# TinfoilHat0/Defending-Against-Backdoors-with-Robust-Learning-Rate

Hardware: NVIDIA H100
Metric: fl_rounds_per_sec (higher is better)
Workload: dtype bf16

## Files before the change

### defending-against-backdoors-with-robust-learning-rate_b200/models/native.py

```python
from __future__ import annotations

import math
import os

import torch
import torch.nn.functional as F

from .. import ops
from .graph import FlatLayout

ACT = torch.bfloat16
FUSE_DROPOUT = bool(int(os.environ.get("RLR_FUSE_DROPOUT", "1")))
FUSE_RELU_POOL = bool(int(os.environ.get("RLR_FUSE_RELU_POOL", "1")))
EPILOGUE_BN_STATS = bool(int(os.environ.get("RLR_EPILOGUE_BN_STATS", "0")))
FWD_BRANCH = bool(int(os.environ.get("RLR_FWD_BRANCH", "1")))
BWD_BRANCH = bool(int(os.environ.get("RLR_BWD_BRANCH", "1")))
EPI_STAT_SLOTS = min(16, max(1, int(os.environ.get("RLR_EPI_STAT_SLOTS", "2"))))
FWD_SLOTS = BWD_SLOTS = max(1, int(os.environ.get("RLR_BN_SLOTS", "1")))
WGRAD_OVERLAP = bool(int(os.environ.get("RLR_WGRAD_OVERLAP", "1")))


def dropout_stream_base(seed: int, agent_id: int, rnd: int) -> int:
    z = (int(seed) * 0x9E3779B97F4A7C15 + (int(agent_id) + 1) * 0xBF58476D1CE4E5B9 + (int(rnd) + 1) * 0x94D049BB133111EB) & (2 ** 64 - 1)
    z = ((z ^ (z >> 30)) * 0xBF58476D1CE4E5B9) & (2 ** 64 - 1)
    z = ((z ^ (z >> 27)) * 0x94D049BB133111EB) & (2 ** 64 - 1)
    return (z ^ (z >> 31)) & (2 ** 62 - 1)


def native_supported(layout: FlatLayout) -> bool:
    return all(nd.op in ("conv", "bn", "relu", "maxpool", "avgpool", "flatten", "dropout", "linear", "save", "add")
               for nd in layout.nodes)


class _Op:
    __slots__ = ("kind", "node", "name", "attrs", "x", "y", "res", "relu", "saved", "acc_dx", "need_dx", "in_shape", "out_shape")

    def __init__(self, kind, **kw):
        self.kind = kind
        self.node = self.name = self.x = self.y = self.res = None
        self.attrs, self.relu, self.saved, self.acc_dx, self.need_dx = {}, False, {}, False, True
        self.in_shape = self.out_shape = None
        for k, v in kw.items():
            setattr(self, k, v)


class NativeNet:
    def __init__(self, layout: FlatLayout, device, max_batch: int, impl: str | dict = "auto", seed: int = 0, act_dtype=None):
        self.layout, self.device, self.max_batch = layout, torch.device(device), int(max_batch)
        self.act_dtype = act_dtype or ACT
        default = ("sm100" if self.device.type == "cuda" else "aten") if impl == "auto" else impl
        self.impl = dict(conv_fwd=default, conv_dgrad=default, conv_wgrad=default, bn=default, pool=default,
                         linear=default, dropout=default) if not isinstance(impl, dict) else dict(impl)
        self.seed = seed
        self.fuse_bn_stats = False
        self.first_wait = None
        self.after_first_op = None
        self.step_counter = torch.zeros(1, dtype=torch.int64, device=device)
        self._build_plan()
        self._alloc()

    def _build_plan(self):
        nodes = self.layout.nodes
        C, H, W = self.layout.in_shape
        shape = {"x": (H, W, C)}
        ver = {"x": 0}
        tid = lambda s: f"{s}@{ver[s]}"
        self.tshape = {tid("x"): shape["x"]}
        plan, consumed = [], set()
        pending_bn = {}
        alias = {}

        def new_out(slot, shp):
            ver[slot] = ver.get(slot, -1) + 1
            shape[slot] = shp
            self.tshape[tid(slot)] = shp
            return tid(slot)

        def next_same_slot(i, slot):
            for j in range(i + 1, len(nodes)):
                if j in consumed:
                    continue
                nd = nodes[j]
                if nd.op == "save":
                    if nd.inp == slot:
                        return None, None
                    continue
                if nd.inp == slot or nd.out == slot:
                    return j, nd
            return None, None

        for i, nd in enumerate(nodes):
            if i in consumed:
                continue
            a = nd.attrs
            if nd.op == "save":
                ver[nd.out] = ver.get(nd.out, -1) + 1
                alias[f"{nd.out}@{ver[nd.out]}"] = tid(nd.inp)
                shape[nd.out] = shape[nd.inp]
                self.tshape[f"{nd.out}@{ver[nd.out]}"] = shape[nd.inp]
                continue
            src = alias.get(tid(nd.inp), tid(nd.inp))
            if nd.op == "conv":
                h, w, c = shape[nd.inp]
                k, s, p = a["k"], a.get("stride", 1), a.get("pad", 0)
                ho, wo = (h + 2 * p - k) // s + 1, (w + 2 * p - k) // s + 1
                op = _Op("conv", node=i, name=nd.name, attrs=a, x=src, in_shape=(h, w, c), out_shape=(ho, wo, a["cout"]))
                j, nx = next_same_slot(i, nd.out)
                want_stats = nx is not None and nx.op == "bn"
                if nx is not None and nx.op == "relu":
                    op.relu = True
                    consumed.add(j)
                op.saved["want_stats"] = want_stats
                op.y = new_out(nd.out, op.out_shape)
                plan.append(op)
            elif nd.op == "bn":
                shp = shape[nd.inp]
                op = _Op("bn", node=i, name=nd.name, attrs=a, x=src, in_shape=shp, out_shape=shp)
                j, nx = next_same_slot(i, nd.out)
                if nx is not None and nx.op == "relu":
                    op.relu = True
                    consumed.add(j)
                    op.y = new_out(nd.out, shp)
                    plan.append(op)
                elif nx is not None and nx.op == "add":
                    pending_bn[j] = op
                else:
                    op.y = new_out(nd.out, shp)
                    plan.append(op)
            elif nd.op == "add":
                other = alias.get(tid(a["other"]), tid(a["other"]))
                op = pending_bn.pop(i, None)
                if op is None:
                    raise NotImplementedError("add without a preceding BatchNorm is not used by any model in the zoo")
                op.res = other
                j, nx = next_same_slot(i, nd.out)
                if nx is not None and nx.op == "relu":
                    op.relu = True
                    consumed.add(j)
                op.y = new_out(nd.out, op.out_shape)
                plan.append(op)
            elif nd.op == "relu":
                raise NotImplementedError("stand-alone ReLU (every ReLU in the zoo follows conv/bn/linear)")
            elif nd.op == "maxpool":
                h, w, c = shape[nd.inp]
                op = _Op("maxpool", node=i, x=src, in_shape=(h, w, c), out_shape=(h // 2, w // 2, c))
                op.y = new_out(nd.out, op.out_shape)
                plan.append(op)
            elif nd.op == "avgpool":
                h, w, c = shape[nd.inp]
                op = _Op("avgpool", node=i, x=src, in_shape=(h, w, c), out_shape=(1, 1, c))
                op.y = new_out(nd.out, op.out_shape)
                plan.append(op)
            elif nd.op == "flatten":
                shp = shape[nd.inp]
                ver[nd.out] += 1
                alias[tid(nd.out)] = src
                shape[nd.out] = (int(math.prod(shp)),)
                self.tshape[tid(nd.out)] = shape[nd.out]
            elif nd.op == "dropout":
                shp = shape[nd.inp]
                prod = next((q for q in reversed(plan) if q.y == src), None)
                fusable = (prod is not None and a.get("p", 0.0) > 0 and "drop" not in prod.saved and
                           (prod.kind == "maxpool" or
                            (prod.kind == "linear" and prod.relu and ops.linear_fused_dropout_ok(prod.attrs["cout"], prod.attrs["cin"]))))
                if fusable and FUSE_DROPOUT:
                    prod.saved["drop"] = (float(a["p"]), i)
                    ver[nd.out] += 1
                    alias[tid(nd.out)] = src
                    shape[nd.out] = shp
                    self.tshape[tid(nd.out)] = shp
                else:
                    op = _Op("dropout", node=i, attrs=a, x=src, in_shape=shp, out_shape=shp)
                    op.y = new_out(nd.out, shp)
                    plan.append(op)
            elif nd.op == "linear":
                op = _Op("linear", node=i, name=nd.name, attrs=a, x=src, in_shape=shape[nd.inp], out_shape=(a["cout"],))
                j, nx = next_same_slot(i, nd.out)
                if nx is not None and nx.op == "relu":
                    op.relu = True
                    consumed.add(j)
                op.y = new_out(nd.out, op.out_shape)
                plan.append(op)
            else:
                raise NotImplementedError(nd.op)
        for op in plan:
            if op.kind != "maxpool":
                continue
            prod = next((q for q in plan if q.y == op.x), None)
            users = [q for q in plan if q.x == op.x or q.res == op.x]
            if prod is not None and prod.kind == "conv" and prod.relu and len(users) == 1 and FUSE_RELU_POOL:
                op.saved["relu_bwd_here"] = True
                prod.saved["relu_bwd_fused"] = True
        self.plan = plan
        self.alias = alias
        self.out_tid = alias.get(tid("x"), tid("x"))
        self.in_tid = "x@0"
        written = set()
        for op in reversed(plan):
            op.need_dx = op.x != self.in_tid
            if op.res is not None:
                written.add(op.res)
            if op.need_dx:
                op.acc_dx = op.x in written
                written.add(op.x)

    def _numel(self, shp):
        return int(math.prod(shp))

    def _alloc(self):
        B, dev = self.max_batch, self.device
        self.act, self.grad = {}, {}
        for op in self.plan:
            self.act[op.y] = torch.empty((B, *op.out_shape), dtype=self.act_dtype, device=dev)
        for op in self.plan:
            for t in (op.x, op.res):
                if t is not None and t != self.in_tid and t not in self.grad:
                    self.grad[t] = torch.empty((B, *self.tshape[t]), dtype=self.act_dtype, device=dev)
        self.grad[self.out_tid] = torch.empty((B, *self.tshape[self.out_tid]), dtype=self.act_dtype, device=dev)
        self.logits = torch.empty((B, self.tshape[self.out_tid][-1]), dtype=torch.float32, device=dev)
        need = [op for op in self.plan if op.kind == "bn" or (op.kind == "conv" and op.saved.get("want_stats"))]
        S = ops.STAT_SLOTS
        tot = sum(2 * op.out_shape[-1] for op in need)
        self.stats_arena = torch.zeros(max(1, tot * S), dtype=torch.float32, device=dev)
        D = BWD_SLOTS
        self.dsum_arena = torch.zeros(max(1, tot * D), dtype=torch.float32, device=dev)
        off = 0
        for op in need:
            c = op.out_shape[-1]
            op.saved["stats"] = self.stats_arena[off * S:(off + 2 * c) * S].view(S, 2, c)
            op.saved["dsum"] = self.dsum_arena[off * D:(off + 2 * c) * D].view(D, 2, c)
            op.saved["mean_rstd"] = torch.zeros(2, c, dtype=torch.float32, device=dev)
            off += 2 * c
        for op in self.plan:
            if op.kind == "maxpool":
                op.saved["idx"] = torch.empty((B, *op.out_shape), dtype=torch.uint8, device=dev)
                if "drop" in op.saved and self.impl["pool"] != "sm100":
                    op.saved["dmask"] = torch.ones((B, *op.out_shape), dtype=torch.uint8, device=dev)
            if op.kind == "dropout":
                op.saved["mask"] = torch.empty((B, *op.out_shape), dtype=torch.uint8, device=dev)
        self._bn_src = {}
        for i, op in enumerate(self.plan):
            if not (FWD_BRANCH and op.kind == "conv" and ".downsample." in (op.name or "")):
                continue
            nxt = self.plan[i + 1] if i + 1 < len(self.plan) else None
            first = next((q for q in self.plan[:i] if q.x == op.x and q is not op), None)
            join = next((q for q in self.plan[i + 1:] if nxt is not None and q.res == nxt.y), None)
            if nxt is None or nxt.kind != "bn" or nxt.x != op.y or first is None or join is None:
                continue
            first.saved["fork_before"] = True
            op.saved["side_branch"] = nxt.saved["side_branch"] = True
            join.saved["join_before"] = True
        for i, op in enumerate(self.plan):
            if op.kind == "bn":
                prod = next((q for q in self.plan[:i] if q.y == op.x and q.kind == "conv"), None)
                op.saved["producer"] = prod

    def bind(self, w, wb, g, w_buffers=None):
        self.w, self.wb, self.g = w, wb, g
        lay = self.layout
        self.pw = {p.name: lay.view(w, p) for p in lay.params}
        self.pw.update({b.name: lay.view(w if w_buffers is None else w_buffers, b) for b in lay.buffers})
        self.pwb = {p.name: lay.view(wb, p) for p in lay.params} if wb is not None else {}
        self.pg = {p.name: lay.view(g, p) for p in lay.params} if g is not None else {}

    def T(self, t, B):
        return self.act[t][:B] if t != self.in_tid else self._x

    def stem_geometry(self):
        op = self.plan[0]
        if op.kind != "conv" or op.x != self.in_tid or self.impl["conv_fwd"] != "sm100" or self.impl["conv_wgrad"] != "sm100":
            return None
        return ops.stem_geometry(op.in_shape, op.attrs)

    def G(self, t, B):
        return self.grad[t][:B]

    def forward(self, x_nhwc, train: bool):
        out = self.forward_raw(x_nhwc, train)
        B = out.shape[0]
        self.logits[:B].copy_(out)
        return self.logits[:B]

    def forward_raw(self, x_nhwc, train: bool):
        B = x_nhwc.shape[0] if x_nhwc.dim() == 4 else x_nhwc.shape[0] // (self.plan[0].out_shape[0] * self.plan[0].out_shape[1])
        self._x, self._B, self._train = x_nhwc, B, train
        self._epoch = getattr(self, "_epoch", 0) + 1
        if train:
            ops.zero_(self.stats_arena)
        branch = FWD_BRANCH and self.device.type == "cuda" and ops.nn.USE_STRIDED_TMA and self.impl["conv_fwd"] == "sm100"
        if branch and getattr(self, "_branch_stream", None) is None:
            self._branch_stream = torch.cuda.Stream(self.device)
        for i, op in enumerate(self.plan):
            if branch and op.saved.get("fork_before"):
                self._branch_stream.wait_stream(torch.cuda.current_stream(self.device))
            if branch and op.saved.get("join_before"):
                torch.cuda.current_stream(self.device).wait_stream(self._branch_stream)
            if branch and op.saved.get("side_branch"):
                with torch.cuda.stream(self._branch_stream):
                    getattr(self, "_fwd_" + op.kind)(op, B, train)
            else:
                getattr(self, "_fwd_" + op.kind)(op, B, train)
            if i == 0 and self.after_first_op is not None:
                self.after_first_op()
        return self.T(self.out_tid, B).reshape(B, -1)

    def dlogits_buffer(self, B):
        return self.G(self.out_tid, B).reshape(B, -1)

    def backward(self, dlogits):
        B = dlogits.shape[0]
        gout = self.G(self.out_tid, B)
        if dlogits.data_ptr() != gout.data_ptr():
            gout.copy_(dlogits.reshape(gout.shape))
        ops.zero_(self.g)
        ops.zero_(self.dsum_arena)
        self._side = None
        if WGRAD_OVERLAP and self.device.type == "cuda":
            if getattr(self, "_side_stream", None) is None:
                self._side_stream = torch.cuda.Stream(self.device)
            self._side = self._side_stream
            self._side.wait_stream(torch.cuda.current_stream(self.device))
        branch = (BWD_BRANCH and FWD_BRANCH and self.device.type == "cuda" and ops.nn.USE_STRIDED_TMA and self.impl["conv_fwd"] == "sm100"
                  and getattr(self, "_branch_stream", None) is not None)
        cur = torch.cuda.current_stream(self.device) if branch else None
        for op in reversed(self.plan):
            if branch and op.saved.get("fork_before"):
                cur.wait_stream(self._branch_stream)
            if branch and op.saved.get("side_branch"):
                if op.kind == "bn":
                    self._branch_stream.wait_stream(cur)
                with torch.cuda.stream(self._branch_stream):
                    getattr(self, "_bwd_" + op.kind)(op, B)
            else:
                getattr(self, "_bwd_" + op.kind)(op, B)
        if self._side is not None:
            torch.cuda.current_stream(self.device).wait_stream(self._side)
            self._side = None

    def _epilogue_stats_free(self, op):
        if not EPILOGUE_BN_STATS or self.impl["conv_fwd"] != "sm100":
            return False
        a = op.attrs
        return a.get("stride", 1) == 1 and a["cin"] % 64 == 0 and a["cout"] % 64 == 0 and not (a["k"] == 3 and a["cin"] == 64)

    def _fwd_conv(self, op, B, train):
        a = op.attrs
        x, y = self.T(op.x, B), self.T(op.y, B)
        bias = self.pw.get(op.name + ".bias")
        stats = op.saved.get("stats") if (train and op.saved.get("want_stats") and (self.fuse_bn_stats or self._epilogue_stats_free(op))) else None
        op.saved["stats_done"] = stats is not None
        if self.impl["conv_fwd"] == "sm100" and ops.conv_supported(op.in_shape, a, "fwd"):
            ops.conv2d_fwd_sm100(x, self.pwb[op.name + ".weight"], bias, y, a.get("stride", 1), a.get("pad", 0), op.relu, stats, tag=(id(self), op.name),
                                 zero_stats=False, s2d_epoch=self._epoch, wait=self.first_wait if (op is self.plan[0] and x.dim() == 2) else None)
            return
        if self.impl["conv_fwd"] == "sm100":
            ops.note_fallback("conv_fwd", f"{op.name} in={op.in_shape} {a}")
        wt = self.pwb[op.name + ".weight"].permute(0, 3, 1, 2)
        out = F.conv2d(x.permute(0, 3, 1, 2), wt, bias.to(self.act_dtype) if bias is not None else None, a.get("stride", 1), a.get("pad", 0))
        if op.relu:
            out = F.relu(out)
        y.copy_(out.permute(0, 2, 3, 1))
        if stats is not None:
            yf = y.float().reshape(-1, y.shape[-1])
            stats[0, 0].copy_(yf.sum(0)); stats[0, 1].copy_((yf * yf).sum(0))

    def _bwd_conv(self, op, B):
        a = op.attrs
        x, y, dy = self.T(op.x, B), self.T(op.y, B), self.G(op.y, B)
        if op.relu and not op.saved.get("relu_bwd_fused"):
            ops.relu_bwd_(dy, y, self.impl["bn"])
        name = op.name + ".weight"
        gw, gb = self.pg[name], self.pg.get(op.name + ".bias")
        s, p = a.get("stride", 1), a.get("pad", 0)
        if self.impl["conv_wgrad"] == "sm100" and ops.conv_supported(op.in_shape, a, "wgrad"):
            if getattr(self, "_side", None) is not None:
                self._side.wait_stream(torch.cuda.current_stream(self.device))
                with torch.cuda.stream(self._side):
                    ops.conv2d_wgrad_sm100(x, dy, gw, gb, s, p, tag=(id(self), op.name), zero=False)
            else:
                ops.conv2d_wgrad_sm100(x, dy, gw, gb, s, p, tag=(id(self), op.name), zero=False)
        else:
            if self.impl["conv_wgrad"] == "sm100":
                ops.note_fallback("conv_wgrad", f"{op.name} in={op.in_shape} {a}")
            _, dw, db = torch.ops.aten.convolution_backward(
                dy.permute(0, 3, 1, 2), x.permute(0, 3, 1, 2), self.pwb[name].permute(0, 3, 1, 2),
                [a["cout"]] if gb is not None else None, [s, s], [p, p], [1, 1], False, [0, 0], 1, [False, True, gb is not None])
            gw.copy_(dw.permute(0, 2, 3, 1))
            if gb is not None:
                gb.copy_(db)
        if not op.need_dx:
            return
        dx = self.G(op.x, B)
        if self.impl["conv_dgrad"] == "sm100" and ops.conv_supported(op.in_shape, a, "dgrad"):
            ops.conv2d_dgrad_sm100(dy, self.pwb[name], dx, s, p, op.acc_dx)
            return
        if self.impl["conv_dgrad"] == "sm100":
            ops.note_fallback("conv_dgrad", f"{op.name} in={op.in_shape} {a}")
        di, _, _ = torch.ops.aten.convolution_backward(
            dy.permute(0, 3, 1, 2), x.permute(0, 3, 1, 2), self.pwb[name].permute(0, 3, 1, 2), None, [s, s], [p, p], [1, 1],
            False, [0, 0], 1, [True, False, False])
        di = di.permute(0, 2, 3, 1)
        if op.acc_dx:
            dx.add_(di)
        else:
            dx.copy_(di)

    def _fwd_bn(self, op, B, train):
        a = op.attrs
        x, y = self.T(op.x, B), self.T(op.y, B)
        res = self.T(op.res, B) if op.res is not None else None
        gamma, beta = self.pw[op.name + ".weight"], self.pw[op.name + ".bias"]
        rm, rv = self.pw[op.name + ".running_mean"], self.pw[op.name + ".running_var"]
        prod = op.saved["producer"]
        stats = prod.saved["stats"] if (train and prod is not None and prod.saved.get("stats_done")) else None
        if stats is not None and not self.fuse_bn_stats:
            stats = stats[0:EPI_STAT_SLOTS]
        count = x.numel() // x.shape[-1]
        ops.bn_fwd(x, y, res, gamma, beta, rm, rv, stats, op.saved["mean_rstd"], count, a.get("eps", 1e-5),
                   a.get("momentum", 0.1), train, op.relu, self.impl["bn"],
                   stats_buf=op.saved["stats"][0:FWD_SLOTS] if train else None)

    def _bwd_bn(self, op, B):
        x, y, dy = self.T(op.x, B), self.T(op.y, B), self.G(op.y, B)
        dres = self.G(op.res, B) if op.res is not None else None
        dx = self.G(op.x, B)
        gamma = self.pw[op.name + ".weight"]
        ops.bn_bwd(dy, y, x, gamma, op.saved["mean_rstd"], op.saved["dsum"], dx, dres,
                   self.pg[op.name + ".weight"], self.pg[op.name + ".bias"], op.relu, self.impl["bn"], zero_dsum=False,
                   beta=self.pw[op.name + ".bias"])

    def _drop(self, op, train=True):
        d = op.saved.get("drop")
        return (d[0], self.seed, self.step_counter, d[1]) if (d is not None and train) else None

    def _fwd_maxpool(self, op, B, train):
        drop = self._drop(op, train)
        op.saved["drop_on"] = drop is not None
        mask = op.saved["dmask"][:B] if (drop is not None and "dmask" in op.saved) else None
        ops.maxpool2_fwd(self.T(op.x, B), self.T(op.y, B), op.saved["idx"][:B], self.impl["pool"], drop, mask)

    def _bwd_maxpool(self, op, B):
        drop = self._drop(op, op.saved.get("drop_on", False))
        mask = op.saved["dmask"][:B] if (drop is not None and "dmask" in op.saved) else None
        ops.maxpool2_bwd(self.G(op.y, B), op.saved["idx"][:B], self.G(op.x, B), self.impl["pool"], drop, mask,
                         relu_out=self.T(op.y, B) if op.saved.get("relu_bwd_here") else None)

    def _fwd_avgpool(self, op, B, train):
        ops.avgpool_fwd(self.T(op.x, B), self.T(op.y, B), self.impl["pool"])

    def _bwd_avgpool(self, op, B):
        ops.avgpool_bwd(self.G(op.y, B), self.G(op.x, B), self.impl["pool"])

    def _fwd_dropout(self, op, B, train):
        x, y = self.T(op.x, B), self.T(op.y, B)
        if not train:
            y.copy_(x.reshape(y.shape))
            return
        ops.dropout_fwd(x.reshape(B, -1), y.reshape(B, -1), op.saved["mask"][:B].reshape(B, -1), op.attrs["p"], self.seed,
                        self.step_counter, op.node, self.impl["dropout"])

    def _bwd_dropout(self, op, B):
        ops.dropout_bwd(self.G(op.y, B).reshape(B, -1), op.saved["mask"][:B].reshape(B, -1), self.G(op.x, B).reshape(B, -1),
                        op.attrs["p"], self.impl["dropout"])

    def _fwd_linear(self, op, B, train):
        x, y = self.T(op.x, B).reshape(B, -1), self.T(op.y, B)
        drop = self._drop(op, train)
        op.saved["drop_on"] = drop is not None
        ops.linear_fwd(x, self.pwb[op.name + ".weight"], self.pw.get(op.name + ".bias"), y, op.relu, self.impl["linear"], drop)

    def _bwd_linear(self, op, B):
        x, y, dy = self.T(op.x, B).reshape(B, -1), self.T(op.y, B), self.G(op.y, B)
        if op.relu:
            scale = 1.0 / (1.0 - op.saved["drop"][0]) if op.saved.get("drop_on", False) else 1.0
            ops.relu_bwd_(dy, y, self.impl["bn"], scale)
        dx = self.G(op.x, B).reshape(B, -1) if op.need_dx else None
        ops.linear_bwd(x, dy, self.pwb[op.name + ".weight"], dx, self.pg[op.name + ".weight"], self.pg.get(op.name + ".bias"),
                       op.acc_dx, self.impl["linear"], zero=False)


class NativeTrainer:
    name = "native"

    def __init__(self, layout, args, device, max_shard: int, impl="auto"):
        self.layout, self.args = layout, args
        self.device = torch.device(device)
        assert self.device.type == "cuda", "the native trainer runs on sm_90a devices only"
        n = layout.n_total
        self.w = torch.zeros(n, dtype=torch.float32, device=device)
        self.wb = torch.zeros(n, dtype=torch.bfloat16, device=device)
        self.g = torch.zeros(n, dtype=torch.float32, device=device)
        self.m = torch.zeros(n, dtype=torch.float32, device=device)
        self.bs = args.bs
        self.net = NativeNet(layout, device, self.bs, impl, seed=args.seed)
        self.net.bind(self.w, self.wb, self.g)
        self.opt = ops.FlatSGD(n, device, args.client_lr, args.client_moment, 10.0, args.clip, n_pgd=layout.n_vote)
        self.loss_sum = torch.zeros(1, dtype=torch.float32, device=device)
        self.use_graphs = not args.no_graphs
        self.max_shard = max_shard
        self.perm = torch.zeros(max(1, max_shard), dtype=torch.int64, device=device)
        self.cursor = torch.zeros(1, dtype=torch.int32, device=device)
        self.y = torch.zeros(self.bs, dtype=torch.int64, device=device)
        C, H, W = layout.in_shape
        self.x = torch.zeros(self.bs, H, W, C, dtype=ACT, device=device)
        self.stem = self.net.stem_geometry()
        self.xA = torch.zeros(self.bs * self.stem[2] * self.stem[3], 64, dtype=ACT, device=device) if self.stem else None
        self._graphs = {}
        self._eval_nets = {}
        self.bcast = None

    def attach_broadcast(self, fused):
        if self.stem is None or fused.w_bf16 is None:
            return False
        self.bcast = fused
        return True

    def _bind_first(self, w0):
        f = self.bcast
        self.net.bind(f.w_global, f.w_bf16, self.g, w_buffers=self.w)
        lay = self.layout
        first_w = lay.by_name[self.net.plan[0].name + ".weight"]
        lo, hi = f.slices_of(first_w.offset, first_w.offset + first_w.numel)
        self.net.first_wait = (f.ready_ptr, lo, hi, f.epoch_dev) if f.ready_ptr else None
        tail_src, tail_dst = f.w_global[lay.n_vote:], self.w[lay.n_vote:]
        self.net.after_first_op = lambda: ops.ext().acquire_slices(f.ready_ptr, 0, max(0, f.n_slices - 1), f.epoch_dev, tail_src, tail_dst)

    def _bind_normal(self):
        self.net.bind(self.w, self.wb, self.g)
        self.net.first_wait = None
        self.net.after_first_op = None

    def _step(self, dataset, B, w0, first=False):
        if first:
            self._bind_first(w0)
        meta = dataset.meta
        if self.stem is not None:
            k, pad, Ho, Wo = self.stem
            xin = self.xA[:B * Ho * Wo]
            ops.gather_im2col(dataset.data, self.perm, meta.mean, meta.std, k, pad, xin, cursor=self.cursor, targets=dataset.targets,
                              out_labels=self.y, batch=B)
        else:
            xin = self.x[:B]
            ops.gather_normalize(dataset.data, self.perm, meta.mean, meta.std, out=xin, nhwc=True, cursor=self.cursor,
                                 targets=dataset.targets, out_labels=self.y, batch=B)
        logits = self.net.forward_raw(xin, True)
        _, dl = ops.softmax_xent(logits, self.y[:B], True, self.loss_sum, dlogits=self.net.dlogits_buffer(B))
        self.net.backward(dl)
        self.opt.step(self.w, self.g, self.m, w0=w0, w_bf16=self.wb, w_in=self.bcast.w_global if first else None)
        ops.ext().advance_cursor(self.cursor, B, self.net.step_counter)
        if first:
            self._bind_normal()

    def _get_graph(self, dataset, B, w0, first=False):
        key = (B, dataset.data.data_ptr(), w0.data_ptr(), bool(first))
        if key in self._graphs:
            return self._graphs[key]
        keep = (self.w.clone(), self.wb.clone(), self.m.clone(), self.cursor.clone(), self.loss_sum.clone(),
                self.net.step_counter.clone())
        self.perm.zero_()
        s = torch.cuda.Stream(self.device)
        s.wait_stream(torch.cuda.current_stream(self.device))
        with torch.cuda.stream(s):
            for _ in range(3):
                self.cursor.zero_()
                c0 = ops.launch_calls()
                self._step(dataset, B, w0, first)
                self._launches = ops.launch_calls() - c0
        torch.cuda.current_stream(self.device).wait_stream(s)
        self.cursor.zero_()
        graph = torch.cuda.CUDAGraph()
        with torch.cuda.graph(graph, capture_error_mode="thread_local"):
            self._step(dataset, B, w0, first)
        self.w.copy_(keep[0]); self.wb.copy_(keep[1]); self.m.copy_(keep[2]); self.cursor.copy_(keep[3])
# ... 58 lines not shown
```

### defending-against-backdoors-with-robust-learning-rate_b200/ops/csrc/common.cuh

```cuda
#pragma once
#include <cuda_runtime.h>
#include <cuda_bf16.h>
#include <stdint.h>

#include "dropspec.h"

#define RLR_CUDA_CHECK(expr)                                                                     \
    do {                                                                                         \
        cudaError_t _e = (expr);                                                                 \
        if (_e != cudaSuccess) return _e;                                                        \
    } while (0)

namespace rlr {

constexpr int kWarp = 32;

__device__ __forceinline__ void pdl_wait() { asm volatile("griddepcontrol.wait;" ::: "memory"); }
__device__ __forceinline__ void pdl_trigger() { asm volatile("griddepcontrol.launch_dependents;" ::: "memory"); }

extern int g_pdl;
bool pdl_enabled();

template <typename... KArgs, typename... Args>
inline cudaError_t launch_kernel(void (*kernel)(KArgs...), dim3 grid, dim3 block, size_t smem, cudaStream_t st, Args&&... args) {
    if (!pdl_enabled()) {
        kernel<<<grid, block, smem, st>>>(static_cast<KArgs>(args)...);
        return cudaGetLastError();
    }
    cudaLaunchConfig_t cfg = {};
    cfg.gridDim = grid; cfg.blockDim = block; cfg.dynamicSmemBytes = smem; cfg.stream = st;
    cudaLaunchAttribute attr[1];
    attr[0].id = cudaLaunchAttributeProgrammaticStreamSerialization;
    attr[0].val.programmaticStreamSerializationAllowed = 1;
    cfg.attrs = attr; cfg.numAttrs = 1;
    return cudaLaunchKernelEx(&cfg, kernel, static_cast<KArgs>(args)...);
}

void* scratch_alloc(size_t bytes, cudaStream_t st);
void scratch_free(void* p);
struct Scratch {
    void* p;
    Scratch(size_t bytes, cudaStream_t st) : p(scratch_alloc(bytes, st)) {}
    ~Scratch() { scratch_free(p); }
    Scratch(const Scratch&) = delete;
    Scratch& operator=(const Scratch&) = delete;
    template <typename T> T* as() const { return static_cast<T*>(p); }
};
template <typename T>
__global__ void __launch_bounds__(256) ordered_sum_kernel(T* __restrict__ out, const T* __restrict__ part, int nparts, long long n) {
    pdl_wait();
    pdl_trigger();
    for (long long i = (long long)blockIdx.x * 256 + threadIdx.x; i < n; i += (long long)gridDim.x * 256) {
        T s = part[i];
        for (int j = 1; j < nparts; ++j) s += part[(size_t)j * n + i];
        out[i] += s;
    }
}

template <typename T>
__global__ void __launch_bounds__(256) ordered_sum_cols_kernel(T* __restrict__ out, const T* __restrict__ part, int nparts, long long n) {
    constexpr int kRows = 64, kPerWarp = kRows / 8;
    __shared__ T tile[kRows][33];
    pdl_wait();
    pdl_trigger();
    const int lane = threadIdx.x & 31, warp = threadIdx.x >> 5;
    const long long col = (long long)blockIdx.x * 32 + lane;
    T s = T(0);
    for (int j0 = 0; j0 < nparts; j0 += kRows) {
        T v[kPerWarp];
#pragma unroll
        for (int q = 0; q < kPerWarp; ++q) {
            const int j = j0 + warp + 8 * q;
            v[q] = (j < nparts && col < n) ? part[(size_t)j * n + col] : T(0);
        }
#pragma unroll
        for (int q = 0; q < kPerWarp; ++q) tile[warp + 8 * q][lane] = v[q];
        __syncthreads();
        if (warp == 0) {
            const int rows = nparts - j0 < kRows ? nparts - j0 : kRows;
            int r = 0;
            if (j0 == 0) { s = tile[0][lane]; r = 1; }
            for (; r < rows; ++r) s += tile[r][lane];
        }
        __syncthreads();
    }
    if (warp == 0 && col < n) out[col] += s;
}

__device__ __forceinline__ unsigned long long gtimer() {
    unsigned long long t;
    asm volatile("mov.u64 %0, %%globaltimer;" : "=l"(t));
    return t;
}

__device__ __forceinline__ float warp_sum(float v) {
#pragma unroll
    for (int o = 16; o > 0; o >>= 1) v += __shfl_xor_sync(0xffffffffu, v, o);
    return v;
}
__device__ __forceinline__ double warp_sum(double v) {
#pragma unroll
    for (int o = 16; o > 0; o >>= 1) v += __shfl_xor_sync(0xffffffffu, v, o);
    return v;
}
__device__ __forceinline__ unsigned long long warp_sum(unsigned long long v) {
#pragma unroll
    for (int o = 16; o > 0; o >>= 1) v += __shfl_xor_sync(0xffffffffu, v, o);
    return v;
}
__device__ __forceinline__ int warp_sum(int v) {
#pragma unroll
    for (int o = 16; o > 0; o >>= 1) v += __shfl_xor_sync(0xffffffffu, v, o);
    return v;
}

__device__ __forceinline__ float warp_transpose_sum32(float (&v)[32], int lane) {
#define RLR_TSTAGE(O, N)                                                         \
    {                                                                            \
        const bool up = (lane & (O)) != 0;                                       \
        _Pragma("unroll") for (int i = 0; i < (N); ++i) {                        \
            const float send = up ? v[i] : v[i + (N)];                           \
            const float keep = up ? v[i + (N)] : v[i];                           \
            v[i] = keep + __shfl_xor_sync(0xffffffffu, send, (O));               \
        }                                                                        \
    }
    RLR_TSTAGE(16, 16) RLR_TSTAGE(8, 8) RLR_TSTAGE(4, 4) RLR_TSTAGE(2, 2) RLR_TSTAGE(1, 1)
#undef RLR_TSTAGE
    return v[0];
}

template <typename T>
__device__ __forceinline__ T block_sum(T v, T* scratch) {
    v = warp_sum(v);
    const int lane = threadIdx.x & 31, wid = threadIdx.x >> 5;
    if (lane == 0) scratch[wid] = v;
    __syncthreads();
    const int nw = (blockDim.x + 31) >> 5;
    v = (threadIdx.x < nw) ? scratch[threadIdx.x] : T(0);
    if (wid == 0) v = warp_sum(v);
    __syncthreads();
    return v;
}

__device__ __forceinline__ float4 ld_stream_f4(const float* p) {
    float4 r;
    asm volatile("ld.global.nc.L1::no_allocate.v4.f32 {%0,%1,%2,%3}, [%4];"
                 : "=f"(r.x), "=f"(r.y), "=f"(r.z), "=f"(r.w) : "l"(p));
    return r;
}
__device__ __forceinline__ float4 ld_f4(const float* p) {
    float4 r;
    asm volatile("ld.global.v4.f32 {%0,%1,%2,%3}, [%4];"
                 : "=f"(r.x), "=f"(r.y), "=f"(r.z), "=f"(r.w) : "l"(p));
    return r;
}
__device__ __forceinline__ float ld_f1(const float* p) {
    float r;
    asm volatile("ld.global.f32 %0, [%1];" : "=f"(r) : "l"(p));
    return r;
}
__device__ __forceinline__ void st_f4(float* p, float4 v) {
    asm volatile("st.global.v4.f32 [%0], {%1,%2,%3,%4};" ::"l"(p), "f"(v.x), "f"(v.y), "f"(v.z), "f"(v.w) : "memory");
}
__device__ __forceinline__ void multimem_st_f4(float* mc, float4 v) {
    asm volatile("multimem.st.relaxed.sys.global.v4.f32 [%0], {%1,%2,%3,%4};" ::"l"(mc), "f"(v.x), "f"(v.y),
                 "f"(v.z), "f"(v.w) : "memory");
}
__device__ __forceinline__ void multimem_st_b2(uint2* mc, uint2 v) {
    asm volatile("multimem.st.relaxed.sys.global.v2.f32 [%0], {%1,%2};" ::"l"(mc), "f"(__uint_as_float(v.x)),
                 "f"(__uint_as_float(v.y)) : "memory");
}

__device__ __forceinline__ void st_release_sys(uint32_t* p, uint32_t v) {
    asm volatile("st.release.sys.global.u32 [%0], %1;" ::"l"(p), "r"(v) : "memory");
}
__device__ __forceinline__ uint32_t ld_acquire_sys(const uint32_t* p) {
    uint32_t v;
    asm volatile("ld.acquire.sys.global.u32 %0, [%1];" : "=r"(v) : "l"(p) : "memory");
    return v;
}
__device__ __forceinline__ void st_release_gpu(uint32_t* p, uint32_t v) {
    asm volatile("st.release.gpu.global.u32 [%0], %1;" ::"l"(p), "r"(v) : "memory");
}
__device__ __forceinline__ uint32_t ld_acquire_gpu(const uint32_t* p) {
    uint32_t v;
    asm volatile("ld.acquire.gpu.global.u32 %0, [%1];" : "=r"(v) : "l"(p) : "memory");
    return v;
}

struct Philox {
    uint32_t k0, k1;
    __device__ __forceinline__ Philox(uint64_t seed) : k0((uint32_t)seed), k1((uint32_t)(seed >> 32)) {}
    __device__ __forceinline__ uint4 operator()(uint64_t ctr, uint64_t stream) const {
        uint32_t c0 = (uint32_t)ctr, c1 = (uint32_t)(ctr >> 32), c2 = (uint32_t)stream, c3 = (uint32_t)(stream >> 32);
        uint32_t a = k0, b = k1;
#pragma unroll
        for (int r = 0; r < 10; ++r) {
            const uint32_t hi0 = __umulhi(0xD2511F53u, c0), lo0 = 0xD2511F53u * c0;
            const uint32_t hi1 = __umulhi(0xCD9E8D57u, c2), lo1 = 0xCD9E8D57u * c2;
            const uint32_t n0 = hi1 ^ c1 ^ a, n2 = hi0 ^ c3 ^ b;
            c0 = n0; c1 = lo1; c2 = n2; c3 = lo0;
            a += 0x9E3779B9u; b += 0xBB67AE85u;
        }
        return make_uint4(c0, c1, c2, c3);
    }
};
__device__ __forceinline__ float u32_to_unit(uint32_t x) {
    return ((float)(x >> 8) + 1.0f) * (1.0f / 16777216.0f);
}
__device__ __forceinline__ float4 philox_normal4(const Philox& ph, uint64_t ctr, uint64_t stream) {
    const uint4 u = ph(ctr, stream);
    const float r0 = sqrtf(-2.0f * logf(u32_to_unit(u.x))), r1 = sqrtf(-2.0f * logf(u32_to_unit(u.z)));
    float s0, c0, s1, c1;
    sincospif(2.0f * u32_to_unit(u.y), &s0, &c0);
    sincospif(2.0f * u32_to_unit(u.w), &s1, &c1);
    return make_float4(r0 * c0, r0 * s0, r1 * c1, r1 * s1);
}

__device__ __forceinline__ uint32_t dropout_keep8(const DropSpec& d, long long q) {
    const Philox ph(d.seed);
    const uint4 u = ph((uint64_t)q, ((uint64_t)(*d.step) << 20) ^ d.stream);
    const uint32_t r[4] = {u.x, u.y, u.z, u.w};
    uint32_t keep = 0;
#pragma unroll
    for (int i = 0; i < 8; ++i) keep |= (uint32_t)(((r[i >> 1] >> (16 * (i & 1))) & 0xffffu) >= d.thr) << i;
    return keep;
}

template <typename T>
inline cudaError_t launch_ordered_sum(T* out, const T* part, int nparts, long long n, cudaStream_t st) {
    if (nparts >= 16)
        return launch_kernel(ordered_sum_cols_kernel<T>, dim3((unsigned)((n + 31) / 32)), dim3(256), (size_t)0, st, out, part, nparts, n);
    long long blocks = (n + 255) / 256;
    if (blocks > 1024) blocks = 1024;
    if (blocks < 1) blocks = 1;
    return launch_kernel(ordered_sum_kernel<T>, dim3((unsigned)blocks), dim3(256), (size_t)0, st, out, part, nparts, n);
}

__device__ __forceinline__ uint32_t pack_bf16x2(float lo, float hi) {
    __nv_bfloat162 v = __floats2bfloat162_rn(lo, hi);
    return *reinterpret_cast<uint32_t*>(&v);
}

}
```

### defending-against-backdoors-with-robust-learning-rate_b200/ops/csrc/conv_halo.cu

```cuda
#include <cuda.h>

#include "common.cuh"
#include "gemm.h"
#include "wgmma.cuh"

namespace rlr {

using namespace wg;

cudaError_t make_tmap_bf16(CUtensorMap* map, const void* base, int rank, const uint64_t* dims, const uint64_t* strides_bytes,
                           const uint32_t* box, const uint32_t* elem_strides = nullptr);

constexpr int HL_THREADS = 256 + 32;
constexpr int HL_TH = 16, HL_TW = 8;
constexpr int HL_PITCH = 16;
constexpr int HL_HALO_BYTES = (HL_TH + 2) * HL_PITCH * 128;
constexpr int HL_W_BYTES = 9 * 64 * 128;
constexpr int HL_STAGES = 3;
constexpr int HL_PITCH_OUT = 64 * 2 + 16;
constexpr int HL_STAGING = 128 * HL_PITCH_OUT;
constexpr int HL_SMEM = HL_W_BYTES + HL_STAGES * HL_HALO_BYTES + 2 * HL_STAGING + 1024 + 1024;

struct HaloParams {
    int NB, H, W;
    int pad;
    int tiles_h, tiles_w, num_tiles;
    int N;
    void* out; int ldc;
    const float* bias;
    float* stats;
    int relu, accumulate;
    long long* dbg;
    int bo_mode;
};

struct __align__(8) HaloShared {
    uint64_t w_full;
    uint64_t halo_full[HL_STAGES];
    uint64_t halo_empty[HL_STAGES];
    float red[128];
    float bias[64];
};

template <bool kStats, bool kAcc>
__global__ void __launch_bounds__(HL_THREADS, 1)
umma_conv3x3_halo_kernel(const __grid_constant__ CUtensorMap tmX, const __grid_constant__ CUtensorMap tmW, const HaloParams p) {
    extern __shared__ uint8_t smem_raw[];
    uint8_t* smem = reinterpret_cast<uint8_t*>((reinterpret_cast<uintptr_t>(smem_raw) + 1023) & ~uintptr_t(1023));
    uint8_t* s_w = smem;
    uint8_t* s_halo = smem + HL_W_BYTES;
    uint8_t* s_stage = s_halo + HL_STAGES * HL_HALO_BYTES;
    HaloShared* sh = reinterpret_cast<HaloShared*>(s_stage + 2 * HL_STAGING);
    const int warp = threadIdx.x >> 5, lane = threadIdx.x & 31;
    const int tile_n = blockIdx.y;
    const int col0 = tile_n * 64;

    if (warp == 8 && lane == 0) {
        prefetch_tmap(&tmX); prefetch_tmap(&tmW);
        mbar_init(&sh->w_full, 1);
        for (int s = 0; s < HL_STAGES; ++s) { mbar_init(&sh->halo_full[s], 1); mbar_init(&sh->halo_empty[s], 4); }
        fence_barrier_init();
    }
    if (threadIdx.x < 128) sh->red[threadIdx.x] = 0.f;
    const int tiles_per_img = p.tiles_h * p.tiles_w;
    pdl_wait();
    pdl_trigger();
    if (threadIdx.x < 64) sh->bias[threadIdx.x] = (p.bias && col0 + (int)threadIdx.x < p.N) ? p.bias[col0 + threadIdx.x] : 0.f;
    __syncthreads();

    if (warp == 8) {
        if (lane == 0) {
            mbar_expect_tx(&sh->w_full, HL_W_BYTES);
            for (int t = 0; t < 9; ++t) tma_load_2d(&tmW, &sh->w_full, s_w + t * 8192, t * 64, tile_n * 64);
            int stage = 0;
            uint32_t phase = 0;
            for (int tile = blockIdx.x; tile < p.num_tiles; tile += gridDim.x) {
                const int n = tile / tiles_per_img, r = tile - n * tiles_per_img;
                const int h0 = (r / p.tiles_w) * HL_TH, w0 = (r % p.tiles_w) * HL_TW;
                mbar_wait(&sh->halo_empty[stage], phase ^ 1);
                mbar_expect_tx(&sh->halo_full[stage], HL_HALO_BYTES);
                tma_load_4d(&tmX, &sh->halo_full[stage], s_halo + stage * HL_HALO_BYTES, 0, w0 - p.pad, h0 - p.pad, n);
                if (++stage == HL_STAGES) { stage = 0; phase ^= 1; }
            }
        }
    } else {
        const int wgi = threadIdx.x >> 7, t = threadIdx.x & 127;
        uint8_t* stage_buf = s_stage + wgi * HL_STAGING;
        const int r0 = frag_row(t, 0);
        __nv_bfloat16* out = reinterpret_cast<__nv_bfloat16*>(p.out);
        float st1[16], st2[16];
#pragma unroll
        for (int i = 0; i < 16; ++i) { st1[i] = 0.f; st2[i] = 0.f; }
        const uint32_t w_base = smem_u32(s_w);
        mbar_wait(&sh->w_full, 0);
        for (int q = wgi;; q += 2) {
            const int tile = blockIdx.x + q * gridDim.x;
            if (tile >= p.num_tiles) break;
            const int stage = q % HL_STAGES;
            const uint32_t phase = (uint32_t)(q / HL_STAGES) & 1u;
            const int n = tile / tiles_per_img, r = tile - n * tiles_per_img;
            const int h0 = (r / p.tiles_w) * HL_TH, w0 = (r % p.tiles_w) * HL_TW;
            uint4 oldv[8];
            if (kAcc) {
#pragma unroll
                for (int it = 0; it < 8; ++it) {
                    const int idx = t + it * 128, rr = idx >> 3, ch = idx & 7;
                    const int h = h0 + (rr >> 3), w = w0 + (rr & 7);
                    oldv[it] = make_uint4(0, 0, 0, 0);
                    if (col0 + ch * 8 < p.N && h < p.H && w < p.W)
                        oldv[it] = *reinterpret_cast<const uint4*>(out + (((size_t)n * p.H + h) * p.W + w) * p.ldc + col0 + ch * 8);
                }
            }
            const bool trace = p.dbg && blockIdx.x == 0 && blockIdx.y == 0 && t == 0;
            if (trace) p.dbg[q * 8 + 0] = clock64();
            mbar_wait(&sh->halo_full[stage], phase);
            if (trace) p.dbg[q * 8 + 2] = clock64();
            const uint32_t halo = smem_u32(s_halo + stage * HL_HALO_BYTES);
            float acc[2][32];
#pragma unroll
            for (int m = 0; m < 2; ++m)
#pragma unroll
                for (int i = 0; i < 32; ++i) acc[m][i] = 0.f;
            wgmma_fence();
#pragma unroll
            for (int tp = 0; tp < 9; ++tp) {
                const int dy = tp / 3, dx = tp - dy * 3;
#pragma unroll
                for (int k = 0; k < 4; ++k) {
                    const uint64_t db = smem_desc_sw128(w_base + tp * 8192 + k * 32, 16, 1024);
#pragma unroll
                    for (int m = 0; m < 2; ++m) {
                        const uint32_t a0 = halo + (dy * HL_PITCH + dx) * 128 + m * 8 * HL_PITCH * 128 + k * 32;
                        const uint32_t bo = p.bo_mode ? ((a0 >> 7) & 7u) : 0u;
                        wgmma_bf16<64, 0, 0>(acc[m], smem_desc_sw128(a0, 16, HL_PITCH * 128, bo), db, (tp > 0 || k > 0) ? 1u : 0u);
                    }
                }
            }
            wgmma_commit();
            wgmma_wait<0>();
            fence_acc(acc[0]);
            fence_acc(acc[1]);
            if (lane == 0) mbar_arrive(&sh->halo_empty[stage]);
            if (trace) p.dbg[q * 8 + 3] = clock64();
#pragma unroll
            for (int m = 0; m < 2; ++m)
#pragma unroll
                for (int j = 0; j < 8; ++j) {
                    const int c = frag_col(t, 4 * j);
#pragma unroll
                    for (int h = 0; h < 2; ++h) {
                        float a = acc[m][4 * j + 2 * h], b = acc[m][4 * j + 2 * h + 1];
                        a += sh->bias[c]; b += sh->bias[c + 1];
                        if (p.relu) { a = fmaxf(a, 0.f); b = fmaxf(b, 0.f); }
                        const uint32_t packed = pack_bf16x2(a, b);
                        if (kStats) {
                            const float2 rq = __bfloat1622float2(*reinterpret_cast<const __nv_bfloat162*>(&packed));
                            st1[2 * j] += rq.x; st1[2 * j + 1] += rq.y;
                            st2[2 * j] += rq.x * rq.x; st2[2 * j + 1] += rq.y * rq.y;
                        }
                        *reinterpret_cast<uint32_t*>(stage_buf + (m * 64 + r0 + 8 * h) * HL_PITCH_OUT + c * 2) = packed;
                    }
                }
            named_bar(1 + wgi, 128);
            if (trace) p.dbg[q * 8 + 6] = clock64();
#pragma unroll
            for (int it = 0; it < 8; ++it) {
                const int idx = t + it * 128;
                const int rr = idx >> 3, ch = idx & 7;
                if (col0 + ch * 8 >= p.N) continue;
                const int h = h0 + (rr >> 3), w = w0 + (rr & 7);
                if (h >= p.H || w >= p.W) continue;
                const size_t gi = ((size_t)n * p.H + h) * p.W + w;
                uint4 val = *reinterpret_cast<const uint4*>(stage_buf + rr * HL_PITCH_OUT + ch * 16);
                uint4* gp = reinterpret_cast<uint4*>(out + gi * p.ldc + col0 + ch * 8);
                if (kAcc) {
                    const __nv_bfloat162* o2 = reinterpret_cast<const __nv_bfloat162*>(&oldv[it]);
                    __nv_bfloat162* v2 = reinterpret_cast<__nv_bfloat162*>(&val);
#pragma unroll
                    for (int qq = 0; qq < 4; ++qq) {
                        const float2 a = __bfloat1622float2(v2[qq]), b = __bfloat1622float2(o2[qq]);
                        v2[qq] = __floats2bfloat162_rn(a.x + b.x, a.y + b.y);
                    }
                }
                *gp = val;
            }
            named_bar(1 + wgi, 128);
            if (trace) p.dbg[q * 8 + 7] = clock64();
        }
        if (kStats) {
#pragma unroll
            for (int i = 0; i < 16; ++i)
#pragma unroll
                for (int o = 4; o < 32; o <<= 1) {
                    st1[i] += __shfl_xor_sync(0xffffffffu, st1[i], o);
                    st2[i] += __shfl_xor_sync(0xffffffffu, st2[i], o);
                }
            if (lane < 4)
#pragma unroll
                for (int i = 0; i < 16; ++i) {
                    const int c = frag_col(t, 2 * (i & ~1)) + (i & 1);
                    atomicAdd(&sh->red[c], st1[i]);
                    atomicAdd(&sh->red[64 + c], st2[i]);
                }
            named_bar(3, 256);
            if (threadIdx.x < 128 && col0 + (threadIdx.x & 63) < p.N)
                atomicAdd(p.stats + (size_t)(blockIdx.x % kStatSlots) * 2 * p.N + (threadIdx.x < 64 ? 0 : p.N) + col0 + (threadIdx.x & 63),
                          sh->red[threadIdx.x]);
        }
    }
}

cudaError_t launch_conv3x3_halo_bf16(const void* x, const void* w, void* out, int NB, int Hin, int Win, int H, int W, int Cout, const float* bias,
                                     int relu, int accumulate, float* stats, int bo_mode, long long* dbg, int num_sms, cudaStream_t st) {
    const int pad = (H - Hin + 2) / 2;
    if (pad < 0 || pad > 2 || H != Hin + 2 * pad - 2 || W != Win + 2 * pad - 2 || H < 1 || W < 1 || Cout % 8) return cudaErrorInvalidValue;
    if (stats && (H % HL_TH || W % HL_TW)) return cudaErrorInvalidValue;
    static bool configured = false;
    if (!configured) {
        RLR_CUDA_CHECK(cudaFuncSetAttribute(umma_conv3x3_halo_kernel<false, false>, cudaFuncAttributeMaxDynamicSharedMemorySize, HL_SMEM));
        RLR_CUDA_CHECK(cudaFuncSetAttribute(umma_conv3x3_halo_kernel<true, false>, cudaFuncAttributeMaxDynamicSharedMemorySize, HL_SMEM));
        RLR_CUDA_CHECK(cudaFuncSetAttribute(umma_conv3x3_halo_kernel<false, true>, cudaFuncAttributeMaxDynamicSharedMemorySize, HL_SMEM));
        configured = true;
    }
    if (stats && accumulate) return cudaErrorInvalidValue;
    HaloParams p{};
    p.NB = NB; p.H = H; p.W = W; p.pad = pad;
    p.tiles_h = (H + HL_TH - 1) / HL_TH; p.tiles_w = (W + HL_TW - 1) / HL_TW; p.num_tiles = NB * p.tiles_h * p.tiles_w;
    p.N = Cout; p.out = out; p.ldc = Cout; p.bias = bias; p.stats = stats; p.relu = relu; p.accumulate = accumulate; p.bo_mode = bo_mode; p.dbg = dbg;
    CUtensorMap tmX, tmW;
    {
        const uint64_t d[4] = {64, (uint64_t)Win, (uint64_t)Hin, (uint64_t)NB};
        const uint64_t s[3] = {128, (uint64_t)Win * 128, (uint64_t)Hin * Win * 128};
        const uint32_t b[4] = {64, HL_PITCH, HL_TH + 2, 1};
        RLR_CUDA_CHECK(make_tmap_bf16(&tmX, x, 4, d, s, b));
    }
    {
        const uint64_t d[2] = {9 * 64, (uint64_t)Cout}, s[1] = {9 * 64 * 2};
        const uint32_t b[2] = {64, 64};
        RLR_CUDA_CHECK(make_tmap_bf16(&tmW, w, 2, d, s, b));
    }
    const int n_tiles_n = (Cout + 63) / 64;
    int gx = num_sms / n_tiles_n;
    if (gx > p.num_tiles) gx = p.num_tiles;
    if (gx < 1) gx = 1;
    const dim3 grid(gx, n_tiles_n);
    if (stats) return launch_kernel(umma_conv3x3_halo_kernel<true, false>, grid, dim3(HL_THREADS), HL_SMEM, st, tmX, tmW, p);
    if (accumulate) return launch_kernel(umma_conv3x3_halo_kernel<false, true>, grid, dim3(HL_THREADS), HL_SMEM, st, tmX, tmW, p);
    return launch_kernel(umma_conv3x3_halo_kernel<false, false>, grid, dim3(HL_THREADS), HL_SMEM, st, tmX, tmW, p);
}

}
```

### defending-against-backdoors-with-robust-learning-rate_b200/ops/csrc/gemm.cu

```cuda
#include <cuda.h>
#include <stdlib.h>

#include "common.cuh"
#include "gemm.h"
#include "stem_gather.cuh"
#include "wgmma.cuh"

namespace rlr {

using namespace wg;

constexpr int BM = 128;
constexpr int BK = 64;
constexpr int kConsumers = 256;
constexpr int kThreads = kConsumers + 64;
constexpr int kEpiThreads = kConsumers;

template <int BN, int kOcc = 2>
struct TileCfg {
    static constexpr int kStages = kOcc == 3 ? (BN == 64 ? 3 : 2) : (BN == 64 ? 4 : 3);
    static constexpr int kABytes = BM * BK * 2;
    static constexpr int kBBytes = BN * BK * 2;
    static constexpr int kStageBytes = kABytes + kBBytes;
    static constexpr int kPitch = BN * 2 + 16;
    static constexpr int kStagingBytes = BM * kPitch;
    static constexpr int kRingBytes = kStages * kStageBytes;
    static_assert(kStagingBytes + 2 * BN * 4 <= kRingBytes, "staging aliases the operand ring");
    static constexpr int kTailBytes = BN == 128 ? 2048 : 1024;
    static constexpr int kSmemBytes = kRingBytes + 1024  + kTailBytes;
};

struct __align__(8) SharedTail {
    uint64_t full[4];
    uint64_t empty[4];
    uint64_t pad0;
    uint32_t pad1;
    uint32_t pad2;
    int row_index[BM];
};
static_assert(sizeof(SharedTail) <= 640, "the bias slice starts 640 bytes into the tail");

template <int BN, bool kStats, bool kBMN, int kOcc = 2>
__global__ void __launch_bounds__(kThreads, kOcc)
umma_conv_gemm_kernel(const __grid_constant__ CUtensorMap tmA, const __grid_constant__ CUtensorMap tmB, const __grid_constant__ CUtensorMap tmC,
                       const ConvGemmParams p) {
    using Cfg = TileCfg<BN, kOcc>;
    extern __shared__ uint8_t smem_raw[];
    uint8_t* smem = reinterpret_cast<uint8_t*>((reinterpret_cast<uintptr_t>(smem_raw) + 1023) & ~uintptr_t(1023));
    SharedTail* tail = reinterpret_cast<SharedTail*>(smem + Cfg::kRingBytes);

    const int warp = threadIdx.x >> 5, lane = threadIdx.x & 31;
    const int tile_m = blockIdx.x, tile_n = blockIdx.y;
    long long* dbg = p.dbg ? p.dbg + ((size_t)blockIdx.y * gridDim.x + blockIdx.x) * 8 : nullptr;
    if (dbg && threadIdx.x == 0) { dbg[0] = (long long)gtimer(); uint32_t sm; asm volatile("mov.u32 %0, %%smid;" : "=r"(sm)); dbg[7] = sm; }

    int n0 = 0, h0 = 0, w0 = 0;
    if (p.mode == 1) {
        const int tw_i = tile_m % p.tiles_w;
        const int th_i = (tile_m / p.tiles_w) % p.tiles_h;
        const int tn_i = tile_m / (p.tiles_w * p.tiles_h);
        w0 = tw_i * p.TW; h0 = th_i * p.TH; n0 = tn_i * p.TN;
    }

    if (warp == 8 && lane == 0) {
        prefetch_tmap(&tmA);
        prefetch_tmap(&tmB);
        if (p.tma_store) prefetch_tmap(&tmC);
        for (int s = 0; s < Cfg::kStages; ++s) { mbar_init(&tail->full[s], (p.split_prod || p.b_src) ? 2 : 1); mbar_init(&tail->empty[s], 8); }
        fence_barrier_init();
    }
    if (threadIdx.x < BM) {
        const int r = threadIdx.x;
        int gi;
        if (p.mode == 1) {
            const int tw = r % p.TW, th = (r / p.TW) % p.TH, tn = r / (p.TW * p.TH);
            const int w = w0 + tw, h = h0 + th, n = n0 + tn;
            gi = (w < p.Wo && h < p.Ho && n < p.NB) ? ((n * p.OutH + h * p.out_stride + p.out_ph) * p.OutW + w * p.out_stride + p.out_pw) : -1;
        } else {
            gi = tile_m * BM + r;
            if (gi >= p.M) gi = -1;
        }
        tail->row_index[r] = gi;
    }
    __syncthreads();
    pdl_wait();
    pdl_trigger();
    if (dbg && threadIdx.x == 0) dbg[1] = (long long)gtimer();

    if (warp == 8) {
        if (p.b_src) {
            if (lane == 0) {
                mbar_expect_tx(&tail->full[0], Cfg::kABytes);
                tma_load_2d(&tmA, &tail->full[0], smem, 0, tile_m * BM);
            }
            stem_gather_b(p, smem + Cfg::kABytes, BN, tile_n, lane);
            if (lane == 0) mbar_arrive(&tail->full[0]);
        } else if (lane == 0) {
            int stage = 0;
            uint32_t phase = 0;
            for (int kb = 0; kb < p.num_kb; ++kb) {
                mbar_wait(&tail->empty[stage], phase ^ 1);
                uint8_t* sa = smem + stage * Cfg::kStageBytes;
                uint8_t* sb = sa + Cfg::kABytes;
                mbar_expect_tx(&tail->full[stage], p.split_prod ? Cfg::kABytes : Cfg::kStageBytes);
                if (dbg && kb == 0) dbg[2] = (long long)gtimer();
                if (p.mode == 1) {
                    const int tap = kb / p.cblocks, cb = kb - tap * p.cblocks;
                    tma_load_4d(&tmA, &tail->full[stage], sa, cb * BK, w0 * p.in_stride + p.dw[tap], h0 * p.in_stride + p.dh[tap],
                                n0 + p.dn[tap]);
                } else {
                    tma_load_2d(&tmA, &tail->full[stage], sa, kb * BK, tile_m * BM);
                }
                if (p.split_prod) {
                } else if (kBMN) {
                    const int tap = kb / p.cblocks, cb = kb - tap * p.cblocks;
                    for (int g = 0; g < BN / 64; ++g)
                        tma_load_2d(&tmB, &tail->full[stage], sb + g * 8192, p.wtap[tap] * p.wcols + tile_n * BN + g * 64, cb * BK);
                } else {
                    tma_load_2d(&tmB, &tail->full[stage], sb, kb * BK, tile_n * BN);
                }
                if (++stage == Cfg::kStages) { stage = 0; phase ^= 1; }
            }
        }
    } else if (warp == 9) {
        if (p.split_prod && lane == 0) {
            int stage = 0;
            uint32_t phase = 0;
            for (int kb = 0; kb < p.num_kb; ++kb) {
                mbar_wait(&tail->empty[stage], phase ^ 1);
                uint8_t* sb = smem + stage * Cfg::kStageBytes + Cfg::kABytes;
                mbar_expect_tx(&tail->full[stage], Cfg::kBBytes);
                if (kBMN) {
                    const int tap = kb / p.cblocks, cb = kb - tap * p.cblocks;
                    for (int g = 0; g < BN / 64; ++g)
                        tma_load_2d(&tmB, &tail->full[stage], sb + g * 8192, p.wtap[tap] * p.wcols + tile_n * BN + g * 64, cb * BK);
                } else {
                    tma_load_2d(&tmB, &tail->full[stage], sb, kb * BK, tile_n * BN);
                }
                if (++stage == Cfg::kStages) { stage = 0; phase ^= 1; }
            }
        }
    } else {
        const int et = threadIdx.x;
        const int wgi = et >> 7, t = et & 127;
        const int col0 = tile_n * BN;
        const bool has_bias = !kBMN && p.bias != nullptr;
        float* bias_w = reinterpret_cast<float*>(reinterpret_cast<uint8_t*>(tail) + 640);
        if (has_bias)
            for (int i = et; i < BN; i += kEpiThreads) bias_w[i] = (col0 + i < p.N) ? p.bias[col0 + i] : 0.f;
        float acc[BN / 2];
#pragma unroll
        for (int i = 0; i < BN / 2; ++i) acc[i] = 0.f;
        {
            int stage = 0;
            uint32_t phase = 0;
            consumer_mainloop<BN, Cfg::kStages, Cfg::kStageBytes, Cfg::kABytes, kBMN>(
                acc, smem, tail->full, tail->empty, p.num_kb, (uint32_t)wgi * 64 * 128, p.b_src ? smem_u32(smem + Cfg::kABytes) : 0u,
                stage, phase, lane);
        }
        if (dbg && et == 0) dbg[4] = (long long)gtimer();
        named_bar(1, kEpiThreads);
        if (dbg && et == 0) dbg[5] = (long long)gtimer();
        const float* bias_s = bias_w;
        uint8_t* staging = smem;
        float* red = reinterpret_cast<float*>(staging + Cfg::kStagingBytes);
        const int r0 = wgi * 64 + frag_row(t, 0);
        int gi_r[2];
        gi_r[0] = tail->row_index[r0];
        gi_r[1] = tail->row_index[r0 + 8];
        if (kStats) {
            for (int i = et; i < 2 * BN; i += kEpiThreads) red[i] = 0.f;
            named_bar(1, kEpiThreads);
        }
        const bool tma_out = !kStats && p.tma_store;
#pragma unroll
        for (int j = 0; j < BN / 8; ++j) {
            const int c = frag_col(t, 4 * j);
            float s1[2] = {0.f, 0.f}, s2[2] = {0.f, 0.f};
#pragma unroll
            for (int h = 0; h < 2; ++h) {
                const int row = r0 + 8 * h, gi_row = gi_r[h];
                float a = acc[4 * j + 2 * h], b = acc[4 * j + 2 * h + 1];
                if (has_bias) { a += bias_s[c]; b += bias_s[c + 1]; }
                if (p.relu) { a = fmaxf(a, 0.f); b = fmaxf(b, 0.f); }
                if (p.drop.thr) {
                    const uint32_t keep8 = dropout_keep8(p.drop, ((long long)(gi_row < 0 ? 0 : gi_row) * p.ldc + col0 + 8 * j) >> 3);
                    a = (keep8 >> (c & 7) & 1) ? a * p.drop.scale : 0.f;
                    b = (keep8 >> ((c & 7) + 1) & 1) ? b * p.drop.scale : 0.f;
                }
                const uint32_t packed = pack_bf16x2(a, b);
                if (kStats && gi_row >= 0) {
                    const float2 rq = __bfloat1622float2(*reinterpret_cast<const __nv_bfloat162*>(&packed));
                    s1[0] += rq.x; s1[1] += rq.y; s2[0] += rq.x * rq.x; s2[1] += rq.y * rq.y;
                }
                if (tma_out)
                    *reinterpret_cast<uint32_t*>(staging + (c >> 6) * (BM * 128) + row * 128 + ((((c & 63) >> 3) ^ (row & 7)) << 4) + (c & 7) * 2) = packed;
                else
                    *reinterpret_cast<uint32_t*>(staging + row * Cfg::kPitch + c * 2) = packed;
            }
            if (kStats) {
#pragma unroll
                for (int o = 4; o < 32; o <<= 1)
#pragma unroll
                    for (int e = 0; e < 2; ++e) {
                        s1[e] += __shfl_xor_sync(0xffffffffu, s1[e], o);
                        s2[e] += __shfl_xor_sync(0xffffffffu, s2[e], o);
                    }
                if (lane < 4) {
                    atomicAdd(&red[c], s1[0]); atomicAdd(&red[c + 1], s1[1]);
                    atomicAdd(&red[BN + c], s2[0]); atomicAdd(&red[BN + c + 1], s2[1]);
                }
            }
        }
        if (tma_out) {
            fence_proxy_async_smem();
            named_bar(1, kEpiThreads);
            if (dbg && et == 0) dbg[6] = (long long)gtimer();
            if (et == 0) {
#pragma unroll
                for (int g = 0; g < BN / 64; ++g) {
                    if (col0 + g * 64 >= p.N) break;
                    if (p.mode == 1) tma_store_4d(&tmC, staging + g * (BM * 128), col0 + g * 64, w0, h0, n0);
                    else tma_store_2d(&tmC, staging + g * (BM * 128), col0 + g * 64, tile_m * BM);
                }
                tma_store_commit();
            }
            if (p.stats) {
                constexpr int kPerCol = kEpiThreads / BN, kRows = BM / kPerCol;
                const int c = et % BN;
                const int r_lo = (et / BN) * kRows, r_hi = r_lo + kRows;
                const uint8_t* colp = staging + (c >> 6) * (BM * 128) + (c & 7) * 2;
                const int chunk = (c & 63) >> 3;
                float s1 = 0.f, s2 = 0.f;
#pragma unroll 8
                for (int r = r_lo; r < r_hi; ++r) {
                    if (tail->row_index[r] < 0) continue;
                    const float v = __bfloat162float(*reinterpret_cast<const __nv_bfloat16*>(colp + r * 128 + ((chunk ^ (r & 7)) << 4)));
                    s1 += v; s2 += v * v;
                }
                if (col0 + c < p.N) {
                    float* dst = p.stats + (size_t)(blockIdx.x % p.stat_slots) * 2 * p.N + col0 + c;
                    atomicAdd(dst, s1);
                    atomicAdd(dst + p.N, s2);
                }
            }
            if (et == 0) tma_store_wait_read();
        } else {
        named_bar(1, kEpiThreads);
        if (dbg && et == 0) dbg[6] = (long long)gtimer();
        constexpr int kChunks = BN * 2 / 16;
        __nv_bfloat16* out = reinterpret_cast<__nv_bfloat16*>(p.out);
        constexpr int kIters = BM * kChunks / kEpiThreads;
        constexpr int kBatch = kIters < 8 ? kIters : 8;
#pragma unroll
        for (int it0 = 0; it0 < kIters; it0 += kBatch) {
            uint4 oldv[kBatch];
            if (p.accumulate) {
#pragma unroll
                for (int j = 0; j < kBatch; ++j) {
                    const int idx = et + (it0 + j) * kEpiThreads, r = idx / kChunks, ch = idx - r * kChunks;
                    const int gi = tail->row_index[r];
                    oldv[j] = make_uint4(0, 0, 0, 0);
                    if (gi >= 0 && col0 + ch * 8 < p.N) oldv[j] = *reinterpret_cast<const uint4*>(out + (size_t)gi * p.ldc + col0 + ch * 8);
                }
            }
#pragma unroll
            for (int j = 0; j < kBatch; ++j) {
                const int idx = et + (it0 + j) * kEpiThreads, r = idx / kChunks, ch = idx - r * kChunks;
                const int gi = tail->row_index[r];
                if (gi < 0 || col0 + ch * 8 >= p.N) continue;
                uint4 val = *reinterpret_cast<const uint4*>(staging + r * Cfg::kPitch + ch * 16);
                if (p.accumulate) {
                    const __nv_bfloat162* o2 = reinterpret_cast<const __nv_bfloat162*>(&oldv[j]);
                    __nv_bfloat162* v2 = reinterpret_cast<__nv_bfloat162*>(&val);
#pragma unroll
                    for (int q = 0; q < 4; ++q) {
                        const float2 a = __bfloat1622float2(v2[q]), b = __bfloat1622float2(o2[q]);
                        v2[q] = __floats2bfloat162_rn(a.x + b.x, a.y + b.y);
                    }
                }
                *reinterpret_cast<uint4*>(out + (size_t)gi * p.ldc + col0 + ch * 8) = val;
            }
        }
        if (kStats) {
            named_bar(1, kEpiThreads);
            for (int i = et; i < 2 * BN; i += kEpiThreads)
                if (col0 + (i % BN) < p.N)
                    atomicAdd(p.stats + (size_t)(blockIdx.x % kStatSlots) * 2 * p.N + (i < BN ? 0 : p.N) + col0 + (i % BN), red[i]);
        }
        }
    }
}

typedef CUresult (*EncodeTiledFn)(CUtensorMap*, CUtensorMapDataType, cuuint32_t, void*, const cuuint64_t*, const cuuint64_t*,
                                  const cuuint32_t*, const cuuint32_t*, CUtensorMapInterleave, CUtensorMapSwizzle,
                                  CUtensorMapL2promotion, CUtensorMapFloatOOBfill);

static EncodeTiledFn get_encode_fn() {
    static EncodeTiledFn fn = nullptr;
    if (!fn) {
        void* f = nullptr;
        cudaDriverEntryPointQueryResult q;
        if (cudaGetDriverEntryPoint("cuTensorMapEncodeTiled", &f, cudaEnableDefault, &q) != cudaSuccess || !f) return nullptr;
        fn = reinterpret_cast<EncodeTiledFn>(f);
    }
    return fn;
}

cudaError_t make_tmap_bf16(CUtensorMap* map, const void* base, int rank, const uint64_t* dims, const uint64_t* strides_bytes,
                           const uint32_t* box, const uint32_t* elem_strides = nullptr) {
    EncodeTiledFn fn = get_encode_fn();
    if (!fn) return cudaErrorNotSupported;
    cuuint64_t gd[5], gs[4];
    cuuint32_t bx[5], es[5];
    for (int i = 0; i < rank; ++i) {
        gd[i] = dims[i];
        es[i] = elem_strides ? elem_strides[i] : 1;
        bx[i] = box[i] * es[i];
        if (bx[i] > 256 || es[i] < 1 || es[i] > 8) return cudaErrorInvalidValue;
    }
    for (int i = 0; i + 1 < rank; ++i) gs[i] = strides_bytes[i];
    const CUresult r = fn(map, CU_TENSOR_MAP_DATA_TYPE_BFLOAT16, (cuuint32_t)rank, const_cast<void*>(base), gd, gs, bx, es,
                          CU_TENSOR_MAP_INTERLEAVE_NONE, CU_TENSOR_MAP_SWIZZLE_128B, CU_TENSOR_MAP_L2_PROMOTION_L2_256B,
                          CU_TENSOR_MAP_FLOAT_OOB_FILL_NONE);
    return r == CUDA_SUCCESS ? cudaSuccess : cudaErrorInvalidValue;
}

template <int BN>
cudaError_t launch_persistent_bn(const CUtensorMap& tmA, const CUtensorMap& tmB, const ConvGemmParams& p, int m_tiles, int num_sms,
                                 cudaStream_t st, int occ = 1);

static int g_occ3 = -1;
void set_conv_occ3(int level) { g_occ3 = level < 0 ? 0 : (level > 1 ? 1 : level); }
static int conv_occ3() {
    if (g_occ3 < 0) { const char* e = getenv("RLR_CONV_OCC3"); set_conv_occ3(e ? atoi(e) : 1); }
    return g_occ3;
}

template <int BN>
static cudaError_t launch_bn_occ3(const CUtensorMap& tmA, const CUtensorMap& tmB, const CUtensorMap& tmC, const ConvGemmParams& p, int m_tiles,
                                  cudaStream_t st) {
    using Cfg = TileCfg<BN, 3>;
    static bool configured = false;
    if (!configured) {
        RLR_CUDA_CHECK(cudaFuncSetAttribute(umma_conv_gemm_kernel<BN, false, false, 3>, cudaFuncAttributeMaxDynamicSharedMemorySize, Cfg::kSmemBytes));
        RLR_CUDA_CHECK(cudaFuncSetAttribute(umma_conv_gemm_kernel<BN, false, true, 3>, cudaFuncAttributeMaxDynamicSharedMemorySize, Cfg::kSmemBytes));
        configured = true;
    }
    dim3 grid(m_tiles, (p.N + BN - 1) / BN);
    if (p.b_mn) return launch_kernel(umma_conv_gemm_kernel<BN, false, true, 3>, grid, dim3(kThreads), Cfg::kSmemBytes, st, tmA, tmB, tmC, p);
    return launch_kernel(umma_conv_gemm_kernel<BN, false, false, 3>, grid, dim3(kThreads), Cfg::kSmemBytes, st, tmA, tmB, tmC, p);
}

static int sm_count() {
    static const int sms = [] {
        int dev = 0, n = 0;
        if (cudaGetDevice(&dev) != cudaSuccess || cudaDeviceGetAttribute(&n, cudaDevAttrMultiProcessorCount, dev) != cudaSuccess) return 132;
        return n;
    }();
    return sms;
}

static int g_persistent = -1;
void set_persistent_conv(int on) { g_persistent = on ? 1 : 0; }

static int persistent_sms() {
    if (g_persistent < 0) { const char* e = getenv("RLR_PERSISTENT_CONV"); g_persistent = (e && atoi(e) > 0) ? 1 : 0; }
    if (!g_persistent) return 0;
    static const int sms = [] {
        int dev = 0, n = 0;
        if (cudaGetDevice(&dev) != cudaSuccess || cudaDeviceGetAttribute(&n, cudaDevAttrMultiProcessorCount, dev) != cudaSuccess) return 0;
        return n;
    }();
    return sms;
}

static int g_split_prod = -1;
void set_conv_split_producer(int on) { g_split_prod = on ? 1 : 0; }
static long long* g_trace = nullptr;
void set_conv_trace(long long* buf) { g_trace = buf; }
long long* conv_trace_buf() { return g_trace; }

static int g_tma_store = -1;
void set_conv_tma_store(int on) { g_tma_store = on ? 1 : 0; }
static bool tma_store_enabled() {
    if (g_tma_store < 0) { const char* e = getenv("RLR_TMA_STORE"); g_tma_store = (e && atoi(e) == 0) ? 0 : 1; }
    return g_tma_store != 0;
}
static cudaError_t make_out_tmap(CUtensorMap* tmC, const ConvGemmParams& p) {
    if (p.ldc % 8) return cudaErrorInvalidValue;
    if (p.mode == 1) {
        const uint64_t d[4] = {(uint64_t)p.N, (uint64_t)p.Wo, (uint64_t)p.Ho, (uint64_t)p.NB};
        const uint64_t s[3] = {(uint64_t)p.out_stride * p.ldc * 2, (uint64_t)p.out_stride * p.OutW * p.ldc * 2, (uint64_t)p.OutH * p.OutW * p.ldc * 2};
        const uint32_t b[4] = {64, (uint32_t)p.TW, (uint32_t)p.TH, (uint32_t)p.TN};
        const char* base = reinterpret_cast<const char*>(p.out) + ((size_t)p.out_ph * p.OutW + p.out_pw) * p.ldc * 2;
        return make_tmap_bf16(tmC, base, 4, d, s, b);
    }
    const uint64_t d[2] = {(uint64_t)p.N, (uint64_t)p.M}, s[1] = {(uint64_t)p.ldc * 2};
    const uint32_t b[2] = {64, BM};
    return make_tmap_bf16(tmC, p.out, 2, d, s, b);
}

template <int BN>
static cudaError_t launch_bn(const CUtensorMap& tmA, const CUtensorMap& tmB, const ConvGemmParams& p_in, int m_tiles, cudaStream_t st) {
    using Cfg = TileCfg<BN>;
    ConvGemmParams p = p_in;
    p.dbg = g_trace;
    CUtensorMap tmC = tmA;
    {
        static const int epi_slots = [] { const char* e = getenv("RLR_EPI_STAT_SLOTS"); int v = e ? atoi(e) : 2; return v < 1 ? 1 : (v > kStatSlots ? kStatSlots : v); }();
        p.stat_slots = epi_slots;
    }
    p.tma_store = 0;
    if (tma_store_enabled() && !p.accumulate && ((reinterpret_cast<uintptr_t>(p.out) & 15) == 0) && make_out_tmap(&tmC, p) == cudaSuccess)
        p.tma_store = 1;
    if (g_split_prod < 0) { const char* e = getenv("RLR_SPLIT_PRODUCER"); g_split_prod = (e && atoi(e) == 0) ? 0 : 1; }
    p.split_prod = (g_split_prod && !p.b_src) ? 1 : 0;
    if (p.b_src && !p.stats && p.N <= BN) {
        static const int stem_persistent = [] { const char* e = getenv("RLR_STEM_PERSISTENT"); return e ? atoi(e) : 2; }();
        if (stem_persistent && m_tiles >= 2 * sm_count())
            return launch_persistent_bn<BN>(tmA, tmB, p, m_tiles, sm_count(), st, stem_persistent == 2 ? 2 : 1);
    }
    if (!p.stats && !p.b_src && persistent_sms() > 0 && m_tiles * ((p.N + BN - 1) / BN) > persistent_sms())
        return launch_persistent_bn<BN>(tmA, tmB, p, m_tiles, persistent_sms(), st);
    if constexpr (BN == 64)
        if ((!p.stats || p.tma_store) && conv_occ3() >= 1) return launch_bn_occ3<BN>(tmA, tmB, tmC, p, m_tiles, st);
    static bool configured = false;
    if (!configured) {
        RLR_CUDA_CHECK(cudaFuncSetAttribute(umma_conv_gemm_kernel<BN, false, false>, cudaFuncAttributeMaxDynamicSharedMemorySize, Cfg::kSmemBytes));
        RLR_CUDA_CHECK(cudaFuncSetAttribute(umma_conv_gemm_kernel<BN, true, false>, cudaFuncAttributeMaxDynamicSharedMemorySize, Cfg::kSmemBytes));
        RLR_CUDA_CHECK(cudaFuncSetAttribute(umma_conv_gemm_kernel<BN, false, true>, cudaFuncAttributeMaxDynamicSharedMemorySize, Cfg::kSmemBytes));
        configured = true;
    }
    dim3 grid(m_tiles, (p.N + BN - 1) / BN);
    if (p.b_mn) return launch_kernel(umma_conv_gemm_kernel<BN, false, true>, grid, dim3(kThreads), Cfg::kSmemBytes, st, tmA, tmB, tmC, p);
    if (p.stats && !p.tma_store) return launch_kernel(umma_conv_gemm_kernel<BN, true, false>, grid, dim3(kThreads), Cfg::kSmemBytes, st, tmA, tmB, tmC, p);
    return launch_kernel(umma_conv_gemm_kernel<BN, false, false>, grid, dim3(kThreads), Cfg::kSmemBytes, st, tmA, tmB, tmC, p);
}

static int pick_bn(int N) { return (N % 128 == 0) ? 128 : 64; }

cudaError_t launch_gemm_bf16(const void* A, const void* B, void* out, int M, int N, int K, int lda, int ldb, int ldc,
                             const float* bias, int relu, int accumulate, float* stats, cudaStream_t st, const DropSpec* drop) {
    if (K % BK || N % 8 || M <= 0) return cudaErrorInvalidValue;
    if (drop && drop->thr && (accumulate || stats || ldc % 8)) return cudaErrorInvalidValue;
    const int m_tiles = (M + BM - 1) / BM;
    int bn = pick_bn(N);
    {
        static const int small64 = [] { const char* e = getenv("RLR_GEMM_SMALL_BN64"); return e ? atoi(e) : 0; }();
        if (small64 && bn == 128 && m_tiles * (N / 128) < sm_count()) bn = 64;
    }
    CUtensorMap tmA, tmB;
    {
        const uint64_t d[2] = {(uint64_t)K, (uint64_t)M}, s[1] = {(uint64_t)lda * 2};
        const uint32_t b[2] = {BK, BM};
        RLR_CUDA_CHECK(make_tmap_bf16(&tmA, A, 2, d, s, b));
    }
    {
        const uint64_t d[2] = {(uint64_t)K, (uint64_t)N}, s[1] = {(uint64_t)ldb * 2};
        const uint32_t b[2] = {BK, (uint32_t)bn};
        RLR_CUDA_CHECK(make_tmap_bf16(&tmB, B, 2, d, s, b));
    }
    ConvGemmParams p{};
    p.M = M; p.N = N; p.num_kb = K / BK; p.mode = 0; p.in_stride = 1; p.out_stride = 1;
    p.out = out; p.ldc = ldc; p.bias = bias; p.stats = stats; p.relu = relu; p.accumulate = accumulate;
    if (drop && drop->thr) p.drop = *drop;
    return bn == 128 ? launch_bn<128>(tmA, tmB, p, m_tiles, st) : launch_bn<64>(tmA, tmB, p, m_tiles, st);
}

cudaError_t launch_stem_gemm_bf16(const void* A, const void* W, void* out, int M, int N, int kvalid, int ldw, const float* bias, int relu,
                                  float* stats, const uint32_t* wait_flags, int wait_lo, int wait_hi, const uint32_t* wait_epoch,
                                  cudaStream_t st) {
    if (N % 8 || M <= 0 || kvalid < 1 || kvalid > BK || ldw < kvalid) return cudaErrorInvalidValue;
    if (wait_flags && (!wait_epoch || wait_lo > wait_hi || wait_lo < 0)) return cudaErrorInvalidValue;
    const int m_tiles = (M + BM - 1) / BM;
    const int bn = pick_bn(N);
    CUtensorMap tmA;
    {
        const uint64_t d[2] = {(uint64_t)BK, (uint64_t)M}, s[1] = {(uint64_t)BK * 2};
        const uint32_t b[2] = {BK, BM};
        RLR_CUDA_CHECK(make_tmap_bf16(&tmA, A, 2, d, s, b));
    }
    ConvGemmParams p{};
    p.M = M; p.N = N; p.num_kb = 1; p.mode = 0; p.in_stride = 1; p.out_stride = 1;
    p.out = out; p.ldc = N; p.bias = bias; p.stats = stats; p.relu = relu; p.accumulate = 0;
    p.b_src = reinterpret_cast<const __nv_bfloat16*>(W); p.b_ld = ldw; p.b_kvalid = kvalid;
    p.wait_flags = wait_flags; p.wait_lo = wait_lo; p.wait_hi = wait_hi; p.wait_epoch = wait_epoch;
    return bn == 128 ? launch_bn<128>(tmA, tmA, p, m_tiles, st) : launch_bn<64>(tmA, tmA, p, m_tiles, st);
}

static int pow2_ceil(int x) { int p = 1; while (p < x) p <<= 1; return p; }

cudaError_t launch_conv_bf16(const void* x, const void* w, void* out, int NB, int planes, int Hin, int Win, int Cin, int Ho, int Wo,
                             int Cout, int ldc, int ntaps, const int* dh, const int* dw, const int* dplane, const float* bias,
                             int relu, int accumulate, float* stats, cudaStream_t st, const int* wtap, int w_taps_total,
                             int in_stride, int out_stride, int out_ph, int out_pw) {
    if (Cin % BK || Cout % 8 || ntaps < 1 || ntaps > 9) return cudaErrorInvalidValue;
    if (in_stride < 1 || in_stride > 2 || out_stride < 1 || out_stride > 2 || (in_stride > 1 && planes != 1)) return cudaErrorInvalidValue;
    if (wtap && (stats || Cout % 64)) return cudaErrorInvalidValue;
    int bn = pick_bn(Cout);
    ConvGemmParams p{};
    {
        static const int small_bn64 = [] { const char* e = getenv("RLR_SMALL_BN64"); return e ? atoi(e) : 1; }();
        const long long px = (long long)NB * Ho * Wo;
        if (small_bn64 && bn == 128 && ((px + BM - 1) / BM) * (Cout / 128) < sm_count()) bn = 64;
    }
    int TW = pow2_ceil(Wo); if (TW > BM) TW = BM;
    int TH = pow2_ceil(Ho); if (TW * TH > BM) TH = BM / TW;
    int TN = BM / (TW * TH);
    p.TW = TW; p.TH = TH; p.TN = TN;
    p.tiles_w = (Wo + TW - 1) / TW; p.tiles_h = (Ho + TH - 1) / TH;
    const int tiles_n = (NB + TN - 1) / TN;
    const int m_tiles = p.tiles_w * p.tiles_h * tiles_n;
    p.M = NB * Ho * Wo; p.N = Cout; p.mode = 1; p.cblocks = Cin / BK; p.num_kb = ntaps * p.cblocks; p.ntaps = ntaps;
    p.Ho = Ho; p.Wo = Wo; p.NB = NB;
    p.in_stride = in_stride; p.out_stride = out_stride; p.out_ph = out_ph; p.out_pw = out_pw; p.OutH = Ho * out_stride; p.OutW = Wo * out_stride;
    for (int t = 0; t < ntaps; ++t) { p.dh[t] = (int8_t)dh[t]; p.dw[t] = (int8_t)dw[t]; p.dn[t] = dplane[t] * NB; }
    p.out = out; p.ldc = ldc; p.bias = bias; p.stats = stats; p.relu = relu; p.accumulate = accumulate;
    CUtensorMap tmA, tmB;
    {
        const uint64_t d[4] = {(uint64_t)Cin, (uint64_t)Win, (uint64_t)Hin, (uint64_t)planes * NB};
        const uint64_t s[3] = {(uint64_t)Cin * 2, (uint64_t)Win * Cin * 2, (uint64_t)Hin * Win * Cin * 2};
        const uint32_t b[4] = {BK, (uint32_t)TW, (uint32_t)TH, (uint32_t)TN};
        const uint32_t es[4] = {1, (uint32_t)in_stride, (uint32_t)in_stride, 1};
        RLR_CUDA_CHECK(make_tmap_bf16(&tmA, x, 4, d, s, b, in_stride > 1 ? es : nullptr));
    }
    if (wtap) {
        if (bias) return cudaErrorInvalidValue;
        p.b_mn = 1; p.wcols = Cout;
        for (int t = 0; t < ntaps; ++t) p.wtap[t] = wtap[t];
        const uint64_t cols = (uint64_t)w_taps_total * Cout;
        const uint64_t d[2] = {cols, (uint64_t)Cin}, s[1] = {cols * 2};
        const uint32_t b[2] = {64, BK};
        RLR_CUDA_CHECK(make_tmap_bf16(&tmB, w, 2, d, s, b));
    } else {
        const uint64_t K = (uint64_t)ntaps * Cin;
        const uint64_t d[2] = {K, (uint64_t)Cout}, s[1] = {K * 2};
        const uint32_t b[2] = {BK, (uint32_t)bn};
        RLR_CUDA_CHECK(make_tmap_bf16(&tmB, w, 2, d, s, b));
    }
    return bn == 128 ? launch_bn<128>(tmA, tmB, p, m_tiles, st) : launch_bn<64>(tmA, tmB, p, m_tiles, st);
}

}
```

### defending-against-backdoors-with-robust-learning-rate_b200/ops/csrc/gemm.h

```cpp
#pragma once
#include <cuda_runtime.h>
#include <cuda_bf16.h>
#include <stdint.h>

#include "dropspec.h"

namespace rlr {

constexpr int kStatSlots = 16;

struct ConvGemmParams {
    int M, N, num_kb;
    int mode;
    int cblocks;
    int TW, TH, TN;
    int Ho, Wo, NB;
    int tiles_w, tiles_h;
    int ntaps;
    int in_stride;
    int out_stride, out_ph, out_pw, OutH, OutW;
    int8_t dh[9], dw[9];
    int dn[9];
    int b_mn;
    int wtap[9];
    int wcols;
    DropSpec drop;
    int tma_store;
    int split_prod;
    long long* dbg;
    const __nv_bfloat16* b_src;
    int b_ld, b_kvalid;
    const uint32_t* wait_flags;
    int wait_lo, wait_hi;
    const uint32_t* wait_epoch;
    void* out;
    int ldc;
    const float* bias;
    float* stats;
    int stat_slots;
    int relu, accumulate;
};

cudaError_t launch_gemm_bf16(const void* A, const void* B, void* out, int M, int N, int K, int lda, int ldb, int ldc,
                             const float* bias, int relu, int accumulate, float* stats, cudaStream_t st, const DropSpec* drop = nullptr);
cudaError_t launch_stem_gemm_bf16(const void* A, const void* W, void* out, int M, int N, int kvalid, int ldw, const float* bias, int relu,
                                  float* stats, const uint32_t* wait_flags, int wait_lo, int wait_hi, const uint32_t* wait_epoch,
                                  cudaStream_t st);
void set_pdl(int on);
cudaError_t launch_gemm_splitk_bf16(const void* A, const void* B, void* out, float* ws, int M, int N, int K, const float* bias, int relu,
                                    int num_sms, cudaStream_t st, const DropSpec* drop = nullptr);
void set_persistent_conv(int on);
void set_conv_occ3(int level);
void set_conv_tma_store(int on);
void set_conv_split_producer(int on);
void set_conv_trace(long long* buf);
long long* conv_trace_buf();
cudaError_t launch_conv_bf16(const void* x, const void* w, void* out, int NB, int planes, int Hin, int Win, int Cin, int Ho, int Wo,
                             int Cout, int ldc, int ntaps, const int* dh, const int* dw, const int* dplane, const float* bias,
                             int relu, int accumulate, float* stats, cudaStream_t st, const int* wtap = nullptr, int w_taps_total = 0,
                             int in_stride = 1, int out_stride = 1, int out_ph = 0, int out_pw = 0);

cudaError_t launch_conv3x3_halo_bf16(const void* x, const void* w, void* out, int NB, int Hin, int Win, int H, int W, int Cout, const float* bias,
                                     int relu, int accumulate, float* stats, int bo_mode, long long* dbg, int num_sms, cudaStream_t st);

cudaError_t launch_conv3x3_halo3_bf16(const void* x, const void* w, void* out, int NB, int H, int W, int Cout, const float* bias, int relu,
                                      int accumulate, int num_sms, cudaStream_t st);

cudaError_t launch_conv_wgrad_bf16(const void* dy, const void* x, float* dW, int NB, int planes, int Hin, int Win, int Cin, int Cin_valid,
                                   int Ho, int Wo, int Cout, int ntaps, const int* dh, const int* dw, const int* dplane, int num_sms,
                                   cudaStream_t st, int in_stride = 1);
cudaError_t launch_conv_wgrad_halo_bf16(const void* dy, const void* x, float* dW, int NB, int H, int W, int Cin_valid, int Cout,
                                        int num_sms, cudaStream_t st);
cudaError_t launch_linear_wgrad_bf16(const void* dy, const void* x, float* dW, int B, int N, int K, int num_sms, cudaStream_t st);

cudaError_t launch_ordered_sum_f32(float* out, const float* part, int nparts, long long n, cudaStream_t st);
cudaError_t launch_ordered_sum_f64(double* out, const double* part, int nparts, long long n, cudaStream_t st);
cudaError_t launch_channel_stats(const __nv_bfloat16* x, long long M, int C, float* stats , int num_sms, cudaStream_t st,
                                 int only_sum = 0, int nslots = 1);
cudaError_t launch_bn_finalize(const float* stats, int slots, float* mean_rstd, float* running_mean, float* running_var, int C,
                               float count, float eps, float momentum, int train, cudaStream_t st);
cudaError_t launch_bn_apply(const __nv_bfloat16* x, const __nv_bfloat16* res, __nv_bfloat16* y, const float* gamma, const float* beta,
                            float* mean_rstd, long long M, int C, int relu, int fin_mode, const float* stats, int slots, float count,
                            float eps, float momentum, float* running_mean, float* running_var, int num_sms, cudaStream_t st);
cudaError_t launch_bn_bwd_reduce(const __nv_bfloat16* dy, const __nv_bfloat16* y, const __nv_bfloat16* x, const float* mean_rstd,
                                 float* dsum , long long M, int C, int relu, int num_sms, cudaStream_t st,
                                 const float* gamma = nullptr, const float* beta = nullptr, int nslots = 1);
cudaError_t launch_bn_bwd_apply(const __nv_bfloat16* dy, const __nv_bfloat16* y, const __nv_bfloat16* x, const float* gamma,
                                const float* mean_rstd, const float* dsum, __nv_bfloat16* dx, __nv_bfloat16* dres, float* dgamma,
                                float* dbeta, long long M, int C, int relu, int num_sms, cudaStream_t st, const float* beta = nullptr, int nslots = 1);
cudaError_t launch_relu_bwd(__nv_bfloat16* dy, const __nv_bfloat16* y, long long n, int num_sms, cudaStream_t st, float scale = 1.0f);
cudaError_t launch_maxpool2_fwd(const __nv_bfloat16* x, __nv_bfloat16* y, uint8_t* idx, int B, int H, int W, int C, cudaStream_t st,
                                float drop_p = 0.f, uint64_t seed = 0, const long long* step = nullptr, uint64_t stream = 0);
cudaError_t launch_maxpool2_bwd(const __nv_bfloat16* dy, const uint8_t* idx, __nv_bfloat16* dx, int B, int H, int W, int C, cudaStream_t st,
                                float drop_p, uint64_t seed, const long long* step, uint64_t stream, const __nv_bfloat16* zmask);
cudaError_t launch_avgpool_fwd(const __nv_bfloat16* x, __nv_bfloat16* y, int B, int HW, int C, cudaStream_t st);
cudaError_t launch_avgpool_bwd(const __nv_bfloat16* dy, __nv_bfloat16* dx, int B, int HW, int C, cudaStream_t st);
cudaError_t launch_dropout_fwd(const __nv_bfloat16* x, __nv_bfloat16* y, uint8_t* mask, long long n, float p, uint64_t seed,
                               const long long* step, uint64_t stream, cudaStream_t st);
cudaError_t launch_dropout_bwd(const __nv_bfloat16* dy, const uint8_t* mask, __nv_bfloat16* dx, long long n, float p, cudaStream_t st);
cudaError_t launch_space_to_depth(const __nv_bfloat16* x, __nv_bfloat16* y, int NB, int H, int W, int C, int num_sms, cudaStream_t st);
cudaError_t launch_im2col_small(const __nv_bfloat16* x, __nv_bfloat16* A, int NB, int H, int W, int C, int Ho, int Wo, int k, int pad,
                                int num_sms, cudaStream_t st);
cudaError_t launch_depth_to_space(const __nv_bfloat16* x4, __nv_bfloat16* y, int NB, int H, int W, int C, int accumulate, int plane_mask,
                                  int num_sms, cudaStream_t st);
cudaError_t launch_filter_gather_transpose(const __nv_bfloat16* w, __nv_bfloat16* wt, int Cout, int T, int Cin, int nsub, const int* taps,
                                           cudaStream_t st);
cudaError_t launch_filter_transpose(const __nv_bfloat16* w, __nv_bfloat16* wt, int Cout, int ntaps, int Cin, cudaStream_t st);
cudaError_t launch_linear_small_fwd(const __nv_bfloat16* x, const __nv_bfloat16* w, const float* bias, __nv_bfloat16* y, int B, int K,
                                    int N, int relu, cudaStream_t st);
cudaError_t launch_linear_small_fwd2(const __nv_bfloat16* x, const __nv_bfloat16* w, const float* bias, __nv_bfloat16* y, int B, int K,
                                     int N, int relu, cudaStream_t st);
cudaError_t launch_linear_small_bwd2(const __nv_bfloat16* x, const __nv_bfloat16* dy, const __nv_bfloat16* w, __nv_bfloat16* dx,
                                     float* dw, float* db, int B, int K, int N, int accumulate_dx, cudaStream_t st);
cudaError_t launch_linear_small_bwd(const __nv_bfloat16* x, const __nv_bfloat16* dy, const __nv_bfloat16* w, __nv_bfloat16* dx,
                                    float* dw, float* db, int B, int K, int N, int accumulate_dx, cudaStream_t st);

}
```

### defending-against-backdoors-with-robust-learning-rate_b200/ops/csrc/gemm_binding.cpp

```cpp
#include <torch/extension.h>
#include <ATen/cuda/CUDAContext.h>
#include <c10/cuda/CUDAGuard.h>
#include <c10/cuda/CUDAStream.h>
#include <c10/cuda/CUDACachingAllocator.h>

#include <vector>

#include "gemm.h"

namespace rlr {
void* scratch_alloc(size_t bytes, cudaStream_t st) {
    return c10::cuda::CUDACachingAllocator::raw_alloc_with_stream(bytes < 256 ? 256 : bytes, st);
}
void scratch_free(void* p) { c10::cuda::CUDACachingAllocator::raw_delete(p); }
}

namespace {
inline cudaStream_t cur_stream() { return c10::cuda::getCurrentCUDAStream().stream(); }
inline int num_sms() { return at::cuda::getCurrentDeviceProperties()->multiProcessorCount; }
inline void check(cudaError_t e, const char* what) { TORCH_CHECK(e == cudaSuccess, what, ": ", cudaGetErrorString(e)); }
template <typename T>
inline T* opt(const c10::optional<at::Tensor>& t) { return t.has_value() && t->defined() ? reinterpret_cast<T*>(t->data_ptr()) : nullptr; }
inline const __nv_bfloat16* bf(const at::Tensor& t) {
    TORCH_CHECK(t.is_cuda() && t.scalar_type() == at::kBFloat16 && t.is_contiguous(), "expected contiguous CUDA bf16 tensor");
    return reinterpret_cast<const __nv_bfloat16*>(t.data_ptr());
}
inline __nv_bfloat16* bfm(at::Tensor& t) { return const_cast<__nv_bfloat16*>(bf(t)); }
inline const __nv_bfloat16* bfo(const c10::optional<at::Tensor>& t) { return t.has_value() && t->defined() ? bf(*t) : nullptr; }
inline float* f32(const at::Tensor& t) {
    TORCH_CHECK(t.is_cuda() && t.scalar_type() == at::kFloat && t.is_contiguous(), "expected contiguous CUDA fp32 tensor");
    return reinterpret_cast<float*>(t.data_ptr());
}

static rlr::DropSpec drop_spec(double p, int64_t seed, const c10::optional<at::Tensor>& step, int64_t stream) {
    rlr::DropSpec d{};
    if (p > 0.0) {
        TORCH_CHECK(p < 1.0 && step.has_value() && step->defined() && step->scalar_type() == at::kLong, "fused dropout needs p < 1 and an int64 step counter");
        d.thr = (uint32_t)(p * 65536.0); d.scale = (float)(1.0 / (1.0 - p)); d.seed = (uint64_t)seed; d.stream = (uint64_t)stream;
        d.step = reinterpret_cast<const long long*>(step->data_ptr<int64_t>());
    }
    return d;
}

void gemm_bf16(at::Tensor A, at::Tensor B, at::Tensor out, c10::optional<at::Tensor> bias, bool relu, bool accumulate,
               c10::optional<at::Tensor> stats, double drop_p, int64_t drop_seed, c10::optional<at::Tensor> drop_step, int64_t drop_stream) {
    c10::cuda::CUDAGuard g(A.device());
    const rlr::DropSpec drop = drop_spec(drop_p, drop_seed, drop_step, drop_stream);
    const int M = A.size(0), K = A.size(1), N = B.size(0);
    TORCH_CHECK(B.size(1) == K && out.size(0) == M && out.size(1) == N);
    TORCH_CHECK(!stats.has_value() || !stats->defined() || stats->numel() == (int64_t)rlr::kStatSlots * 2 * N, "stats must be [STAT_SLOTS,2,N]");
    check(rlr::launch_gemm_bf16(bf(A), bf(B), bfm(out), M, N, K, K, K, N, opt<const float>(bias), relu, accumulate, opt<float>(stats),
                                cur_stream(), drop.thr ? &drop : nullptr), "gemm_bf16");
}

void stem_gemm_bf16(at::Tensor A, at::Tensor W, at::Tensor out, c10::optional<at::Tensor> bias, bool relu, c10::optional<at::Tensor> stats,
                    int64_t ready_ptr, int64_t lo, int64_t hi, c10::optional<at::Tensor> epoch) {
    c10::cuda::CUDAGuard g(A.device());
    const int M = A.size(0), N = W.size(0), kvalid = W.size(1);
    TORCH_CHECK(A.dim() == 2 && A.size(1) == 64 && W.dim() == 2 && W.is_contiguous() && out.size(0) == M && out.size(1) == N, "stem_gemm shapes");
    TORCH_CHECK(ready_ptr == 0 || (epoch.has_value() && epoch->defined() && epoch->scalar_type() == at::kInt), "epoch must be an int32 device tensor");
    check(rlr::launch_stem_gemm_bf16(bf(A), bf(W), bfm(out), M, N, kvalid, kvalid, opt<const float>(bias), relu, opt<float>(stats),
                                     reinterpret_cast<const uint32_t*>(ready_ptr), (int)lo, (int)hi,
                                     ready_ptr ? reinterpret_cast<const uint32_t*>(epoch->data_ptr()) : nullptr, cur_stream()), "stem_gemm_bf16");
}

void conv_bf16(at::Tensor x, at::Tensor w, at::Tensor out, int64_t NB, int64_t planes, std::vector<int64_t> dh, std::vector<int64_t> dw,
               std::vector<int64_t> dplane, c10::optional<at::Tensor> bias, bool relu, bool accumulate, c10::optional<at::Tensor> stats,
               std::vector<int64_t> wtap, int64_t w_taps_total) {
    c10::cuda::CUDAGuard g(x.device());
    TORCH_CHECK(x.dim() == 4 && out.dim() == 4 && w.dim() == 2);
    const int Hin = x.size(1), Win = x.size(2), Cin = x.size(3), Ho = out.size(1), Wo = out.size(2), Cout = out.size(3);
    const int T = (int)dh.size();
    const bool bmn = !wtap.empty();
    TORCH_CHECK(x.size(0) == planes * NB && out.size(0) == NB);
    TORCH_CHECK(bmn ? (w.size(0) == Cin && w.size(1) == w_taps_total * Cout && (int)wtap.size() == T)
                    : (w.size(0) == Cout && w.size(1) == (int64_t)T * Cin), "filter shape");
    TORCH_CHECK(!stats.has_value() || !stats->defined() || stats->numel() == (int64_t)rlr::kStatSlots * 2 * Cout, "stats must be [STAT_SLOTS,2,Cout]");
    int a[9], b[9], c[9], wt[9];
    for (int t = 0; t < T; ++t) { a[t] = (int)dh[t]; b[t] = (int)dw[t]; c[t] = (int)dplane[t]; wt[t] = bmn ? (int)wtap[t] : 0; }
    check(rlr::launch_conv_bf16(bf(x), bf(w), bfm(out), (int)NB, (int)planes, Hin, Win, Cin, Ho, Wo, Cout, Cout, T, a, b, c,
                                opt<const float>(bias), relu, accumulate, opt<float>(stats), cur_stream(), bmn ? wt : nullptr,
                                (int)w_taps_total), "conv_bf16");
}

void gemm_splitk_bf16(at::Tensor A, at::Tensor B, at::Tensor out, at::Tensor ws, c10::optional<at::Tensor> bias, bool relu, double drop_p,
                      int64_t drop_seed, c10::optional<at::Tensor> drop_step, int64_t drop_stream) {
    c10::cuda::CUDAGuard g(A.device());
    const rlr::DropSpec drop = drop_spec(drop_p, drop_seed, drop_step, drop_stream);
    const int M = A.size(0), K = A.size(1), N = B.size(0);
    TORCH_CHECK(B.size(1) == K && out.size(0) == M && out.size(1) == N && ws.numel() == (int64_t)M * N);
    check(rlr::launch_gemm_splitk_bf16(bf(A), bf(B), bfm(out), f32(ws), M, N, K, opt<const float>(bias), relu, num_sms(), cur_stream(),
                                       drop.thr ? &drop : nullptr), "gemm_splitk_bf16");
}

void conv_bf16_strided(at::Tensor x, at::Tensor w, at::Tensor out, std::vector<int64_t> dh, std::vector<int64_t> dw,
                       c10::optional<at::Tensor> bias, bool relu, bool accumulate, std::vector<int64_t> wtap, int64_t w_taps_total,
                       int64_t in_stride, int64_t out_stride, int64_t out_ph, int64_t out_pw) {
    c10::cuda::CUDAGuard g(x.device());
    TORCH_CHECK(x.dim() == 4 && out.dim() == 4 && w.dim() == 2 && x.size(0) == out.size(0));
    TORCH_CHECK(out.size(1) % out_stride == 0 && out.size(2) % out_stride == 0, "output image must be a multiple of out_stride");
    const int NB = x.size(0), Hin = x.size(1), Win = x.size(2), Cin = x.size(3), Cout = out.size(3);
    const int Ho = out.size(1) / out_stride, Wo = out.size(2) / out_stride;
    const int T = (int)dh.size();
    const bool bmn = !wtap.empty();
    TORCH_CHECK(bmn ? (w.size(0) == Cin && w.size(1) == w_taps_total * Cout && (int)wtap.size() == T)
                    : (w.size(0) == Cout && w.size(1) == (int64_t)T * Cin), "filter shape");
    int a[9], b[9], c[9] = {0}, wt[9];
    for (int t = 0; t < T; ++t) { a[t] = (int)dh[t]; b[t] = (int)dw[t]; wt[t] = bmn ? (int)wtap[t] : 0; }
    check(rlr::launch_conv_bf16(bf(x), bf(w), bfm(out), NB, 1, Hin, Win, Cin, Ho, Wo, Cout, Cout, T, a, b, c, opt<const float>(bias), relu,
                                accumulate, nullptr, cur_stream(), bmn ? wt : nullptr, (int)w_taps_total, (int)in_stride, (int)out_stride,
                                (int)out_ph, (int)out_pw), "conv_bf16_strided");
}

void conv3x3_halo_bf16(at::Tensor x, at::Tensor w, at::Tensor out, c10::optional<at::Tensor> bias, bool relu, bool accumulate,
                       c10::optional<at::Tensor> stats, int64_t bo_mode, c10::optional<at::Tensor> dbg) {
    c10::cuda::CUDAGuard g(x.device());
    TORCH_CHECK(x.dim() == 4 && x.size(3) == 64 && out.dim() == 4 && w.dim() == 2 && w.size(1) == 9 * 64 && w.size(0) == out.size(3));
    TORCH_CHECK(out.size(0) == x.size(0) && out.size(1) - x.size(1) == out.size(2) - x.size(2), "halo conv: output = input + 2*pad - 2, pad in {0,1,2}");
    TORCH_CHECK(!stats.has_value() || !stats->defined() || stats->numel() == (int64_t)rlr::kStatSlots * 2 * out.size(3), "stats must be [STAT_SLOTS,2,Cout]");
    check(rlr::launch_conv3x3_halo_bf16(bf(x), bf(w), bfm(out), x.size(0), x.size(1), x.size(2), out.size(1), out.size(2), out.size(3), opt<const float>(bias), relu,
                                        accumulate, opt<float>(stats), (int)bo_mode, opt<long long>(dbg), num_sms(), cur_stream()), "conv3x3_halo_bf16");
}

void conv3x3_halo3_bf16(at::Tensor x, at::Tensor w, at::Tensor out, c10::optional<at::Tensor> bias, bool relu, bool accumulate) {
    c10::cuda::CUDAGuard g(x.device());
    TORCH_CHECK(x.dim() == 4 && x.size(3) == 64 && out.dim() == 4 && w.dim() == 2 && w.size(1) == 9 * 64 && w.size(0) == out.size(3));
    TORCH_CHECK(out.size(0) == x.size(0) && out.size(1) == x.size(1) && out.size(2) == x.size(2));
    check(rlr::launch_conv3x3_halo3_bf16(bf(x), bf(w), bfm(out), x.size(0), x.size(1), x.size(2), out.size(3), opt<const float>(bias), relu,
                                         accumulate, num_sms(), cur_stream()), "conv3x3_halo3_bf16");
}

void conv_wgrad_bf16(at::Tensor dy, at::Tensor x, at::Tensor dW, int64_t NB, int64_t planes, int64_t cin_valid, std::vector<int64_t> dh,
                     std::vector<int64_t> dw, std::vector<int64_t> dplane) {
    c10::cuda::CUDAGuard g(x.device());
    TORCH_CHECK(x.dim() == 4 && dy.dim() == 4);
    const int Hin = x.size(1), Win = x.size(2), Cin = x.size(3), Ho = dy.size(1), Wo = dy.size(2), Cout = dy.size(3);
    const int T = (int)dh.size();
    TORCH_CHECK(x.size(0) == planes * NB && dy.size(0) == NB && dW.numel() == (int64_t)Cout * T * cin_valid);
    TORCH_CHECK((Cout <= 64 && Cout % 8 == 0) || Cout % 128 == 0, "wgrad: Cout must be <= 64 or a multiple of 128");
    int a[9], b[9], c[9];
    for (int t = 0; t < T; ++t) { a[t] = (int)dh[t]; b[t] = (int)dw[t]; c[t] = (int)dplane[t]; }
    check(rlr::launch_conv_wgrad_bf16(bf(dy), bf(x), f32(dW), (int)NB, (int)planes, Hin, Win, Cin, (int)cin_valid, Ho, Wo, Cout, T, a, b, c,
                                      num_sms(), cur_stream()), "conv_wgrad_bf16");
}
void conv_wgrad_bf16_strided(at::Tensor dy, at::Tensor x, at::Tensor dW, int64_t cin_valid, std::vector<int64_t> dh, std::vector<int64_t> dw,
                             int64_t in_stride) {
    c10::cuda::CUDAGuard g(x.device());
    TORCH_CHECK(x.dim() == 4 && dy.dim() == 4 && x.size(0) == dy.size(0));
    const int NB = x.size(0), Hin = x.size(1), Win = x.size(2), Cin = x.size(3), Ho = dy.size(1), Wo = dy.size(2), Cout = dy.size(3);
    const int T = (int)dh.size();
    TORCH_CHECK(dW.numel() == (int64_t)Cout * T * cin_valid);
    TORCH_CHECK((Cout <= 64 && Cout % 8 == 0) || Cout % 128 == 0, "wgrad: Cout must be <= 64 or a multiple of 128");
    int a[9], b[9], c[9] = {0};
    for (int t = 0; t < T; ++t) { a[t] = (int)dh[t]; b[t] = (int)dw[t]; }
    check(rlr::launch_conv_wgrad_bf16(bf(dy), bf(x), f32(dW), NB, 1, Hin, Win, Cin, (int)cin_valid, Ho, Wo, Cout, T, a, b, c, num_sms(),
                                      cur_stream(), (int)in_stride), "conv_wgrad_bf16_strided");
}
void conv_wgrad_halo_bf16(at::Tensor dy, at::Tensor x, at::Tensor dW, int64_t cin_valid) {
    c10::cuda::CUDAGuard g(x.device());
    TORCH_CHECK(x.dim() == 4 && x.size(3) == 64 && dy.dim() == 4 && dy.size(0) == x.size(0) && dy.size(1) == x.size(1) && dy.size(2) == x.size(2));
    TORCH_CHECK(dW.numel() == dy.size(3) * 9 * cin_valid);
    check(rlr::launch_conv_wgrad_halo_bf16(bf(dy), bf(x), f32(dW), x.size(0), x.size(1), x.size(2), (int)cin_valid, dy.size(3), num_sms(),
                                           cur_stream()), "conv_wgrad_halo_bf16");
}
void linear_wgrad_bf16(at::Tensor dy, at::Tensor x, at::Tensor dW) {
    c10::cuda::CUDAGuard g(x.device());
    const int B = x.size(0), K = x.size(1), N = dy.size(1);
    TORCH_CHECK(dy.size(0) == B && dW.numel() == (int64_t)N * K && ((N <= 64 && N % 8 == 0) || N % 128 == 0));
    check(rlr::launch_linear_wgrad_bf16(bf(dy), bf(x), f32(dW), B, N, K, num_sms(), cur_stream()), "linear_wgrad_bf16");
}

void ordered_sum(at::Tensor out, at::Tensor part) {
    c10::cuda::CUDAGuard g(out.device());
    TORCH_CHECK(out.is_contiguous() && part.is_contiguous() && part.dim() == 2 && part.size(1) == out.numel() &&
                part.scalar_type() == out.scalar_type(), "ordered_sum: out [n], part [nparts][n]");
    const int nparts = (int)part.size(0);
    const long long n = out.numel();
    if (out.scalar_type() == at::kDouble)
        check(rlr::launch_ordered_sum_f64(out.data_ptr<double>(), part.data_ptr<double>(), nparts, n, cur_stream()), "ordered_sum");
    else
        check(rlr::launch_ordered_sum_f32(out.data_ptr<float>(), part.data_ptr<float>(), nparts, n, cur_stream()), "ordered_sum");
}

void channel_stats(at::Tensor x, at::Tensor stats) {
    c10::cuda::CUDAGuard g(x.device());
    const int C = x.size(-1);
    const int nslots = (int)(stats.numel() / (2 * C));
    TORCH_CHECK(nslots >= 1 && stats.numel() == (int64_t)nslots * 2 * C, "stats must be [slots, 2, C]");
    check(rlr::launch_channel_stats(bf(x), x.numel() / C, C, f32(stats), num_sms(), cur_stream(), 0, nslots), "channel_stats");
}
void bias_grad(at::Tensor dy, at::Tensor db) {
    c10::cuda::CUDAGuard g(dy.device());
    const int C = dy.size(-1);
    TORCH_CHECK(db.numel() == C && db.scalar_type() == at::kFloat && dy.is_contiguous(), "bias_grad: db must be fp32 [C]");
    check(rlr::launch_channel_stats(bf(dy), dy.numel() / C, C, f32(db), num_sms(), cur_stream(), 1), "bias_grad");
}
void bn_finalize(at::Tensor stats, at::Tensor mean_rstd, at::Tensor rm, at::Tensor rv, double count, double eps, double momentum, bool train) {
    c10::cuda::CUDAGuard g(stats.device());
    const int C = mean_rstd.size(-1);
    const int slots = (int)(stats.numel() / (2 * C));
    TORCH_CHECK(slots >= 1 && stats.numel() == (int64_t)slots * 2 * C, "stats must be [slots, 2, C]");
    check(rlr::launch_bn_finalize(f32(stats), slots, f32(mean_rstd), (float*)rm.data_ptr(), (float*)rv.data_ptr(), C, (float)count, (float)eps,
                                  (float)momentum, train, cur_stream()), "bn_finalize");
}
void bn_apply(at::Tensor x, c10::optional<at::Tensor> res, at::Tensor y, at::Tensor gamma, at::Tensor beta, at::Tensor mean_rstd, bool relu,
              int64_t fin_mode, c10::optional<at::Tensor> stats, double count, double eps, double momentum,
              c10::optional<at::Tensor> rm, c10::optional<at::Tensor> rv) {
    c10::cuda::CUDAGuard g(x.device());
    const int C = x.size(-1);
    int slots = 1;
    if (fin_mode == 1) {
        TORCH_CHECK(stats.has_value() && stats->defined() && rm.has_value() && rv.has_value(), "bn_apply: training finalize needs stats and running stats");
        slots = (int)(stats->numel() / (2 * C));
        TORCH_CHECK(slots >= 1 && stats->numel() == (int64_t)slots * 2 * C, "stats must be [slots,2,C]");
    }
    if (fin_mode == 2) TORCH_CHECK(rm.has_value() && rv.has_value(), "bn_apply: eval needs running stats");
    check(rlr::launch_bn_apply(bf(x), bfo(res), bfm(y), (const float*)gamma.data_ptr(), (const float*)beta.data_ptr(), f32(mean_rstd),
                               x.numel() / C, C, relu, (int)fin_mode, opt<const float>(stats), slots, (float)count, (float)eps, (float)momentum,
                               opt<float>(rm), opt<float>(rv), num_sms(), cur_stream()), "bn_apply");
}
void bn_bwd(at::Tensor dy, at::Tensor y, at::Tensor x, at::Tensor gamma, at::Tensor mean_rstd, at::Tensor dsum, at::Tensor dx,
            c10::optional<at::Tensor> dres, at::Tensor dgamma, at::Tensor dbeta, bool relu, bool zero_dsum) {
    c10::cuda::CUDAGuard g(x.device());
    const int C = x.size(-1);
    const long long M = x.numel() / C;
    const int nslots = (int)(dsum.numel() / (2 * C));
    TORCH_CHECK(nslots >= 1 && dsum.numel() == (int64_t)nslots * 2 * C, "dsum must be [slots, 2, C]");
    if (zero_dsum) check(cudaMemsetAsync(dsum.data_ptr(), 0, sizeof(float) * dsum.numel(), cur_stream()), "bn_bwd/memset");
    check(rlr::launch_bn_bwd_reduce(bf(dy), bf(y), bf(x), f32(mean_rstd), f32(dsum), M, C, relu, num_sms(), cur_stream(), nullptr, nullptr, nslots),
          "bn_bwd_reduce");
    check(rlr::launch_bn_bwd_apply(bf(dy), bf(y), bf(x), (const float*)gamma.data_ptr(), f32(mean_rstd), f32(dsum), bfm(dx),
                                   const_cast<__nv_bfloat16*>(bfo(dres)), (float*)dgamma.data_ptr(), (float*)dbeta.data_ptr(), M, C, relu,
                                   num_sms(), cur_stream(), nullptr, nslots), "bn_bwd_apply");
}
void bn_bwd_recompute(at::Tensor dy, at::Tensor x, at::Tensor gamma, at::Tensor beta, at::Tensor mean_rstd, at::Tensor dsum, at::Tensor dx,
                      at::Tensor dgamma, at::Tensor dbeta, bool zero_dsum) {
    c10::cuda::CUDAGuard g(x.device());
    const int C = x.size(-1);
    const long long M = x.numel() / C;
    const int nslots = (int)(dsum.numel() / (2 * C));
    TORCH_CHECK(nslots >= 1 && dsum.numel() == (int64_t)nslots * 2 * C, "dsum must be [slots, 2, C]");
    if (zero_dsum) check(cudaMemsetAsync(dsum.data_ptr(), 0, sizeof(float) * dsum.numel(), cur_stream()), "bn_bwd/memset");
    check(rlr::launch_bn_bwd_reduce(bf(dy), nullptr, bf(x), f32(mean_rstd), f32(dsum), M, C, 2, num_sms(), cur_stream(),
                                    (const float*)gamma.data_ptr(), (const float*)beta.data_ptr(), nslots), "bn_bwd_reduce(recompute)");
    check(rlr::launch_bn_bwd_apply(bf(dy), nullptr, bf(x), (const float*)gamma.data_ptr(), f32(mean_rstd), f32(dsum), bfm(dx), nullptr,
                                   (float*)dgamma.data_ptr(), (float*)dbeta.data_ptr(), M, C, 2, num_sms(), cur_stream(),
                                   (const float*)beta.data_ptr(), nslots), "bn_bwd_apply(recompute)");
}
void relu_bwd(at::Tensor dy, at::Tensor y, double scale) {
    c10::cuda::CUDAGuard g(dy.device());
    check(rlr::launch_relu_bwd(bfm(dy), bf(y), dy.numel(), num_sms(), cur_stream(), (float)scale), "relu_bwd");
}
void maxpool2_fwd(at::Tensor x, at::Tensor y, at::Tensor idx, double drop_p, int64_t drop_seed, c10::optional<at::Tensor> drop_step, int64_t drop_stream) {
    c10::cuda::CUDAGuard g(x.device());
    const rlr::DropSpec d = drop_spec(drop_p, drop_seed, drop_step, drop_stream);
    check(rlr::launch_maxpool2_fwd(bf(x), bfm(y), (uint8_t*)idx.data_ptr(), x.size(0), x.size(1), x.size(2), x.size(3), cur_stream(),
                                   (float)drop_p, d.seed, d.step, d.stream), "maxpool2_fwd");
}
void maxpool2_bwd(at::Tensor dy, at::Tensor idx, at::Tensor dx, double drop_p, int64_t drop_seed, c10::optional<at::Tensor> drop_step, int64_t drop_stream,
                  c10::optional<at::Tensor> relu_out) {
    c10::cuda::CUDAGuard g(dx.device());
    const rlr::DropSpec d = drop_spec(drop_p, drop_seed, drop_step, drop_stream);
    const bool zm = relu_out.has_value() && relu_out->defined();
    TORCH_CHECK(!zm || (relu_out->scalar_type() == at::kBFloat16 && relu_out->is_contiguous() && relu_out->numel() == dy.numel()), "relu_out must match dy");
    TORCH_CHECK(dy.is_contiguous() && dx.is_contiguous() && idx.is_contiguous() && dy.size(1) == dx.size(1) / 2 && dy.size(2) == dx.size(2) / 2);
    check(rlr::launch_maxpool2_bwd(bf(dy), (const uint8_t*)idx.data_ptr(), bfm(dx), dx.size(0), dx.size(1), dx.size(2), dx.size(3), cur_stream(),
                                   (float)drop_p, d.seed, d.step, d.stream, zm ? bf(*relu_out) : nullptr), "maxpool2_bwd");
}
void avgpool_fwd(at::Tensor x, at::Tensor y) {
    c10::cuda::CUDAGuard g(x.device());
    check(rlr::launch_avgpool_fwd(bf(x), bfm(y), x.size(0), x.size(1) * x.size(2), x.size(3), cur_stream()), "avgpool_fwd");
}
void avgpool_bwd(at::Tensor dy, at::Tensor dx) {
    c10::cuda::CUDAGuard g(dx.device());
    check(rlr::launch_avgpool_bwd(bf(dy), bfm(dx), dx.size(0), dx.size(1) * dx.size(2), dx.size(3), cur_stream()), "avgpool_bwd");
}
void dropout_fwd(at::Tensor x, at::Tensor y, at::Tensor mask, double p, int64_t seed, at::Tensor step, int64_t stream) {
    c10::cuda::CUDAGuard g(x.device());
    check(rlr::launch_dropout_fwd(bf(x), bfm(y), (uint8_t*)mask.data_ptr(), x.numel(), (float)p, (uint64_t)seed,
                                  (const long long*)step.data_ptr(), (uint64_t)stream, cur_stream()), "dropout_fwd");
}
void dropout_bwd(at::Tensor dy, at::Tensor mask, at::Tensor dx, double p) {
    c10::cuda::CUDAGuard g(dx.device());
    check(rlr::launch_dropout_bwd(bf(dy), (const uint8_t*)mask.data_ptr(), bfm(dx), dx.numel(), (float)p, cur_stream()), "dropout_bwd");
}
void space_to_depth(at::Tensor x, at::Tensor y) {
    c10::cuda::CUDAGuard g(x.device());
    check(rlr::launch_space_to_depth(bf(x), bfm(y), x.size(0), x.size(1), x.size(2), x.size(3), num_sms(), cur_stream()), "space_to_depth");
}
void im2col_small(at::Tensor x, at::Tensor A, int64_t k, int64_t pad) {
    c10::cuda::CUDAGuard g(x.device());
    const int NB = x.size(0), H = x.size(1), W = x.size(2), C = x.size(3);
    const int Ho = H + 2 * pad - k + 1, Wo = W + 2 * pad - k + 1;
    TORCH_CHECK(x.dim() == 4 && x.is_contiguous() && A.is_contiguous() && A.numel() == (int64_t)NB * Ho * Wo * 64, "im2col_small: A must be [NB*Ho*Wo, 64]");
    check(rlr::launch_im2col_small(bf(x), bfm(A), NB, H, W, C, Ho, Wo, (int)k, (int)pad, num_sms(), cur_stream()), "im2col_small");
}
void depth_to_space(at::Tensor x4, at::Tensor y, bool accumulate, int64_t plane_mask) {
    c10::cuda::CUDAGuard g(y.device());
    check(rlr::launch_depth_to_space(bf(x4), bfm(y), y.size(0), y.size(1), y.size(2), y.size(3), accumulate, (int)plane_mask, num_sms(),
                                     cur_stream()), "depth_to_space");
}
void filter_gather_transpose(at::Tensor w, at::Tensor wt, int64_t Cout, int64_t T, int64_t Cin, std::vector<int64_t> taps) {
    c10::cuda::CUDAGuard g(w.device());
    int t[9];
    TORCH_CHECK(taps.size() >= 1 && taps.size() <= 9);
    for (size_t i = 0; i < taps.size(); ++i) t[i] = (int)taps[i];
    check(rlr::launch_filter_gather_transpose(bf(w), bfm(wt), Cout, T, Cin, (int)taps.size(), t, cur_stream()), "filter_gather_transpose");
}
void filter_transpose(at::Tensor w, at::Tensor wt, int64_t Cout, int64_t ntaps, int64_t Cin) {
    c10::cuda::CUDAGuard g(w.device());
    check(rlr::launch_filter_transpose(bf(w), bfm(wt), Cout, ntaps, Cin, cur_stream()), "filter_transpose");
}
void linear_small_fwd(at::Tensor x, at::Tensor w, c10::optional<at::Tensor> bias, at::Tensor y, bool relu) {
    c10::cuda::CUDAGuard g(x.device());
    check(rlr::launch_linear_small_fwd(bf(x), bf(w), opt<const float>(bias), bfm(y), x.size(0), x.size(1), w.size(0), relu, cur_stream()), "linear_small_fwd");
}
void linear_small_bwd(at::Tensor x, at::Tensor dy, at::Tensor w, c10::optional<at::Tensor> dx, at::Tensor dw, c10::optional<at::Tensor> db,
                      bool accumulate_dx) {
    c10::cuda::CUDAGuard g(x.device());
    check(rlr::launch_linear_small_bwd(bf(x), bf(dy), bf(w), const_cast<__nv_bfloat16*>(bfo(dx)), (float*)dw.data_ptr(), opt<float>(db),
                                       x.size(0), x.size(1), w.size(0), accumulate_dx, cur_stream()), "linear_small_bwd");
}
void linear_small_fwd2(at::Tensor x, at::Tensor w, c10::optional<at::Tensor> bias, at::Tensor y, bool relu) {
    c10::cuda::CUDAGuard g(x.device());
    check(rlr::launch_linear_small_fwd2(bf(x), bf(w), opt<const float>(bias), bfm(y), x.size(0), x.size(1), w.size(0), relu, cur_stream()), "linear_small_fwd2");
}
void linear_small_bwd2(at::Tensor x, at::Tensor dy, at::Tensor w, c10::optional<at::Tensor> dx, at::Tensor dw, c10::optional<at::Tensor> db,
                       bool accumulate_dx) {
    c10::cuda::CUDAGuard g(x.device());
    check(rlr::launch_linear_small_bwd2(bf(x), bf(dy), bf(w), const_cast<__nv_bfloat16*>(bfo(dx)), (float*)dw.data_ptr(), opt<float>(db),
                                        x.size(0), x.size(1), w.size(0), accumulate_dx, cur_stream()), "linear_small_bwd2");
}
}

void register_gemm_bindings(py::module_& m) {
    m.attr("STAT_SLOTS") = rlr::kStatSlots;
    m.def("set_persistent_conv", [](bool on) { rlr::set_persistent_conv(on ? 1 : 0); });
    m.def("set_pdl", [](bool on) { rlr::set_pdl(on ? 1 : 0); });
    m.def("set_conv_occ3", [](int64_t level) { rlr::set_conv_occ3((int)level); });
    m.def("set_conv_tma_store", [](bool on) { rlr::set_conv_tma_store(on ? 1 : 0); });
    m.def("set_conv_split_producer", [](bool on) { rlr::set_conv_split_producer(on ? 1 : 0); });
    m.def("set_conv_trace", [](c10::optional<at::Tensor> buf) {
        rlr::set_conv_trace(buf.has_value() && buf->defined() ? reinterpret_cast<long long*>(buf->data_ptr<int64_t>()) : nullptr);
    });
    m.def("gemm_bf16", &gemm_bf16, py::arg("A"), py::arg("B"), py::arg("out"), py::arg("bias"), py::arg("relu"), py::arg("accumulate"), py::arg("stats"),
          py::arg("drop_p") = 0.0, py::arg("drop_seed") = 0, py::arg("drop_step") = py::none(), py::arg("drop_stream") = 0);
    m.def("stem_gemm_bf16", &stem_gemm_bf16, py::arg("A"), py::arg("W"), py::arg("out"), py::arg("bias"), py::arg("relu"), py::arg("stats"),
          py::arg("ready_ptr") = 0, py::arg("lo") = 0, py::arg("hi") = 0, py::arg("epoch") = py::none());
    m.def("gemm_splitk_bf16", &gemm_splitk_bf16, py::arg("A"), py::arg("B"), py::arg("out"), py::arg("ws"), py::arg("bias"), py::arg("relu"),
          py::arg("drop_p") = 0.0, py::arg("drop_seed") = 0, py::arg("drop_step") = py::none(), py::arg("drop_stream") = 0);
    m.def("conv_bf16", &conv_bf16);
    m.def("conv_bf16_strided", &conv_bf16_strided);
    m.def("conv_wgrad_bf16_strided", &conv_wgrad_bf16_strided);
    m.def("conv3x3_halo_bf16", &conv3x3_halo_bf16);
    m.def("conv3x3_halo3_bf16", &conv3x3_halo3_bf16);
    m.def("conv_wgrad_bf16", &conv_wgrad_bf16);
    m.def("linear_wgrad_bf16", &linear_wgrad_bf16);
    m.def("conv_wgrad_halo_bf16", &conv_wgrad_halo_bf16);
    m.def("channel_stats", &channel_stats);
    m.def("ordered_sum", &ordered_sum);
    m.def("bias_grad", &bias_grad);
    m.def("bn_finalize", &bn_finalize);
    m.def("bn_apply", &bn_apply);
    m.def("bn_bwd", &bn_bwd);
    m.def("bn_bwd_recompute", &bn_bwd_recompute);
    m.def("relu_bwd", &relu_bwd, py::arg("dy"), py::arg("y"), py::arg("scale") = 1.0);
    m.def("maxpool2_fwd", &maxpool2_fwd, py::arg("x"), py::arg("y"), py::arg("idx"), py::arg("drop_p") = 0.0, py::arg("drop_seed") = 0,
          py::arg("drop_step") = py::none(), py::arg("drop_stream") = 0);
    m.def("maxpool2_bwd", &maxpool2_bwd, py::arg("dy"), py::arg("idx"), py::arg("dx"), py::arg("drop_p") = 0.0, py::arg("drop_seed") = 0,
          py::arg("drop_step") = py::none(), py::arg("drop_stream") = 0, py::arg("relu_out") = py::none());
    m.def("avgpool_fwd", &avgpool_fwd);
    m.def("avgpool_bwd", &avgpool_bwd);
    m.def("dropout_fwd", &dropout_fwd);
    m.def("dropout_bwd", &dropout_bwd);
    m.def("space_to_depth", &space_to_depth);
    m.def("im2col_small", &im2col_small);
    m.def("filter_transpose", &filter_transpose);
    m.def("depth_to_space", &depth_to_space);
    m.def("filter_gather_transpose", &filter_gather_transpose);
    m.def("linear_small_fwd", &linear_small_fwd);
    m.def("linear_small_bwd", &linear_small_bwd);
    m.def("linear_small_fwd2", &linear_small_fwd2);
    m.def("linear_small_bwd2", &linear_small_bwd2);
}
```

### defending-against-backdoors-with-robust-learning-rate_b200/ops/csrc/gemm_persistent.cu

```cuda
#include <cuda.h>

#include "common.cuh"
#include "gemm.h"
#include "stem_gather.cuh"
#include "wgmma.cuh"

namespace rlr {

using namespace wg;

constexpr int PBM = 128, PBK = 64, PConsumers = 256, PThreads = PConsumers + 32;

template <int BN, int kOcc = 1>
struct PCfg {
    static constexpr int kStages = kOcc == 2 ? 3 : (BN == 64 ? 7 : 5);
    static constexpr int kABytes = PBM * PBK * 2;
    static constexpr int kBBytes = BN * PBK * 2;
    static constexpr int kStageBytes = kABytes + kBBytes;
    static constexpr int kPitch = BN * 2 + 16;
    static constexpr int kStagingBytes = PBM * kPitch;
    static constexpr int kRingBytes = kStages * kStageBytes;
    static constexpr int kTailBytes = BN == 128 ? 2048 : 1024;
    static constexpr int kSmemBytes = kRingBytes + kStagingBytes + 1024 + kTailBytes;
};

struct __align__(8) PShared {
    uint64_t full[8];
    uint64_t empty[8];
    int row_index[PBM];
};
static_assert(sizeof(PShared) <= 704, "the bias slice starts 704 bytes into the tail");

template <int BN, bool kBMN, int kOcc = 1>
__global__ void __launch_bounds__(PThreads, kOcc)
umma_conv_gemm_persistent_kernel(const __grid_constant__ CUtensorMap tmA, const __grid_constant__ CUtensorMap tmB, const ConvGemmParams p,
                                  const int m_tiles, const int total_tiles) {
    using Cfg = PCfg<BN, kOcc>;
    extern __shared__ uint8_t smem_raw[];
    uint8_t* smem = reinterpret_cast<uint8_t*>((reinterpret_cast<uintptr_t>(smem_raw) + 1023) & ~uintptr_t(1023));
    uint8_t* staging = smem + Cfg::kRingBytes;
    PShared* sh = reinterpret_cast<PShared*>(staging + Cfg::kStagingBytes);
    const int warp = threadIdx.x >> 5, lane = threadIdx.x & 31;

    if (warp == 8 && lane == 0) {
        prefetch_tmap(&tmA); prefetch_tmap(&tmB);
        for (int s = 0; s < Cfg::kStages; ++s) { mbar_init(&sh->full[s], 1); mbar_init(&sh->empty[s], 8); }
        fence_barrier_init();
    }
    __syncthreads();

    auto origin = [&](int tile, int& tile_m, int& tile_n, int& n0, int& h0, int& w0) {
        tile_m = tile % m_tiles; tile_n = tile / m_tiles;
        n0 = h0 = w0 = 0;
        if (p.mode == 1) {
            const int tw_i = tile_m % p.tiles_w, th_i = (tile_m / p.tiles_w) % p.tiles_h, tn_i = tile_m / (p.tiles_w * p.tiles_h);
            w0 = tw_i * p.TW; h0 = th_i * p.TH; n0 = tn_i * p.TN;
        }
    };

    if (warp == 8) {
        if (p.b_src) stem_gather_b(p, smem + Cfg::kABytes, BN, 0, lane);
        if (lane == 0) {
            int stage = 0;
            uint32_t phase = 0;
            for (int tile = blockIdx.x; tile < total_tiles; tile += gridDim.x) {
                int tile_m, tile_n, n0, h0, w0;
                origin(tile, tile_m, tile_n, n0, h0, w0);
                for (int kb = 0; kb < p.num_kb; ++kb) {
                    mbar_wait(&sh->empty[stage], phase ^ 1);
                    uint8_t* sa = smem + stage * Cfg::kStageBytes;
                    uint8_t* sb = sa + Cfg::kABytes;
                    mbar_expect_tx(&sh->full[stage], p.b_src ? Cfg::kABytes : Cfg::kStageBytes);
                    const int tap = p.mode == 1 ? kb / p.cblocks : 0, cb = p.mode == 1 ? kb - tap * p.cblocks : 0;
                    if (p.mode == 1) tma_load_4d(&tmA, &sh->full[stage], sa, cb * PBK, w0 * p.in_stride + p.dw[tap], h0 * p.in_stride + p.dh[tap],
                                                n0 + p.dn[tap]);
                    else tma_load_2d(&tmA, &sh->full[stage], sa, kb * PBK, tile_m * PBM);
                    if (p.b_src) {
                    } else if (kBMN) {
                        for (int g = 0; g < BN / 64; ++g)
                            tma_load_2d(&tmB, &sh->full[stage], sb + g * 8192, p.wtap[tap] * p.wcols + tile_n * BN + g * 64, cb * PBK);
                    } else {
                        tma_load_2d(&tmB, &sh->full[stage], sb, kb * PBK, tile_n * BN);
                    }
                    if (++stage == Cfg::kStages) { stage = 0; phase ^= 1; }
                }
            }
        }
    } else {
        const int et = threadIdx.x;
        const int wgi = et >> 7, t = et & 127;
        const int r0 = wgi * 64 + frag_row(t, 0);
        __nv_bfloat16* out = reinterpret_cast<__nv_bfloat16*>(p.out);
        constexpr int kChunks = BN * 2 / 16;
        constexpr int kIters = PBM * kChunks / PConsumers;
        constexpr int kBatch = kIters < 8 ? kIters : 8;
        float* bias_s = reinterpret_cast<float*>(reinterpret_cast<uint8_t*>(sh) + 704);
        int bias_tile_n = -1;
        int stage = 0;
        uint32_t phase = 0;
        const uint32_t b_fixed = p.b_src ? smem_u32(smem + Cfg::kABytes) : 0u;
        for (int tile = blockIdx.x; tile < total_tiles; tile += gridDim.x) {
            int tile_m, tile_n, n0, h0, w0;
            origin(tile, tile_m, tile_n, n0, h0, w0);
            const int col0 = tile_n * BN;
            if (p.bias && tile_n != bias_tile_n) {
                for (int i = et; i < BN; i += PConsumers) bias_s[i] = (col0 + i < p.N) ? p.bias[col0 + i] : 0.f;
                bias_tile_n = tile_n;
            }
            if (et < PBM) {
                const int row = et;
                int gi;
                if (p.mode == 1) {
                    const int tw = row % p.TW, th = (row / p.TW) % p.TH, tn = row / (p.TW * p.TH);
                    const int w = w0 + tw, h = h0 + th, n = n0 + tn;
                    gi = (w < p.Wo && h < p.Ho && n < p.NB)
                             ? ((n * p.OutH + h * p.out_stride + p.out_ph) * p.OutW + w * p.out_stride + p.out_pw) : -1;
                } else {
                    gi = tile_m * PBM + row;
                    if (gi >= p.M) gi = -1;
                }
                sh->row_index[row] = gi;
            }
            float acc[BN / 2];
#pragma unroll
            for (int i = 0; i < BN / 2; ++i) acc[i] = 0.f;
            consumer_mainloop<BN, Cfg::kStages, Cfg::kStageBytes, Cfg::kABytes, kBMN>(acc, smem, sh->full, sh->empty, p.num_kb,
                                                                                       (uint32_t)wgi * 64 * 128, b_fixed, stage, phase, lane);
            named_bar(1, PConsumers);
#pragma unroll
            for (int j = 0; j < BN / 8; ++j) {
                const int c = frag_col(t, 4 * j);
#pragma unroll
                for (int h = 0; h < 2; ++h) {
                    float a = acc[4 * j + 2 * h], b = acc[4 * j + 2 * h + 1];
                    if (p.bias) { a += bias_s[c]; b += bias_s[c + 1]; }
                    if (p.relu) { a = fmaxf(a, 0.f); b = fmaxf(b, 0.f); }
                    *reinterpret_cast<uint32_t*>(staging + (r0 + 8 * h) * Cfg::kPitch + c * 2) = pack_bf16x2(a, b);
                }
            }
            named_bar(1, PConsumers);
#pragma unroll
            for (int it0 = 0; it0 < kIters; it0 += kBatch) {
                uint4 oldv[kBatch];
                if (p.accumulate) {
#pragma unroll
                    for (int j = 0; j < kBatch; ++j) {
                        const int idx = et + (it0 + j) * PConsumers, r = idx / kChunks, ch = idx - r * kChunks;
                        const int gi = sh->row_index[r];
                        oldv[j] = make_uint4(0, 0, 0, 0);
                        if (gi >= 0 && col0 + ch * 8 < p.N) oldv[j] = *reinterpret_cast<const uint4*>(out + (size_t)gi * p.ldc + col0 + ch * 8);
                    }
                }
#pragma unroll
                for (int j = 0; j < kBatch; ++j) {
                    const int idx = et + (it0 + j) * PConsumers, r = idx / kChunks, ch = idx - r * kChunks;
                    const int gi = sh->row_index[r];
                    if (gi < 0 || col0 + ch * 8 >= p.N) continue;
                    uint4 val = *reinterpret_cast<const uint4*>(staging + r * Cfg::kPitch + ch * 16);
                    if (p.accumulate) {
                        const __nv_bfloat162* o2 = reinterpret_cast<const __nv_bfloat162*>(&oldv[j]);
                        __nv_bfloat162* v2 = reinterpret_cast<__nv_bfloat162*>(&val);
#pragma unroll
                        for (int q = 0; q < 4; ++q) {
                            const float2 a = __bfloat1622float2(v2[q]), b = __bfloat1622float2(o2[q]);
                            v2[q] = __floats2bfloat162_rn(a.x + b.x, a.y + b.y);
                        }
                    }
                    *reinterpret_cast<uint4*>(out + (size_t)gi * p.ldc + col0 + ch * 8) = val;
                }
            }
            named_bar(1, PConsumers);
        }
    }
}

template <int BN>
cudaError_t launch_persistent_bn(const CUtensorMap& tmA, const CUtensorMap& tmB, const ConvGemmParams& p, int m_tiles, int num_sms,
                                 cudaStream_t st, int occ) {
    const int n_tiles = (p.N + BN - 1) / BN;
    const int total = m_tiles * n_tiles;
    if (occ == 2 && !p.b_mn) {
        using Cfg = PCfg<BN, 2>;
        static bool configured2 = false;
        if (!configured2) {
            RLR_CUDA_CHECK(cudaFuncSetAttribute(umma_conv_gemm_persistent_kernel<BN, false, 2>, cudaFuncAttributeMaxDynamicSharedMemorySize, Cfg::kSmemBytes));
            configured2 = true;
        }
        const int grid = total < 2 * num_sms ? total : 2 * num_sms;
        umma_conv_gemm_persistent_kernel<BN, false, 2><<<grid, PThreads, Cfg::kSmemBytes, st>>>(tmA, tmB, p, m_tiles, total);
        return cudaGetLastError();
    }
    using Cfg = PCfg<BN>;
    static bool configured = false;
    if (!configured) {
        RLR_CUDA_CHECK(cudaFuncSetAttribute(umma_conv_gemm_persistent_kernel<BN, false>, cudaFuncAttributeMaxDynamicSharedMemorySize, Cfg::kSmemBytes));
        RLR_CUDA_CHECK(cudaFuncSetAttribute(umma_conv_gemm_persistent_kernel<BN, true>, cudaFuncAttributeMaxDynamicSharedMemorySize, Cfg::kSmemBytes));
        configured = true;
    }
    const int grid = total < num_sms ? total : num_sms;
    if (p.b_mn) umma_conv_gemm_persistent_kernel<BN, true><<<grid, PThreads, Cfg::kSmemBytes, st>>>(tmA, tmB, p, m_tiles, total);
    else umma_conv_gemm_persistent_kernel<BN, false><<<grid, PThreads, Cfg::kSmemBytes, st>>>(tmA, tmB, p, m_tiles, total);
    return cudaGetLastError();
}
template cudaError_t launch_persistent_bn<64>(const CUtensorMap&, const CUtensorMap&, const ConvGemmParams&, int, int, cudaStream_t, int);
template cudaError_t launch_persistent_bn<128>(const CUtensorMap&, const CUtensorMap&, const ConvGemmParams&, int, int, cudaStream_t, int);

}
```

### defending-against-backdoors-with-robust-learning-rate_b200/ops/csrc/norm.cu

```cuda
#include <stdlib.h>

#include "common.cuh"
#include "gemm.h"

namespace rlr {

struct bf8 { float v[8]; };
__device__ __forceinline__ bf8 load8(const __nv_bfloat16* p) {
    const uint4 u = *reinterpret_cast<const uint4*>(p);
    const __nv_bfloat162* h = reinterpret_cast<const __nv_bfloat162*>(&u);
    bf8 r;
#pragma unroll
    for (int i = 0; i < 4; ++i) { const float2 f = __bfloat1622float2(h[i]); r.v[2 * i] = f.x; r.v[2 * i + 1] = f.y; }
    return r;
}
__device__ __forceinline__ void store8(__nv_bfloat16* p, const bf8& r) {
    uint4 u;
    u.x = pack_bf16x2(r.v[0], r.v[1]); u.y = pack_bf16x2(r.v[2], r.v[3]);
    u.z = pack_bf16x2(r.v[4], r.v[5]); u.w = pack_bf16x2(r.v[6], r.v[7]);
    *reinterpret_cast<uint4*>(p) = u;
}
static inline int rows_grid(long long M, int rows_per_block, int num_sms, int per_sm) {
    long long want = (M + rows_per_block - 1) / rows_per_block;
    long long cap = (long long)num_sms * per_sm;
// ... 58 lines not shown
                        dz.y = (xv.y * msc[2 * i + 1] + msh[2 * i + 1]) > 0.f ? dz.y : 0.f;
                    }
                    a[2 * i] += dz.x; a[2 * i + 1] += dz.y;
                    b[2 * i] += dz.x * (xv.x - mu[2 * i]) * rs[2 * i]; b[2 * i + 1] += dz.y * (xv.y - mu[2 * i + 1]) * rs[2 * i + 1];
                }
            }
        }
    }
    float* mine = sh + (size_t)ry * 2 * C + cg * 8;
#pragma unroll
    for (int i = 0; i < 8; ++i) { mine[i] = a[i]; mine[C + i] = b[i]; }
    __syncthreads();
    const int ncols = out_cols > 0 ? out_cols : 2 * C;
    float* dst = part + (size_t)blockIdx.x * ncols;
    for (int i = threadIdx.x; i < ncols; i += 256) {
        float t = 0.f;
        for (int r = 0; r < rpi; ++r) t += sh[(size_t)r * 2 * C + i];
        dst[i] = t;
    }
}

cudaError_t launch_ordered_sum_f32(float* out, const float* part, int nparts, long long n, cudaStream_t st) {
    return launch_ordered_sum(out, part, nparts, n, st);
}
cudaError_t launch_ordered_sum_f64(double* out, const double* part, int nparts, long long n, cudaStream_t st) {
    return launch_ordered_sum(out, part, nparts, n, st);
}

cudaError_t launch_channel_stats(const __nv_bfloat16* x, long long M, int C, float* stats, int num_sms, cudaStream_t st, int only_sum, int nslots) {
    if (!chan_ok(C) || nslots < 1) return cudaErrorInvalidValue;
    const int rpi = 256 / (C / 8);
    const int grid = rows_grid(M, rpi * 8, num_sms, nslots >= 4 ? 4 : 2), ncols = only_sum ? C : 2 * C;
    Scratch part((size_t)grid * ncols * sizeof(float), st);
    RLR_CUDA_CHECK(launch_kernel(channel_reduce_kernel<0, false>, dim3(grid), dim3(256), (size_t)rpi * 2 * C * sizeof(float), st, x, nullptr,
                                 nullptr, nullptr, part.as<float>(), M, C, 0, nullptr, nullptr, only_sum ? C : 0));
    return launch_ordered_sum(stats, part.as<float>(), grid, (long long)ncols, st);
}
cudaError_t launch_bn_bwd_reduce(const __nv_bfloat16* dy, const __nv_bfloat16* y, const __nv_bfloat16* x, const float* mean_rstd,
                                 float* dsum, long long M, int C, int relu, int num_sms, cudaStream_t st, const float* gamma,
                                 const float* beta, int nslots) {
    if (!chan_ok(C) || (relu == 2 && (!gamma || !beta)) || (relu == 1 && !y) || nslots < 1) return cudaErrorInvalidValue;
    const int rpi = 256 / (C / 8);
    const int grid = rows_grid(M, rpi * 8, num_sms, nslots >= 3 ? 3 : 2);
    const size_t smem = (size_t)rpi * 2 * C * sizeof(float);
    Scratch part((size_t)grid * 2 * C * sizeof(float), st);
    if (relu == 2)
        RLR_CUDA_CHECK(launch_kernel(channel_reduce_kernel<1, true>, dim3(grid), dim3(256), smem, st, x, dy, y, mean_rstd, part.as<float>(), M, C,
                                     relu, gamma, beta, 0));
    else
        RLR_CUDA_CHECK(launch_kernel(channel_reduce_kernel<1, false>, dim3(grid), dim3(256), smem, st, x, dy, y, mean_rstd, part.as<float>(), M, C,
                                     relu, nullptr, nullptr, 0));
    return launch_ordered_sum(dsum, part.as<float>(), grid, 2LL * C, st);
}

__global__ void bn_finalize_kernel(const float* __restrict__ stats, int slots, float* __restrict__ mean_rstd, float* running_mean,
                                   float* running_var, int C, float count, float eps, float momentum, int train) {
    const int c = blockIdx.x * blockDim.x + threadIdx.x;
    if (c >= C) return;
    if (train) {
        float s1 = 0.f, s2 = 0.f;
        for (int k = 0; k < slots; ++k) { s1 += stats[(size_t)k * 2 * C + c]; s2 += stats[(size_t)k * 2 * C + C + c]; }
        const float mean = s1 / count;
        const float var = fmaxf(s2 / count - mean * mean, 0.f);
        mean_rstd[c] = mean;
        mean_rstd[C + c] = rsqrtf(var + eps);
        running_mean[c] = (1.f - momentum) * running_mean[c] + momentum * mean;
        const float unbiased = count > 1.f ? var * count / (count - 1.f) : var;
        running_var[c] = (1.f - momentum) * running_var[c] + momentum * unbiased;
    } else {
        mean_rstd[c] = running_mean[c];
        mean_rstd[C + c] = rsqrtf(running_var[c] + eps);
    }
}
cudaError_t launch_bn_finalize(const float* stats, int slots, float* mean_rstd, float* running_mean, float* running_var, int C,
                               float count, float eps, float momentum, int train, cudaStream_t st) {
    bn_finalize_kernel<<<(C + 127) / 128, 128, 0, st>>>(stats, slots, mean_rstd, running_mean, running_var, C, count, eps, momentum, train);
    return cudaGetLastError();
}

struct BnFinalize {
    int mode;
    const float* stats; int slots;
    float count, eps, momentum;
    float* running_mean; float* running_var;
};
template <int U, int kMinBlocks>
__global__ void __launch_bounds__(256, kMinBlocks) bn_apply_kernel(const __nv_bfloat16* __restrict__ x, const __nv_bfloat16* __restrict__ res,
                                                         __nv_bfloat16* __restrict__ y, const float* __restrict__ gamma,
                                                         const float* __restrict__ beta, float* __restrict__ mean_rstd,
                                                         long long M, int C, int relu, BnFinalize fin) {
    pdl_wait();
    pdl_trigger();
    const int tpr = C / 8, rpi = 256 / tpr;
    const int cg = threadIdx.x % tpr, ry = threadIdx.x / tpr;
    float sc[8], sh[8];
#pragma unroll
    for (int i = 0; i < 8; ++i) {
        const int c = cg * 8 + i;
        float mean, rstd;
        if (fin.mode == 1) {
            float s1 = 0.f, s2 = 0.f;
            for (int k = 0; k < fin.slots; ++k) { s1 += fin.stats[(size_t)k * 2 * C + c]; s2 += fin.stats[(size_t)k * 2 * C + C + c]; }
            mean = s1 / fin.count;
            const float var = fmaxf(s2 / fin.count - mean * mean, 0.f);
            rstd = rsqrtf(var + fin.eps);
            if (blockIdx.x == 0 && ry == 0) {
                mean_rstd[c] = mean; mean_rstd[C + c] = rstd;
                fin.running_mean[c] = (1.f - fin.momentum) * fin.running_mean[c] + fin.momentum * mean;
                const float unbiased = fin.count > 1.f ? var * fin.count / (fin.count - 1.f) : var;
                fin.running_var[c] = (1.f - fin.momentum) * fin.running_var[c] + fin.momentum * unbiased;
            }
        } else if (fin.mode == 2) {
            mean = fin.running_mean[c]; rstd = rsqrtf(fin.running_var[c] + fin.eps);
        } else {
            mean = mean_rstd[c]; rstd = mean_rstd[C + c];
        }
        sc[i] = gamma[c] * rstd;
        sh[i] = beta[c] - mean * sc[i];
    }
    const long long stride = (long long)gridDim.x * rpi;
    for (long long r0 = (long long)blockIdx.x * rpi + ry; r0 < M; r0 += stride * U) {
        uint4 xr[U], rr[U];
#pragma unroll
        for (int u = 0; u < U; ++u) {
            const long long r = r0 + u * stride;
            const size_t off = (size_t)(r < M ? r : r0) * C + cg * 8;
            xr[u] = *reinterpret_cast<const uint4*>(x + off);
            if (res) rr[u] = *reinterpret_cast<const uint4*>(res + off);
        }
#pragma unroll
        for (int u = 0; u < U; ++u) {
            const long long r = r0 + u * stride;
            if (r >= M) continue;
            const __nv_bfloat162* xh = reinterpret_cast<const __nv_bfloat162*>(&xr[u]);
            const __nv_bfloat162* rh = reinterpret_cast<const __nv_bfloat162*>(&rr[u]);
            bf8 v;
#pragma unroll
            for (int i = 0; i < 4; ++i) {
                const float2 xv = __bfloat1622float2(xh[i]);
                v.v[2 * i] = xv.x * sc[2 * i] + sh[2 * i]; v.v[2 * i + 1] = xv.y * sc[2 * i + 1] + sh[2 * i + 1];
                if (res) { const float2 q = __bfloat1622float2(rh[i]); v.v[2 * i] += q.x; v.v[2 * i + 1] += q.y; }
                if (relu) { v.v[2 * i] = fmaxf(v.v[2 * i], 0.f); v.v[2 * i + 1] = fmaxf(v.v[2 * i + 1], 0.f); }
            }
            store8(y + (size_t)r * C + cg * 8, v);
        }
    }
}
cudaError_t launch_bn_apply(const __nv_bfloat16* x, const __nv_bfloat16* res, __nv_bfloat16* y, const float* gamma, const float* beta,
                            float* mean_rstd, long long M, int C, int relu, int fin_mode, const float* stats, int slots, float count,
                            float eps, float momentum, float* running_mean, float* running_var, int num_sms, cudaStream_t st) {
    if (!chan_ok(C)) return cudaErrorInvalidValue;
    const int rpi = 256 / (C / 8);
    BnFinalize fin{fin_mode, stats, slots, count, eps, momentum, running_mean, running_var};
    static const int unroll = [] { const char* e = getenv("RLR_BN_UNROLL"); return e ? atoi(e) : 1; }();
    static const int occ = [] { const char* e = getenv("RLR_BN_OCC"); return e ? atoi(e) : 0; }();
    if (unroll <= 1 && occ)
        return launch_kernel(bn_apply_kernel<1, 6>, dim3(rows_grid(M, rpi * 4, num_sms, 12)), dim3(256), (size_t)0, st, x, res, y, gamma, beta, mean_rstd,
                             M, C, relu, fin);
    if (unroll <= 1)
        return launch_kernel(bn_apply_kernel<1, 1>, dim3(rows_grid(M, rpi * 4, num_sms, 8)), dim3(256), (size_t)0, st, x, res, y, gamma, beta, mean_rstd, M,
                             C, relu, fin);
    return launch_kernel(bn_apply_kernel<4, 1>, dim3(rows_grid(M, rpi * 4, num_sms, 6)), dim3(256), (size_t)0, st, x, res, y, gamma, beta, mean_rstd, M, C,
                         relu, fin);
}

template <bool kRecompute, int U, int kMinBlocks = 1>
__global__ void __launch_bounds__(256, kMinBlocks) bn_bwd_apply_kernel(const __nv_bfloat16* __restrict__ dy, const __nv_bfloat16* __restrict__ y,
                                                             const __nv_bfloat16* __restrict__ x, const float* __restrict__ gamma,
                                                             const float* __restrict__ mean_rstd, const float* __restrict__ dsum,
                                                             __nv_bfloat16* __restrict__ dx, __nv_bfloat16* __restrict__ dres,
                                                             float* dgamma, float* dbeta, long long M, int C, int relu,
                                                             const float* __restrict__ beta = nullptr, int nslots = 1) {
    pdl_wait();
    pdl_trigger();
    const int tpr = C / 8, rpi = 256 / tpr;
    const int cg = threadIdx.x % tpr, ry = threadIdx.x / tpr;
    float mu[8], rs[8], g[8], k1[8], k2[8], msh[8];
    const float invM = 1.0f / (float)M;
#pragma unroll
    for (int i = 0; i < 8; ++i) {
        const int c = cg * 8 + i;
        mu[i] = mean_rstd[c]; rs[i] = mean_rstd[C + c]; g[i] = gamma[c] * rs[i];
        float s0 = 0.f, s1 = 0.f;
        for (int k = 0; k < nslots; ++k) { s0 += dsum[(size_t)k * 2 * C + c]; s1 += dsum[(size_t)k * 2 * C + C + c]; }
        k1[i] = s0 * invM; k2[i] = s1 * invM;
        msh[i] = kRecompute ? beta[c] - mu[i] * g[i] : 0.f;
    }
    if (blockIdx.x == 0 && ry == 0) {
#pragma unroll
        for (int i = 0; i < 8; ++i) { dbeta[cg * 8 + i] = k1[i] * (float)M; dgamma[cg * 8 + i] = k2[i] * (float)M; }
    }
    const long long stride = (long long)gridDim.x * rpi;
    for (long long r0 = (long long)blockIdx.x * rpi + ry; r0 < M; r0 += stride * U) {
        bf8 dzv[U], xvv[U], yvv[U];
#pragma unroll
        for (int u = 0; u < U; ++u) {
            const long long r = r0 + u * stride;
            const size_t off = (size_t)(r < M ? r : r0) * C + cg * 8;
            dzv[u] = load8(dy + off);
            xvv[u] = load8(x + off);
            if (!kRecompute && relu) yvv[u] = load8(y + off);
        }
#pragma unroll
        for (int u = 0; u < U; ++u) {
            const long long r = r0 + u * stride;
            if (r >= M) continue;
            const size_t off = (size_t)r * C + cg * 8;
            bf8 dz = dzv[u];
            const bf8 xv = xvv[u];
            if (!kRecompute && relu) {
#pragma unroll
                for (int i = 0; i < 8; ++i) dz.v[i] = yvv[u].v[i] > 0.f ? dz.v[i] : 0.f;
            } else if (kRecompute) {
#pragma unroll
                for (int i = 0; i < 8; ++i) dz.v[i] = (xv.v[i] * g[i] + msh[i]) > 0.f ? dz.v[i] : 0.f;
            }
            if (dres) store8(dres + off, dz);
            bf8 o;
#pragma unroll
            for (int i = 0; i < 8; ++i) o.v[i] = g[i] * (dz.v[i] - k1[i] - (xv.v[i] - mu[i]) * rs[i] * k2[i]);
            store8(dx + off, o);
        }
    }
}
cudaError_t launch_bn_bwd_apply(const __nv_bfloat16* dy, const __nv_bfloat16* y, const __nv_bfloat16* x, const float* gamma,
                                const float* mean_rstd, const float* dsum, __nv_bfloat16* dx, __nv_bfloat16* dres, float* dgamma,
                                float* dbeta, long long M, int C, int relu, int num_sms, cudaStream_t st, const float* beta, int nslots) {
    if (!chan_ok(C) || (relu == 2 && !beta) || (relu == 1 && !y) || nslots < 1) return cudaErrorInvalidValue;
    const int rpi = 256 / (C / 8);
    const int grid = rows_grid(M, rpi * 4, num_sms, 8);
    static const int unroll = [] { const char* e = getenv("RLR_BN_UNROLL"); return e ? atoi(e) : 1; }();
    if (unroll > 1) {
        if (relu == 2)
            return launch_kernel(bn_bwd_apply_kernel<true, 2>, dim3(grid), dim3(256), (size_t)0, st, dy, y, x, gamma, mean_rstd, dsum, dx, dres, dgamma,
                                 dbeta, M, C, relu, beta, nslots);
        return launch_kernel(bn_bwd_apply_kernel<false, 2>, dim3(grid), dim3(256), (size_t)0, st, dy, y, x, gamma, mean_rstd, dsum, dx, dres, dgamma, dbeta,
                             M, C, relu, nullptr, nslots);
    }
    static const int occ = [] { const char* e = getenv("RLR_BN_OCC"); return e ? atoi(e) : 0; }();
    if (occ) {
        const int grid2 = rows_grid(M, rpi * 4, num_sms, 12);
        if (relu == 2)
            return launch_kernel(bn_bwd_apply_kernel<true, 1, 4>, dim3(grid2), dim3(256), (size_t)0, st, dy, y, x, gamma, mean_rstd, dsum, dx, dres, dgamma,
                                 dbeta, M, C, relu, beta, nslots);
        return launch_kernel(bn_bwd_apply_kernel<false, 1, 4>, dim3(grid2), dim3(256), (size_t)0, st, dy, y, x, gamma, mean_rstd, dsum, dx, dres, dgamma,
                             dbeta, M, C, relu, nullptr, nslots);
    }
    if (relu == 2)
        return launch_kernel(bn_bwd_apply_kernel<true, 1>, dim3(grid), dim3(256), (size_t)0, st, dy, y, x, gamma, mean_rstd, dsum, dx, dres, dgamma, dbeta, M,
                             C, relu, beta, nslots);
    return launch_kernel(bn_bwd_apply_kernel<false, 1>, dim3(grid), dim3(256), (size_t)0, st, dy, y, x, gamma, mean_rstd, dsum, dx, dres, dgamma, dbeta, M, C,
                         relu, nullptr, nslots);
}

__global__ void __launch_bounds__(256) relu_bwd_kernel(__nv_bfloat16* __restrict__ dy, const __nv_bfloat16* __restrict__ y, long long n8, float scale) {
    for (long long q = (long long)blockIdx.x * blockDim.x + threadIdx.x; q < n8; q += (long long)gridDim.x * blockDim.x) {
        bf8 d = load8(dy + 8 * q);
        const bf8 yv = load8(y + 8 * q);
#pragma unroll
        for (int i = 0; i < 8; ++i) d.v[i] = yv.v[i] > 0.f ? d.v[i] * scale : 0.f;
        store8(dy + 8 * q, d);
    }
}
cudaError_t launch_relu_bwd(__nv_bfloat16* dy, const __nv_bfloat16* y, long long n, int num_sms, cudaStream_t st, float scale) {
    if (n % 8) return cudaErrorInvalidValue;
    relu_bwd_kernel<<<rows_grid(n / 8, 256, num_sms, 8), 256, 0, st>>>(dy, y, n / 8, scale);
    return cudaGetLastError();
}

__global__ void __launch_bounds__(256) maxpool2_fwd_kernel(const __nv_bfloat16* __restrict__ x, __nv_bfloat16* __restrict__ y,
                                                             uint8_t* __restrict__ idx, int B, int H, int W, int C, DropSpec drop) {
    const int Ho = H / 2, Wo = W / 2, cg_n = C / 8;
    const long long total = (long long)B * Ho * Wo * cg_n;
    for (long long t = (long long)blockIdx.x * blockDim.x + threadIdx.x; t < total; t += (long long)gridDim.x * blockDim.x) {
        const int cg = (int)(t % cg_n);
        long long r = t / cg_n;
        const int wo = (int)(r % Wo); r /= Wo;
        const int ho = (int)(r % Ho);
        const int b = (int)(r / Ho);
        const __nv_bfloat16* base = x + (((size_t)b * H + 2 * ho) * W + 2 * wo) * C + cg * 8;
        bf8 best = load8(base);
        uint8_t bi[8] = {0, 0, 0, 0, 0, 0, 0, 0};
#pragma unroll
        for (int k = 1; k < 4; ++k) {
            const bf8 v = load8(base + ((size_t)(k >> 1) * W + (k & 1)) * C);
#pragma unroll
            for (int i = 0; i < 8; ++i) if (v.v[i] > best.v[i]) { best.v[i] = v.v[i]; bi[i] = (uint8_t)k; }
        }
        const size_t o = (((size_t)b * Ho + ho) * Wo + wo) * C + cg * 8;
        if (drop.thr) {
            const uint32_t keep = dropout_keep8(drop, (long long)(o >> 3));
#pragma unroll
            for (int i = 0; i < 8; ++i) best.v[i] = (keep >> i & 1) ? best.v[i] * drop.scale : 0.f;
        }
        store8(y + o, best);
        uint2 pk;
        pk.x = bi[0] | (bi[1] << 8) | (bi[2] << 16) | (bi[3] << 24);
        pk.y = bi[4] | (bi[5] << 8) | (bi[6] << 16) | (bi[7] << 24);
        *reinterpret_cast<uint2*>(idx + o) = pk;
    }
}
__global__ void __launch_bounds__(256) maxpool2_bwd_kernel(const __nv_bfloat16* __restrict__ dy, const uint8_t* __restrict__ idx,
                                                             __nv_bfloat16* __restrict__ dx, const __nv_bfloat16* __restrict__ zmask,
                                                             int B, int H, int W, int C, DropSpec drop) {
    const int Ho = H / 2, Wo = W / 2, cg_n = C / 8;
    const long long total = (long long)B * Ho * Wo * cg_n;
    for (long long t = (long long)blockIdx.x * blockDim.x + threadIdx.x; t < total; t += (long long)gridDim.x * blockDim.x) {
        const int cg = (int)(t % cg_n);
        long long r = t / cg_n;
        const int wo = (int)(r % Wo); r /= Wo;
        const int ho = (int)(r % Ho);
        const int b = (int)(r / Ho);
        const size_t src = (size_t)t * 8;
        bf8 g = load8(dy + src);
        if (drop.thr) {
            const uint32_t keep = dropout_keep8(drop, (long long)(src >> 3));
#pragma unroll
            for (int i = 0; i < 8; ++i) g.v[i] = (keep >> i & 1) ? g.v[i] * drop.scale : 0.f;
        }
        if (zmask) {
            const bf8 z = load8(zmask + src);
#pragma unroll
            for (int i = 0; i < 8; ++i) g.v[i] = z.v[i] > 0.f ? g.v[i] : 0.f;
        }
        const uint2 pk = *reinterpret_cast<const uint2*>(idx + src);
        bf8 zero;
#pragma unroll
        for (int i = 0; i < 8; ++i) zero.v[i] = 0.f;
#pragma unroll
        for (int me = 0; me < 4; ++me) {
            bf8 o;
#pragma unroll
            for (int i = 0; i < 8; ++i) {
                const int k = ((i < 4 ? pk.x : pk.y) >> (8 * (i & 3))) & 0xff;
                o.v[i] = (k == me) ? g.v[i] : 0.f;
            }
            store8(dx + (((size_t)b * H + 2 * ho + (me >> 1)) * W + 2 * wo + (me & 1)) * C + cg * 8, o);
        }
        const bool last_w = (W & 1) && wo == Wo - 1, last_h = (H & 1) && ho == Ho - 1;
        if (last_w) {
            store8(dx + (((size_t)b * H + 2 * ho) * W + W - 1) * C + cg * 8, zero);
            store8(dx + (((size_t)b * H + 2 * ho + 1) * W + W - 1) * C + cg * 8, zero);
        }
        if (last_h) {
            store8(dx + (((size_t)b * H + H - 1) * W + 2 * wo) * C + cg * 8, zero);
            store8(dx + (((size_t)b * H + H - 1) * W + 2 * wo + 1) * C + cg * 8, zero);
            if (last_w) store8(dx + (((size_t)b * H + H - 1) * W + W - 1) * C + cg * 8, zero);
        }
    }
}
static DropSpec make_drop(float p, uint64_t seed, const long long* step, uint64_t stream) {
    DropSpec d{};
    if (p > 0.f && step) { d.thr = (uint32_t)(p * 65536.0f); d.scale = 1.0f / (1.0f - p); d.seed = seed; d.stream = stream; d.step = step; }
    return d;
}
cudaError_t launch_maxpool2_fwd(const __nv_bfloat16* x, __nv_bfloat16* y, uint8_t* idx, int B, int H, int W, int C, cudaStream_t st, float drop_p,
                                uint64_t seed, const long long* step, uint64_t stream) {
    if (C % 8) return cudaErrorInvalidValue;
    const long long total = (long long)B * (H / 2) * (W / 2) * (C / 8);
    maxpool2_fwd_kernel<<<rows_grid(total, 256, 132, 8), 256, 0, st>>>(x, y, idx, B, H, W, C, make_drop(drop_p, seed, step, stream));
    return cudaGetLastError();
}
cudaError_t launch_maxpool2_bwd(const __nv_bfloat16* dy, const uint8_t* idx, __nv_bfloat16* dx, int B, int H, int W, int C, cudaStream_t st, float drop_p,
                                uint64_t seed, const long long* step, uint64_t stream, const __nv_bfloat16* zmask) {
    if (C % 8 || H < 2 || W < 2) return cudaErrorInvalidValue;
    const long long total = (long long)B * (H / 2) * (W / 2) * (C / 8);
    maxpool2_bwd_kernel<<<rows_grid(total, 256, 132, 8), 256, 0, st>>>(dy, idx, dx, zmask, B, H, W, C, make_drop(drop_p, seed, step, stream));
    return cudaGetLastError();
}

__global__ void avgpool_fwd_kernel(const __nv_bfloat16* __restrict__ x, __nv_bfloat16* __restrict__ y, int B, int HW, int C) {
    const int cg_n = C / 8;
    const int t = blockIdx.x * blockDim.x + threadIdx.x;
    if (t >= B * cg_n) return;
    const int b = t / cg_n, cg = t % cg_n;
    float acc[8] = {0, 0, 0, 0, 0, 0, 0, 0};
    for (int p = 0; p < HW; ++p) {
        const bf8 v = load8(x + ((size_t)b * HW + p) * C + cg * 8);
#pragma unroll
        for (int i = 0; i < 8; ++i) acc[i] += v.v[i];
    }
    bf8 o;
#pragma unroll
    for (int i = 0; i < 8; ++i) o.v[i] = acc[i] / (float)HW;
// ... 406 lines not shown
```

### defending-against-backdoors-with-robust-learning-rate_b200/ops/nn.py

```python
from __future__ import annotations

import os

import torch
import torch.nn.functional as F

_scratch = {}
_s2d_done = {}
STAT_SLOTS = 16
USE_WGRAD_HALO = True
USE_STRIDED_TMA = bool(int(os.environ.get("RLR_STRIDED_TMA", "1")))
USE_IM2COL_STEM = bool(int(os.environ.get("RLR_IM2COL_STEM", "1")))
USE_BN_RECOMPUTE = bool(int(os.environ.get("RLR_BN_RECOMPUTE", "1")))
USE_HALO3 = bool(int(os.environ.get("RLR_HALO3", "0")))
USE_HALO_ANY = bool(int(os.environ.get("RLR_HALO_ANY", "1")))
USE_SPLITK = bool(int(os.environ.get("RLR_SPLITK", "1")))
USE_HEAD_V2 = bool(int(os.environ.get("RLR_HEAD_V2", "1")))


def _stem_ok(k, stride, cin, cout):
    return USE_IM2COL_STEM and stride == 1 and cin * k * k <= 64 and cout % 8 == 0 and (cout <= 64 or cout % 128 == 0)


def stem_geometry(in_shape, a):
    h, w, c = in_shape
    k, s, p = a["k"], a.get("stride", 1), a.get("pad", 0)
    if not _stem_ok(k, s, c, a["cout"]):
        return None
    return k, p, h + 2 * p - k + 1, w + 2 * p - k + 1


def _ext():
    from . import ext
    return ext()


def _zero(t):
    from . import zero_
    return zero_(t)


def _fallback(site, detail=""):
    from . import note_fallback
    note_fallback(site, detail)


def scratch(tag, shape, dtype, device):
    key = (tag, tuple(shape), dtype, str(device))
    t = _scratch.get(key)
    if t is None:
        t = _scratch[key] = torch.zeros(shape, dtype=dtype, device=device)
    return t


def conv_supported(in_shape, a, kind):
    h, w, cin = in_shape
    k, s, p, cout = a["k"], a.get("stride", 1), a.get("pad", 0), a["cout"]
    if k not in (1, 3) or s not in (1, 2) or cout % 8:
        return False
    even = s == 1 or (h % 2 == 0 and w % 2 == 0)
    if kind == "fwd":
        return even and (cin % 64 == 0 or cin < 64)
    if kind == "dgrad":
        return even and cin % 8 == 0 and cout % 64 == 0
    if kind == "wgrad":
        return even and (cin % 64 == 0 or cin < 64) and (cout <= 64 or cout % 128 == 0)
    return False


def _halo_ok(k, stride, pad, cin, h, w, stats=False):
    if not (k == 3 and stride == 1 and cin == 64 and pad in (0, 1, 2)):
        return False
    if not USE_HALO_ANY:
        return pad == 1 and h % 16 == 0 and w % 8 == 0
    ho, wo = h + 2 * pad - 2, w + 2 * pad - 2
    if ho < 1 or wo < 1:
        return False
    if stats and (ho % 16 or wo % 8):
        return False
    return 2 * ho * wo >= (-(-ho // 16) * 16) * (-(-wo // 8) * 8)


def _wgrad_halo_ok(k, stride, pad, cin, h, w):
    return k == 3 and stride == 1 and pad == 1 and cin == 64 and h % 16 == 0 and w % 8 == 0


def _taps(k, stride, pad):
    dh, dw, pl = [], [], []
    for dy in range(k):
        for dx in range(k):
            oy, ox = dy - pad, dx - pad
            if stride == 1:
                dh.append(oy); dw.append(ox); pl.append(0)
            else:
                dh.append(oy // 2); dw.append(ox // 2); pl.append((oy % 2) * 2 + (ox % 2))
    return dh, dw, pl


def conv2d_fwd_sm100(x, w, bias, y, stride, pad, relu, stats, tag="fwd", zero_stats=True, s2d_epoch=None, wait=None):
    e = _ext()
    Cout, k = w.shape[0], w.shape[1]
    if x.dim() == 2:
        B, Ho, Wo, Cin = y.shape[0], y.shape[1], y.shape[2], w.shape[3]
        assert x.shape == (B * Ho * Wo, 64) and _stem_ok(k, stride, Cin, Cout)
        if stats is not None and zero_stats:
            _zero(stats)
        rp, lo, hi, ep = wait if wait is not None else (0, 0, 0, None)
        e.stem_gemm_bf16(x, w.reshape(Cout, k * k * Cin), y.view(B * Ho * Wo, Cout), bias, bool(relu), stats, int(rp), int(lo), int(hi), ep)
        return y
    B, H, W, Cin = x.shape
    if _stem_ok(k, stride, Cin, Cout):
        Ho, Wo = y.shape[1], y.shape[2]
        A = scratch(("im2col", tag), (B * Ho * Wo, 64), x.dtype, x.device)
        e.im2col_small(x.contiguous(), A, k, pad)
        if stats is not None and zero_stats:
            _zero(stats)
        e.stem_gemm_bf16(A, w.reshape(Cout, k * k * Cin), y.view(B * Ho * Wo, Cout), bias, bool(relu), stats, 0, 0, 0, None)
        return y
    if Cin % 64:
        cp = (Cin + 63) // 64 * 64
        xp = scratch(("xpad", tag), (B, H, W, cp), x.dtype, x.device)
        e.pad_rows(x.reshape(B * H * W, Cin), xp.view(B * H * W, cp))
        wp = scratch(("wpad", tag, w.data_ptr()), (Cout, k, k, cp), w.dtype, w.device)
        e.pad_rows(w.reshape(Cout * k * k, Cin), wp.view(Cout * k * k, cp))
        x, w, Cin = xp, wp, cp
    if _halo_ok(k, stride, pad, Cin, H, W, stats is not None):
        if USE_HALO3 and stats is None and pad == 1 and H % 16 == 0:
            e.conv3x3_halo3_bf16(x, w.reshape(Cout, 9 * 64), y, bias, bool(relu), False)
            return y
        if stats is not None and zero_stats:
            _zero(stats)
        e.conv3x3_halo_bf16(x, w.reshape(Cout, 9 * 64), y, bias, bool(relu), False, stats, 0, None)
        return y
    if stride == 2 and USE_STRIDED_TMA and stats is None:
        e.conv_bf16_strided(x, w.reshape(Cout, k * k * Cin), y, [dy_ - pad for dy_ in range(k) for _ in range(k)],
                            [dx_ - pad for _ in range(k) for dx_ in range(k)], bias, bool(relu), False, [], 0, 2, 1, 0, 0)
        return y
    planes = 1
    if stride == 2:
        key = ("s2d", x.data_ptr(), Cin)
        x4 = scratch(key, (4 * B, H // 2, W // 2, Cin), x.dtype, x.device)
        if s2d_epoch is None or _s2d_done.get(key + (B,)) != s2d_epoch:
            e.space_to_depth(x, x4)
            _s2d_done[key + (B,)] = s2d_epoch
        x, planes = x4, 4
    dh, dw, pl = _taps(k, stride, pad)
    if stats is not None and zero_stats:
        _zero(stats)
    e.conv_bf16(x, w.reshape(Cout, k * k * Cin), y, B, planes, dh, dw, pl, bias, bool(relu), False, stats, [], 0)
    return y


def conv2d_dgrad_sm100(dy, w, dx, stride, pad, accumulate):
    e = _ext()
    Cout, k, _, Cin = w.shape
    B = dy.shape[0]
    if stride == 2:
        return _conv2d_dgrad_s2(e, dy, w, dx, pad, accumulate)
    if _halo_ok(k, 1, k - 1 - pad, Cout, dy.shape[1], dy.shape[2]) and dx.shape[-1] % 8 == 0:
        wt = scratch(("wt", w.data_ptr(), dx.data_ptr()), (Cin, k * k * Cout), w.dtype, w.device)
        e.filter_transpose(w, wt, Cout, k * k, Cin)
        if USE_HALO3 and pad == 1 and dy.shape[1] % 16 == 0:
            e.conv3x3_halo3_bf16(dy, wt, dx, None, False, bool(accumulate))
        else:
            e.conv3x3_halo_bf16(dy, wt, dx, None, False, bool(accumulate), None, 0, None)
        return dx
    dh, dw, pl = _taps(k, 1, k - 1 - pad)
    if Cin % 64 == 0:
        T = k * k
        e.conv_bf16(dy, w.reshape(Cout, T * Cin), dx, B, 1, dh, dw, pl, None, False, bool(accumulate), None,
                    [T - 1 - t for t in range(T)], T)
        return dx
    wt = scratch(("wt", w.data_ptr(), dx.data_ptr()), (Cin, k * k * Cout), w.dtype, w.device)
    e.filter_transpose(w, wt, Cout, k * k, Cin)
    e.conv_bf16(dy, wt, dx, B, 1, dh, dw, pl, None, False, bool(accumulate), None, [], 0)
    return dx


def _conv2d_dgrad_s2(e, dy, w, dx, pad, accumulate):
    Cout, k, _, Cin = w.shape
    B, Ho, Wo, _ = dy.shape
    plan = []
    for pi in range(2):
        for pj in range(2):
            taps, dh, dw = [], [], []
            for fy in range(k):
                for fx in range(k):
                    if (pi + pad - fy) % 2 == 0 and (pj + pad - fx) % 2 == 0:
                        taps.append(fy * k + fx); dh.append((pi + pad - fy) // 2); dw.append((pj + pad - fx) // 2)
            if taps:
                plan.append((pi, pj, taps, dh, dw))
    if USE_STRIDED_TMA and Cin % 64 == 0 and dx.shape[1] == 2 * Ho and dx.shape[2] == 2 * Wo:
        if not accumulate and len(plan) < 4:
            _zero(dx)
        for pi, pj, taps, dh, dw in plan:
            e.conv_bf16_strided(dy, w.reshape(Cout, k * k * Cin), dx, dh, dw, None, False, bool(accumulate), taps, k * k, 1, 2, pi, pj)
        return dx
    dx4 = scratch(("dx4", w.data_ptr(), dx.data_ptr()), (4 * B, Ho, Wo, Cin), dy.dtype, dy.device)
    mask = 0
    for pi, pj, taps, dh, dw in plan:
        plane = pi * 2 + pj
        mask |= 1 << plane
        if Cin % 64 == 0:
            e.conv_bf16(dy, w.reshape(Cout, k * k * Cin), dx4[plane * B:(plane + 1) * B], B, 1, dh, dw, [0] * len(taps), None,
                        False, False, None, taps, k * k)
            continue
        wt = scratch(("wt_s2", w.data_ptr(), dx.data_ptr(), plane), (Cin, len(taps) * Cout), w.dtype, w.device)
        e.filter_gather_transpose(w, wt, Cout, k * k, Cin, taps)
        e.conv_bf16(dy, wt, dx4[plane * B:(plane + 1) * B], B, 1, dh, dw, [0] * len(taps), None, False, False, None, [], 0)
    e.depth_to_space(dx4, dx, bool(accumulate), mask)
    return dx


def conv2d_wgrad_sm100(x, dy, gw, gb, stride, pad, tag="fwd", zero=True):
    e = _ext()
    Cout, k = gw.shape[0], gw.shape[1]
    pre = x.dim() == 2
    B, H, W, Cin = (dy.shape[0], 0, 0, gw.shape[3]) if pre else x.shape
    cin_valid = Cin
    if pre or _stem_ok(k, stride, Cin, Cout):
        Ho, Wo = dy.shape[1], dy.shape[2]
        A = x if pre else scratch(("im2col", tag), (B * Ho * Wo, 64), x.dtype, x.device)
        dW = scratch(("dwstem", tag), (Cout, 64), torch.float32, x.device)
        _zero(dW)
        e.linear_wgrad_bf16(dy.view(B * Ho * Wo, Cout), A, dW)
        if zero:
            _zero(gw)
        e.unpad_add(dW, gw.view(Cout, k * k * Cin))
        if gb is not None:
            _bias_grad(e, dy, gb, zero)
        return
    if Cin % 64:
        cp = (Cin + 63) // 64 * 64
        x = scratch(("xpad", tag), (B, H, W, cp), x.dtype, x.device)
        Cin = cp
    planes = 1
    strided = stride == 2 and USE_STRIDED_TMA
    if stride == 2 and not strided:
        x = scratch(("s2d", x.data_ptr(), Cin), (4 * B, H // 2, W // 2, Cin), x.dtype, x.device)
        planes = 4
    dh, dw, pl = _taps(k, stride, pad)
    if zero:
        _zero(gw)
    if strided:
        e.conv_wgrad_bf16_strided(dy, x, gw, cin_valid, [dy_ - pad for dy_ in range(k) for _ in range(k)],
                                  [dx_ - pad for _ in range(k) for dx_ in range(k)], 2)
    elif USE_WGRAD_HALO and _wgrad_halo_ok(k, stride, pad, Cin, H, W) and (Cout <= 64 or Cout % 128 == 0):
        e.conv_wgrad_halo_bf16(dy, x, gw, cin_valid)
    else:
        e.conv_wgrad_bf16(dy, x, gw, B, planes, cin_valid, dh, dw, pl)
    if gb is not None:
        _bias_grad(e, dy, gb, zero)


def _bias_ok(C):
    return C >= 8 and C <= 2048 and C % 8 == 0 and 256 % (C // 8) == 0


def _bias_grad(e, dy, gb, zero):
    C = dy.shape[-1]
    if zero:
        _zero(gb)
    if _bias_ok(C):
        e.bias_grad(dy.contiguous(), gb)
    else:
        _fallback("bias_grad", f"C={C}")
        gb.add_(dy.float().reshape(-1, C).sum(0))


def bn_fwd(x, y, res, gamma, beta, rm, rv, stats, mean_rstd, count, eps, momentum, train, relu, impl, stats_buf=None):
    C = x.shape[-1]
    if impl == "sm100":
        e = _ext()
        if train and stats is None:
            if stats_buf is not None:
                stats = stats_buf
            else:
                stats = scratch(("bnstats", mean_rstd.data_ptr()), (1, 2, C), torch.float32, x.device)
                _zero(stats)
            e.channel_stats(x, stats)
        e.bn_apply(x, res, y, gamma, beta, mean_rstd, bool(relu), 1 if train else 2, stats if train else None, float(count), float(eps),
                   float(momentum), rm, rv)
        return
    xf = x.float().reshape(-1, C)
    if train:
        if stats is not None:
            tot = stats.reshape(-1, 2, C).sum(0)
            mean = tot[0] / count
            var = (tot[1] / count - mean * mean).clamp_min(0)
# ... 194 lines not shown
```

Measured before the change: 0.5362.

## Replace atomic slot-based BN statistics with per-CTA partials and ordered reduction

Conv epilogues no longer atomically add BN sums into a 16-slot arena. Each CTA now writes per-column partial sums to a scratch buffer, and a separate ordered-sum kernel reduces them, which makes the statistics deterministic and removes atomic contention. Epilogue statistics are extended to strided and persistent conv paths, and the BN unroll default changes from 1 to 4. This adds an extra reduction kernel launch and scratch traffic per stats-producing conv, and epilogue stats stay off by default (RLR_EPILOGUE_BN_STATS=0).

```diff
diff --git a/defending-against-backdoors-with-robust-learning-rate_b200/models/native.py b/defending-against-backdoors-with-robust-learning-rate_b200/models/native.py
--- a/defending-against-backdoors-with-robust-learning-rate_b200/models/native.py
+++ b/defending-against-backdoors-with-robust-learning-rate_b200/models/native.py
@@ -15,8 +15,6 @@
 EPILOGUE_BN_STATS = bool(int(os.environ.get("RLR_EPILOGUE_BN_STATS", "0")))
 FWD_BRANCH = bool(int(os.environ.get("RLR_FWD_BRANCH", "1")))
 BWD_BRANCH = bool(int(os.environ.get("RLR_BWD_BRANCH", "1")))
-EPI_STAT_SLOTS = min(16, max(1, int(os.environ.get("RLR_EPI_STAT_SLOTS", "2"))))
-FWD_SLOTS = BWD_SLOTS = max(1, int(os.environ.get("RLR_BN_SLOTS", "1")))
 WGRAD_OVERLAP = bool(int(os.environ.get("RLR_WGRAD_OVERLAP", "1")))
 
 
@@ -52,7 +50,6 @@
         self.impl = dict(conv_fwd=default, conv_dgrad=default, conv_wgrad=default, bn=default, pool=default,
                          linear=default, dropout=default) if not isinstance(impl, dict) else dict(impl)
         self.seed = seed
-        self.fuse_bn_stats = False
         self.first_wait = None
         self.after_first_op = None
         self.step_counter = torch.zeros(1, dtype=torch.int64, device=device)
@@ -219,16 +216,14 @@
         self.grad[self.out_tid] = torch.empty((B, *self.tshape[self.out_tid]), dtype=self.act_dtype, device=dev)
         self.logits = torch.empty((B, self.tshape[self.out_tid][-1]), dtype=torch.float32, device=dev)
         need = [op for op in self.plan if op.kind == "bn" or (op.kind == "conv" and op.saved.get("want_stats"))]
-        S = ops.STAT_SLOTS
         tot = sum(2 * op.out_shape[-1] for op in need)
-        self.stats_arena = torch.zeros(max(1, tot * S), dtype=torch.float32, device=dev)
-        D = BWD_SLOTS
-        self.dsum_arena = torch.zeros(max(1, tot * D), dtype=torch.float32, device=dev)
+        self.stats_arena = torch.zeros(max(1, tot), dtype=torch.float32, device=dev)
+        self.dsum_arena = torch.zeros(max(1, tot), dtype=torch.float32, device=dev)
         off = 0
         for op in need:
             c = op.out_shape[-1]
-            op.saved["stats"] = self.stats_arena[off * S:(off + 2 * c) * S].view(S, 2, c)
-            op.saved["dsum"] = self.dsum_arena[off * D:(off + 2 * c) * D].view(D, 2, c)
+            op.saved["stats"] = self.stats_arena[off:off + 2 * c].view(1, 2, c)
+            op.saved["dsum"] = self.dsum_arena[off:off + 2 * c].view(1, 2, c)
             op.saved["mean_rstd"] = torch.zeros(2, c, dtype=torch.float32, device=dev)
             off += 2 * c
         for op in self.plan:
@@ -337,9 +332,11 @@
             torch.cuda.current_stream(self.device).wait_stream(self._side)
             self._side = None
 
-    def _epilogue_stats_free(self, op):
+    def _epilogue_stats(self, op):
         if not EPILOGUE_BN_STATS or self.impl["conv_fwd"] != "sm100":
             return False
+        if self.impl["conv_dgrad"] == "sm100" and self.impl["bn"] == "sm100":
+            return True
         a = op.attrs
         return a.get("stride", 1) == 1 and a["cin"] % 64 == 0 and a["cout"] % 64 == 0 and not (a["k"] == 3 and a["cin"] == 64)
 
@@ -347,7 +344,7 @@
         a = op.attrs
         x, y = self.T(op.x, B), self.T(op.y, B)
         bias = self.pw.get(op.name + ".bias")
-        stats = op.saved.get("stats") if (train and op.saved.get("want_stats") and (self.fuse_bn_stats or self._epilogue_stats_free(op))) else None
+        stats = op.saved.get("stats") if (train and op.saved.get("want_stats") and self._epilogue_stats(op)) else None
         op.saved["stats_done"] = stats is not None
         if self.impl["conv_fwd"] == "sm100" and ops.conv_supported(op.in_shape, a, "fwd"):
             ops.conv2d_fwd_sm100(x, self.pwb[op.name + ".weight"], bias, y, a.get("stride", 1), a.get("pad", 0), op.relu, stats, tag=(id(self), op.name),
@@ -413,12 +410,10 @@
         rm, rv = self.pw[op.name + ".running_mean"], self.pw[op.name + ".running_var"]
         prod = op.saved["producer"]
         stats = prod.saved["stats"] if (train and prod is not None and prod.saved.get("stats_done")) else None
-        if stats is not None and not self.fuse_bn_stats:
-            stats = stats[0:EPI_STAT_SLOTS]
         count = x.numel() // x.shape[-1]
         ops.bn_fwd(x, y, res, gamma, beta, rm, rv, stats, op.saved["mean_rstd"], count, a.get("eps", 1e-5),
                    a.get("momentum", 0.1), train, op.relu, self.impl["bn"],
-                   stats_buf=op.saved["stats"][0:FWD_SLOTS] if train else None)
+                   stats_buf=op.saved["stats"] if train else None)
 
     def _bwd_bn(self, op, B):
         x, y, dy = self.T(op.x, B), self.T(op.y, B), self.G(op.y, B)
diff --git a/defending-against-backdoors-with-robust-learning-rate_b200/ops/csrc/common.cuh b/defending-against-backdoors-with-robust-learning-rate_b200/ops/csrc/common.cuh
--- a/defending-against-backdoors-with-robust-learning-rate_b200/ops/csrc/common.cuh
+++ b/defending-against-backdoors-with-robust-learning-rate_b200/ops/csrc/common.cuh
@@ -87,6 +87,18 @@
     if (warp == 0 && col < n) out[col] += s;
 }
 
+template <int kCols, int kSlots>
+__device__ __forceinline__ void store_col_partials(const float* red, float* part, int row, int N, int col0, int tid, int nthreads) {
+    for (int i = tid; i < 2 * kCols; i += nthreads) {
+        const int c = i % kCols;
+        if (col0 + c >= N) continue;
+        float s = red[i];
+#pragma unroll
+        for (int q = 1; q < kSlots; ++q) s += red[q * 2 * kCols + i];
+        part[(size_t)row * 2 * N + (i / kCols) * N + col0 + c] = s;
+    }
+}
+
 __device__ __forceinline__ unsigned long long gtimer() {
     unsigned long long t;
     asm volatile("mov.u64 %0, %%globaltimer;" : "=l"(t));
@@ -237,6 +249,13 @@
     return launch_kernel(ordered_sum_kernel<T>, dim3((unsigned)blocks), dim3(256), (size_t)0, st, out, part, nparts, n);
 }
 
+template <typename F>
+inline cudaError_t launch_with_partials(float* out, int rows, long long cols, cudaStream_t st, F&& launch) {
+    Scratch part((size_t)rows * cols * sizeof(float), st);
+    RLR_CUDA_CHECK(launch(part.as<float>()));
+    return launch_ordered_sum(out, part.as<float>(), rows, cols, st);
+}
+
 __device__ __forceinline__ uint32_t pack_bf16x2(float lo, float hi) {
     __nv_bfloat162 v = __floats2bfloat162_rn(lo, hi);
     return *reinterpret_cast<uint32_t*>(&v);
diff --git a/defending-against-backdoors-with-robust-learning-rate_b200/ops/csrc/conv_halo.cu b/defending-against-backdoors-with-robust-learning-rate_b200/ops/csrc/conv_halo.cu
--- a/defending-against-backdoors-with-robust-learning-rate_b200/ops/csrc/conv_halo.cu
+++ b/defending-against-backdoors-with-robust-learning-rate_b200/ops/csrc/conv_halo.cu
@@ -38,7 +38,6 @@
     uint64_t w_full;
     uint64_t halo_full[HL_STAGES];
     uint64_t halo_empty[HL_STAGES];
-    float red[128];
     float bias[64];
 };
 
@@ -61,7 +60,6 @@
         for (int s = 0; s < HL_STAGES; ++s) { mbar_init(&sh->halo_full[s], 1); mbar_init(&sh->halo_empty[s], 4); }
         fence_barrier_init();
     }
-    if (threadIdx.x < 128) sh->red[threadIdx.x] = 0.f;
     const int tiles_per_img = p.tiles_h * p.tiles_w;
     pdl_wait();
     pdl_trigger();
@@ -195,17 +193,17 @@
                     st1[i] += __shfl_xor_sync(0xffffffffu, st1[i], o);
                     st2[i] += __shfl_xor_sync(0xffffffffu, st2[i], o);
                 }
+            float* red = reinterpret_cast<float*>(s_stage);
+            named_bar(3, 256);
             if (lane < 4)
 #pragma unroll
                 for (int i = 0; i < 16; ++i) {
                     const int c = frag_col(t, 2 * (i & ~1)) + (i & 1);
-                    atomicAdd(&sh->red[c], st1[i]);
-                    atomicAdd(&sh->red[64 + c], st2[i]);
+                    red[warp * 128 + c] = st1[i];
+                    red[warp * 128 + 64 + c] = st2[i];
                 }
             named_bar(3, 256);
-            if (threadIdx.x < 128 && col0 + (threadIdx.x & 63) < p.N)
-                atomicAdd(p.stats + (size_t)(blockIdx.x % kStatSlots) * 2 * p.N + (threadIdx.x < 64 ? 0 : p.N) + col0 + (threadIdx.x & 63),
-                          sh->red[threadIdx.x]);
+            store_col_partials<64, 8>(red, p.stats, blockIdx.x, p.N, col0, threadIdx.x, 256);
         }
     }
 }
@@ -244,7 +242,12 @@
     if (gx > p.num_tiles) gx = p.num_tiles;
     if (gx < 1) gx = 1;
     const dim3 grid(gx, n_tiles_n);
-    if (stats) return launch_kernel(umma_conv3x3_halo_kernel<true, false>, grid, dim3(HL_THREADS), HL_SMEM, st, tmX, tmW, p);
+    if (stats)
+        return launch_with_partials(stats, gx, 2LL * Cout, st, [&](float* part) {
+            HaloParams q = p;
+            q.stats = part;
+            return launch_kernel(umma_conv3x3_halo_kernel<true, false>, grid, dim3(HL_THREADS), HL_SMEM, st, tmX, tmW, q);
+        });
     if (accumulate) return launch_kernel(umma_conv3x3_halo_kernel<false, true>, grid, dim3(HL_THREADS), HL_SMEM, st, tmX, tmW, p);
     return launch_kernel(umma_conv3x3_halo_kernel<false, false>, grid, dim3(HL_THREADS), HL_SMEM, st, tmX, tmW, p);
 }
diff --git a/defending-against-backdoors-with-robust-learning-rate_b200/ops/csrc/gemm.cu b/defending-against-backdoors-with-robust-learning-rate_b200/ops/csrc/gemm.cu
--- a/defending-against-backdoors-with-robust-learning-rate_b200/ops/csrc/gemm.cu
+++ b/defending-against-backdoors-with-robust-learning-rate_b200/ops/csrc/gemm.cu
@@ -25,7 +25,7 @@
     static constexpr int kPitch = BN * 2 + 16;
     static constexpr int kStagingBytes = BM * kPitch;
     static constexpr int kRingBytes = kStages * kStageBytes;
-    static_assert(kStagingBytes + 2 * BN * 4 <= kRingBytes, "staging aliases the operand ring");
+    static_assert(kStagingBytes + 8 * 2 * BN * 4 <= kRingBytes, "staging and the per-warp statistics partials alias the operand ring");
     static constexpr int kTailBytes = BN == 128 ? 2048 : 1024;
     static constexpr int kSmemBytes = kRingBytes + 1024  + kTailBytes;
 };
@@ -168,10 +168,6 @@
         int gi_r[2];
         gi_r[0] = tail->row_index[r0];
         gi_r[1] = tail->row_index[r0 + 8];
-        if (kStats) {
-            for (int i = et; i < 2 * BN; i += kEpiThreads) red[i] = 0.f;
-            named_bar(1, kEpiThreads);
-        }
         const bool tma_out = !kStats && p.tma_store;
 #pragma unroll
         for (int j = 0; j < BN / 8; ++j) {
@@ -207,8 +203,9 @@
                         s2[e] += __shfl_xor_sync(0xffffffffu, s2[e], o);
                     }
                 if (lane < 4) {
-                    atomicAdd(&red[c], s1[0]); atomicAdd(&red[c + 1], s1[1]);
-                    atomicAdd(&red[BN + c], s2[0]); atomicAdd(&red[BN + c + 1], s2[1]);
+                    float* mine = red + warp * 2 * BN;
+                    mine[c] = s1[0]; mine[c + 1] = s1[1];
+                    mine[BN + c] = s2[0]; mine[BN + c + 1] = s2[1];
                 }
             }
         }
@@ -225,7 +222,7 @@
                 }
                 tma_store_commit();
             }
-            if (p.stats) {
+            if (!kBMN && p.stats) {
                 constexpr int kPerCol = kEpiThreads / BN, kRows = BM / kPerCol;
                 const int c = et % BN;
                 const int r_lo = (et / BN) * kRows, r_hi = r_lo + kRows;
@@ -238,11 +235,10 @@
                     const float v = __bfloat162float(*reinterpret_cast<const __nv_bfloat16*>(colp + r * 128 + ((chunk ^ (r & 7)) << 4)));
                     s1 += v; s2 += v * v;
                 }
-                if (col0 + c < p.N) {
-                    float* dst = p.stats + (size_t)(blockIdx.x % p.stat_slots) * 2 * p.N + col0 + c;
-                    atomicAdd(dst, s1);
-                    atomicAdd(dst + p.N, s2);
-                }
+                float* mine = red + (et / BN) * 2 * BN;
+                mine[c] = s1; mine[BN + c] = s2;
+                named_bar(1, kEpiThreads);
+                store_col_partials<BN, kPerCol>(red, p.stats, blockIdx.x, p.N, col0, et, kEpiThreads);
             }
             if (et == 0) tma_store_wait_read();
         } else {
@@ -282,12 +278,7 @@
                 *reinterpret_cast<uint4*>(out + (size_t)gi * p.ldc + col0 + ch * 8) = val;
             }
         }
-        if (kStats) {
-            named_bar(1, kEpiThreads);
-            for (int i = et; i < 2 * BN; i += kEpiThreads)
-                if (col0 + (i % BN) < p.N)
-                    atomicAdd(p.stats + (size_t)(blockIdx.x % kStatSlots) * 2 * p.N + (i < BN ? 0 : p.N) + col0 + (i % BN), red[i]);
-        }
+        if (kStats) store_col_partials<BN, 8>(red, p.stats, blockIdx.x, p.N, col0, et, kEpiThreads);
         }
     }
 }
@@ -402,27 +393,9 @@
 }
 
 template <int BN>
-static cudaError_t launch_bn(const CUtensorMap& tmA, const CUtensorMap& tmB, const ConvGemmParams& p_in, int m_tiles, cudaStream_t st) {
+static cudaError_t launch_bn_grid(const CUtensorMap& tmA, const CUtensorMap& tmB, const CUtensorMap& tmC, const ConvGemmParams& p, int m_tiles,
+                                  cudaStream_t st) {
     using Cfg = TileCfg<BN>;
-    ConvGemmParams p = p_in;
-    p.dbg = g_trace;
-    CUtensorMap tmC = tmA;
-    {
-        static const int epi_slots = [] { const char* e = getenv("RLR_EPI_STAT_SLOTS"); int v = e ? atoi(e) : 2; return v < 1 ? 1 : (v > kStatSlots ? kStatSlots : v); }();
-        p.stat_slots = epi_slots;
-    }
-    p.tma_store = 0;
-    if (tma_store_enabled() && !p.accumulate && ((reinterpret_cast<uintptr_t>(p.out) & 15) == 0) && make_out_tmap(&tmC, p) == cudaSuccess)
-        p.tma_store = 1;
-    if (g_split_prod < 0) { const char* e = getenv("RLR_SPLIT_PRODUCER"); g_split_prod = (e && atoi(e) == 0) ? 0 : 1; }
-    p.split_prod = (g_split_prod && !p.b_src) ? 1 : 0;
-    if (p.b_src && !p.stats && p.N <= BN) {
-        static const int stem_persistent = [] { const char* e = getenv("RLR_STEM_PERSISTENT"); return e ? atoi(e) : 2; }();
-        if (stem_persistent && m_tiles >= 2 * sm_count())
-            return launch_persistent_bn<BN>(tmA, tmB, p, m_tiles, sm_count(), st, stem_persistent == 2 ? 2 : 1);
-    }
-    if (!p.stats && !p.b_src && persistent_sms() > 0 && m_tiles * ((p.N + BN - 1) / BN) > persistent_sms())
-        return launch_persistent_bn<BN>(tmA, tmB, p, m_tiles, persistent_sms(), st);
     if constexpr (BN == 64)
         if ((!p.stats || p.tma_store) && conv_occ3() >= 1) return launch_bn_occ3<BN>(tmA, tmB, tmC, p, m_tiles, st);
     static bool configured = false;
@@ -436,6 +409,34 @@
     if (p.b_mn) return launch_kernel(umma_conv_gemm_kernel<BN, false, true>, grid, dim3(kThreads), Cfg::kSmemBytes, st, tmA, tmB, tmC, p);
     if (p.stats && !p.tma_store) return launch_kernel(umma_conv_gemm_kernel<BN, true, false>, grid, dim3(kThreads), Cfg::kSmemBytes, st, tmA, tmB, tmC, p);
     return launch_kernel(umma_conv_gemm_kernel<BN, false, false>, grid, dim3(kThreads), Cfg::kSmemBytes, st, tmA, tmB, tmC, p);
+}
+
+template <int BN>
+static cudaError_t launch_bn(const CUtensorMap& tmA, const CUtensorMap& tmB, const ConvGemmParams& p_in, int m_tiles, cudaStream_t st) {
+    ConvGemmParams p = p_in;
+    p.dbg = g_trace;
+    CUtensorMap tmC = tmA;
+    p.tma_store = 0;
+    if (tma_store_enabled() && !p.accumulate && ((reinterpret_cast<uintptr_t>(p.out) & 15) == 0) && make_out_tmap(&tmC, p) == cudaSuccess)
+        p.tma_store = 1;
+    if (g_split_prod < 0) { const char* e = getenv("RLR_SPLIT_PRODUCER"); g_split_prod = (e && atoi(e) == 0) ? 0 : 1; }
+    p.split_prod = (g_split_prod && !p.b_src) ? 1 : 0;
+    if (p.b_src && p.N <= BN) {
+        static const int stem_persistent = [] { const char* e = getenv("RLR_STEM_PERSISTENT"); return e ? atoi(e) : 2; }();
+        if (stem_persistent && m_tiles >= 2 * sm_count())
+            return launch_persistent_bn<BN>(tmA, tmB, p, m_tiles, sm_count(), st, stem_persistent == 2 ? 2 : 1);
+    }
+    if (!p.stats && !p.b_src && persistent_sms() > 0 && m_tiles * ((p.N + BN - 1) / BN) > persistent_sms())
+        return launch_persistent_bn<BN>(tmA, tmB, p, m_tiles, persistent_sms(), st);
+    if (p.stats) {
+        float* const stats = p.stats;
+        return launch_with_partials(stats, m_tiles, 2LL * p.N, st, [&](float* part) {
+            ConvGemmParams q = p;
+            q.stats = part;
+            return launch_bn_grid<BN>(tmA, tmB, tmC, q, m_tiles, st);
+        });
+    }
+    return launch_bn_grid<BN>(tmA, tmB, tmC, p, m_tiles, st);
 }
 
 static int pick_bn(int N) { return (N % 128 == 0) ? 128 : 64; }
diff --git a/defending-against-backdoors-with-robust-learning-rate_b200/ops/csrc/gemm.h b/defending-against-backdoors-with-robust-learning-rate_b200/ops/csrc/gemm.h
--- a/defending-against-backdoors-with-robust-learning-rate_b200/ops/csrc/gemm.h
+++ b/defending-against-backdoors-with-robust-learning-rate_b200/ops/csrc/gemm.h
@@ -6,8 +6,6 @@
 #include "dropspec.h"
 
 namespace rlr {
-
-constexpr int kStatSlots = 16;
 
 struct ConvGemmParams {
     int M, N, num_kb;
@@ -37,7 +35,6 @@
     int ldc;
     const float* bias;
     float* stats;
-    int stat_slots;
     int relu, accumulate;
 };
 
diff --git a/defending-against-backdoors-with-robust-learning-rate_b200/ops/csrc/gemm_binding.cpp b/defending-against-backdoors-with-robust-learning-rate_b200/ops/csrc/gemm_binding.cpp
--- a/defending-against-backdoors-with-robust-learning-rate_b200/ops/csrc/gemm_binding.cpp
+++ b/defending-against-backdoors-with-robust-learning-rate_b200/ops/csrc/gemm_binding.cpp
@@ -32,6 +32,12 @@
     return reinterpret_cast<float*>(t.data_ptr());
 }
 
+inline void check_stats(const c10::optional<at::Tensor>& stats, int64_t N) {
+    if (!stats.has_value() || !stats->defined()) return;
+    TORCH_CHECK(stats->is_cuda() && stats->scalar_type() == at::kFloat && stats->is_contiguous() && stats->numel() >= 2 * N &&
+                stats->numel() % (2 * N) == 0, "stats must be a contiguous fp32 [S,2,N] buffer");
+}
+
 static rlr::DropSpec drop_spec(double p, int64_t seed, const c10::optional<at::Tensor>& step, int64_t stream) {
     rlr::DropSpec d{};
     if (p > 0.0) {
@@ -48,7 +54,7 @@
     const rlr::DropSpec drop = drop_spec(drop_p, drop_seed, drop_step, drop_stream);
     const int M = A.size(0), K = A.size(1), N = B.size(0);
     TORCH_CHECK(B.size(1) == K && out.size(0) == M && out.size(1) == N);
-    TORCH_CHECK(!stats.has_value() || !stats->defined() || stats->numel() == (int64_t)rlr::kStatSlots * 2 * N, "stats must be [STAT_SLOTS,2,N]");
+    check_stats(stats, N);
     check(rlr::launch_gemm_bf16(bf(A), bf(B), bfm(out), M, N, K, K, K, N, opt<const float>(bias), relu, accumulate, opt<float>(stats),
                                 cur_stream(), drop.thr ? &drop : nullptr), "gemm_bf16");
 }
@@ -58,6 +64,7 @@
     c10::cuda::CUDAGuard g(A.device());
     const int M = A.size(0), N = W.size(0), kvalid = W.size(1);
     TORCH_CHECK(A.dim() == 2 && A.size(1) == 64 && W.dim() == 2 && W.is_contiguous() && out.size(0) == M && out.size(1) == N, "stem_gemm shapes");
+    check_stats(stats, N);
     TORCH_CHECK(ready_ptr == 0 || (epoch.has_value() && epoch->defined() && epoch->scalar_type() == at::kInt), "epoch must be an int32 device tensor");
     check(rlr::launch_stem_gemm_bf16(bf(A), bf(W), bfm(out), M, N, kvalid, kvalid, opt<const float>(bias), relu, opt<float>(stats),
                                      reinterpret_cast<const uint32_t*>(ready_ptr), (int)lo, (int)hi,
@@ -75,7 +82,7 @@
     TORCH_CHECK(x.size(0) == planes * NB && out.size(0) == NB);
     TORCH_CHECK(bmn ? (w.size(0) == Cin && w.size(1) == w_taps_total * Cout && (int)wtap.size() == T)
                     : (w.size(0) == Cout && w.size(1) == (int64_t)T * Cin), "filter shape");
-    TORCH_CHECK(!stats.has_value() || !stats->defined() || stats->numel() == (int64_t)rlr::kStatSlots * 2 * Cout, "stats must be [STAT_SLOTS,2,Cout]");
+    check_stats(stats, Cout);
     int a[9], b[9], c[9], wt[9];
     for (int t = 0; t < T; ++t) { a[t] = (int)dh[t]; b[t] = (int)dw[t]; c[t] = (int)dplane[t]; wt[t] = bmn ? (int)wtap[t] : 0; }
     check(rlr::launch_conv_bf16(bf(x), bf(w), bfm(out), (int)NB, (int)planes, Hin, Win, Cin, Ho, Wo, Cout, Cout, T, a, b, c,
@@ -95,9 +102,10 @@
 
 void conv_bf16_strided(at::Tensor x, at::Tensor w, at::Tensor out, std::vector<int64_t> dh, std::vector<int64_t> dw,
                        c10::optional<at::Tensor> bias, bool relu, bool accumulate, std::vector<int64_t> wtap, int64_t w_taps_total,
-                       int64_t in_stride, int64_t out_stride, int64_t out_ph, int64_t out_pw) {
+                       int64_t in_stride, int64_t out_stride, int64_t out_ph, int64_t out_pw, c10::optional<at::Tensor> stats) {
     c10::cuda::CUDAGuard g(x.device());
     TORCH_CHECK(x.dim() == 4 && out.dim() == 4 && w.dim() == 2 && x.size(0) == out.size(0));
+    check_stats(stats, out.size(3));
     TORCH_CHECK(out.size(1) % out_stride == 0 && out.size(2) % out_stride == 0, "output image must be a multiple of out_stride");
     const int NB = x.size(0), Hin = x.size(1), Win = x.size(2), Cin = x.size(3), Cout = out.size(3);
     const int Ho = out.size(1) / out_stride, Wo = out.size(2) / out_stride;
@@ -108,7 +116,7 @@
     int a[9], b[9], c[9] = {0}, wt[9];
     for (int t = 0; t < T; ++t) { a[t] = (int)dh[t]; b[t] = (int)dw[t]; wt[t] = bmn ? (int)wtap[t] : 0; }
     check(rlr::launch_conv_bf16(bf(x), bf(w), bfm(out), NB, 1, Hin, Win, Cin, Ho, Wo, Cout, Cout, T, a, b, c, opt<const float>(bias), relu,
-                                accumulate, nullptr, cur_stream(), bmn ? wt : nullptr, (int)w_taps_total, (int)in_stride, (int)out_stride,
+                                accumulate, opt<float>(stats), cur_stream(), bmn ? wt : nullptr, (int)w_taps_total, (int)in_stride, (int)out_stride,
                                 (int)out_ph, (int)out_pw), "conv_bf16_strided");
 }
 
@@ -117,7 +125,7 @@
     c10::cuda::CUDAGuard g(x.device());
     TORCH_CHECK(x.dim() == 4 && x.size(3) == 64 && out.dim() == 4 && w.dim() == 2 && w.size(1) == 9 * 64 && w.size(0) == out.size(3));
     TORCH_CHECK(out.size(0) == x.size(0) && out.size(1) - x.size(1) == out.size(2) - x.size(2), "halo conv: output = input + 2*pad - 2, pad in {0,1,2}");
-    TORCH_CHECK(!stats.has_value() || !stats->defined() || stats->numel() == (int64_t)rlr::kStatSlots * 2 * out.size(3), "stats must be [STAT_SLOTS,2,Cout]");
+    check_stats(stats, out.size(3));
     check(rlr::launch_conv3x3_halo_bf16(bf(x), bf(w), bfm(out), x.size(0), x.size(1), x.size(2), out.size(1), out.size(2), out.size(3), opt<const float>(bias), relu,
                                         accumulate, opt<float>(stats), (int)bo_mode, opt<long long>(dbg), num_sms(), cur_stream()), "conv3x3_halo_bf16");
 }
@@ -334,7 +342,6 @@
 }
 
 void register_gemm_bindings(py::module_& m) {
-    m.attr("STAT_SLOTS") = rlr::kStatSlots;
     m.def("set_persistent_conv", [](bool on) { rlr::set_persistent_conv(on ? 1 : 0); });
     m.def("set_pdl", [](bool on) { rlr::set_pdl(on ? 1 : 0); });
     m.def("set_conv_occ3", [](int64_t level) { rlr::set_conv_occ3((int)level); });
@@ -350,7 +357,9 @@
     m.def("gemm_splitk_bf16", &gemm_splitk_bf16, py::arg("A"), py::arg("B"), py::arg("out"), py::arg("ws"), py::arg("bias"), py::arg("relu"),
           py::arg("drop_p") = 0.0, py::arg("drop_seed") = 0, py::arg("drop_step") = py::none(), py::arg("drop_stream") = 0);
     m.def("conv_bf16", &conv_bf16);
-    m.def("conv_bf16_strided", &conv_bf16_strided);
+    m.def("conv_bf16_strided", &conv_bf16_strided, py::arg("x"), py::arg("w"), py::arg("out"), py::arg("dh"), py::arg("dw"), py::arg("bias"),
+          py::arg("relu"), py::arg("accumulate"), py::arg("wtap"), py::arg("w_taps_total"), py::arg("in_stride"), py::arg("out_stride"),
+          py::arg("out_ph"), py::arg("out_pw"), py::arg("stats") = py::none());
     m.def("conv_wgrad_bf16_strided", &conv_wgrad_bf16_strided);
     m.def("conv3x3_halo_bf16", &conv3x3_halo_bf16);
     m.def("conv3x3_halo3_bf16", &conv3x3_halo3_bf16);
diff --git a/defending-against-backdoors-with-robust-learning-rate_b200/ops/csrc/gemm_persistent.cu b/defending-against-backdoors-with-robust-learning-rate_b200/ops/csrc/gemm_persistent.cu
--- a/defending-against-backdoors-with-robust-learning-rate_b200/ops/csrc/gemm_persistent.cu
+++ b/defending-against-backdoors-with-robust-learning-rate_b200/ops/csrc/gemm_persistent.cu
@@ -99,6 +99,8 @@
         int stage = 0;
         uint32_t phase = 0;
         const uint32_t b_fixed = p.b_src ? smem_u32(smem + Cfg::kABytes) : 0u;
+        constexpr int kPerCol = PConsumers / BN, kRows = PBM / kPerCol;
+        float s1 = 0.f, s2 = 0.f;
         for (int tile = blockIdx.x; tile < total_tiles; tile += gridDim.x) {
             int tile_m, tile_n, n0, h0, w0;
             origin(tile, tile_m, tile_n, n0, h0, w0);
@@ -139,6 +141,15 @@
                 }
             }
             named_bar(1, PConsumers);
+            if (p.stats) {
+                const int c = et % BN, r_lo = (et / BN) * kRows;
+#pragma unroll 8
+                for (int r = r_lo; r < r_lo + kRows; ++r) {
+                    if (sh->row_index[r] < 0) continue;
+                    const float v = __bfloat162float(*reinterpret_cast<const __nv_bfloat16*>(staging + r * Cfg::kPitch + c * 2));
+                    s1 += v; s2 += v * v;
+                }
+            }
 #pragma unroll
             for (int it0 = 0; it0 < kIters; it0 += kBatch) {
                 uint4 oldv[kBatch];
@@ -171,12 +182,19 @@
             }
             named_bar(1, PConsumers);
         }
+        if (p.stats) {
+            float* red = reinterpret_cast<float*>(staging);
+            red[(et / BN) * 2 * BN + et % BN] = s1;
+            red[(et / BN) * 2 * BN + BN + et % BN] = s2;
+            named_bar(1, PConsumers);
+            store_col_partials<BN, kPerCol>(red, p.stats, blockIdx.x, p.N, 0, et, PConsumers);
+        }
     }
 }
 
 template <int BN>
-cudaError_t launch_persistent_bn(const CUtensorMap& tmA, const CUtensorMap& tmB, const ConvGemmParams& p, int m_tiles, int num_sms,
-                                 cudaStream_t st, int occ) {
+static cudaError_t launch_persistent_grid(const CUtensorMap& tmA, const CUtensorMap& tmB, const ConvGemmParams& p, int m_tiles, int num_sms,
+                                          cudaStream_t st, int occ) {
     const int n_tiles = (p.N + BN - 1) / BN;
     const int total = m_tiles * n_tiles;
     if (occ == 2 && !p.b_mn) {
@@ -202,6 +220,19 @@
     else umma_conv_gemm_persistent_kernel<BN, false><<<grid, PThreads, Cfg::kSmemBytes, st>>>(tmA, tmB, p, m_tiles, total);
     return cudaGetLastError();
 }
+
+template <int BN>
+cudaError_t launch_persistent_bn(const CUtensorMap& tmA, const CUtensorMap& tmB, const ConvGemmParams& p, int m_tiles, int num_sms,
+                                 cudaStream_t st, int occ) {
+    if (!p.stats) return launch_persistent_grid<BN>(tmA, tmB, p, m_tiles, num_sms, st, occ);
+    if (p.N > BN || p.b_mn) return cudaErrorInvalidValue;
+    const int ctas = (occ == 2 ? 2 : 1) * num_sms, grid = m_tiles < ctas ? m_tiles : ctas;
+    return launch_with_partials(p.stats, grid, 2LL * p.N, st, [&](float* part) {
+        ConvGemmParams q = p;
+        q.stats = part;
+        return launch_persistent_grid<BN>(tmA, tmB, q, m_tiles, num_sms, st, occ);
+    });
+}
 template cudaError_t launch_persistent_bn<64>(const CUtensorMap&, const CUtensorMap&, const ConvGemmParams&, int, int, cudaStream_t, int);
 template cudaError_t launch_persistent_bn<128>(const CUtensorMap&, const CUtensorMap&, const ConvGemmParams&, int, int, cudaStream_t, int);
 
diff --git a/defending-against-backdoors-with-robust-learning-rate_b200/ops/csrc/norm.cu b/defending-against-backdoors-with-robust-learning-rate_b200/ops/csrc/norm.cu
--- a/defending-against-backdoors-with-robust-learning-rate_b200/ops/csrc/norm.cu
+++ b/defending-against-backdoors-with-robust-learning-rate_b200/ops/csrc/norm.cu
@@ -234,7 +234,7 @@
     if (!chan_ok(C)) return cudaErrorInvalidValue;
     const int rpi = 256 / (C / 8);
     BnFinalize fin{fin_mode, stats, slots, count, eps, momentum, running_mean, running_var};
-    static const int unroll = [] { const char* e = getenv("RLR_BN_UNROLL"); return e ? atoi(e) : 1; }();
+    static const int unroll = [] { const char* e = getenv("RLR_BN_UNROLL"); return e ? atoi(e) : 4; }();
     static const int occ = [] { const char* e = getenv("RLR_BN_OCC"); return e ? atoi(e) : 0; }();
     if (unroll <= 1 && occ)
         return launch_kernel(bn_apply_kernel<1, 6>, dim3(rows_grid(M, rpi * 4, num_sms, 12)), dim3(256), (size_t)0, st, x, res, y, gamma, beta, mean_rstd,
@@ -311,7 +311,7 @@
     if (!chan_ok(C) || (relu == 2 && !beta) || (relu == 1 && !y) || nslots < 1) return cudaErrorInvalidValue;
     const int rpi = 256 / (C / 8);
     const int grid = rows_grid(M, rpi * 4, num_sms, 8);
-    static const int unroll = [] { const char* e = getenv("RLR_BN_UNROLL"); return e ? atoi(e) : 1; }();
+    static const int unroll = [] { const char* e = getenv("RLR_BN_UNROLL"); return e ? atoi(e) : 4; }();
     if (unroll > 1) {
         if (relu == 2)
             return launch_kernel(bn_bwd_apply_kernel<true, 2>, dim3(grid), dim3(256), (size_t)0, st, dy, y, x, gamma, mean_rstd, dsum, dx, dres, dgamma,
diff --git a/defending-against-backdoors-with-robust-learning-rate_b200/ops/nn.py b/defending-against-backdoors-with-robust-learning-rate_b200/ops/nn.py
--- a/defending-against-backdoors-with-robust-learning-rate_b200/ops/nn.py
+++ b/defending-against-backdoors-with-robust-learning-rate_b200/ops/nn.py
@@ -132,9 +132,12 @@
             _zero(stats)
         e.conv3x3_halo_bf16(x, w.reshape(Cout, 9 * 64), y, bias, bool(relu), False, stats, 0, None)
         return y
-    if stride == 2 and USE_STRIDED_TMA and stats is None:
+    if stride == 2 and USE_STRIDED_TMA:
+        if stats is not None and zero_stats:
+            _zero(stats)
         e.conv_bf16_strided(x, w.reshape(Cout, k * k * Cin), y, [dy_ - pad for dy_ in range(k) for _ in range(k)],
-                            [dx_ - pad for _ in range(k) for dx_ in range(k)], bias, bool(relu), False, [], 0, 2, 1, 0, 0)
+                            [dx_ - pad for _ in range(k) for dx_ in range(k)], bias, bool(relu), False, [], 0, 2, 1, 0, 0,
+                            **({} if stats is None else {"stats": stats}))
         return y
     planes = 1
     if stride == 2:
```

Measured after the change: 0.5455, median of 6. 1.7% higher.
